# alipbcs/ZetaRay

Measured on AMD Instinct MI355X. Metric: Mrays/s, higher is better.
Workload: dtype f32; 1 GPU; Cornell Box (cornell_emissive: 58 triangles, 2 emissive) 1920x1080, G-buffer + ReSTIR PT (K1 + K11-K16: initial candidates, temporal + spatial reconnection reuse, boiling suppression; 3 non-transmissive / 4 glossy-transmissive bounces, static camera); integrator=restir_pt, parallelism=screen tiles (1, 1), settle_frames=32, ramp_frames=350, arith=contract, library=libzetaray_amd.so, frame_overlap=True, kernel_class=plain

## Files before the change

zetaray_amd/csrc/zr_api.hip:

```cpp
#include <hip/hip_runtime.h>
#include <immintrin.h>
#include <string>
#include <vector>
#include <cstdio>
#include <cstdarg>
#include <cstring>
#include <new>
#include <mutex>
#include "zr_stages.h"
#include "zr_rpt.h"
#include "zr_rdi.h"
#include "zr_sdi.h"
#include "zr_rgi.h"
#include "zr_rgi_spatial.h"
#include "zr_bvh.h"
#include "zr_taa.h"
#include "zr_svgf.h"
#include "zr_post.h"
#include "../../include/zr_srgb_table.h"

static const uint16_t kRptSampleSet[1024] = {
#include "zr_rpt_sample_set.inc"
};


static thread_local std::string g_err;
static int Fail(int code, const char* fmt, ...)
{
    char buf[512];
    va_list ap; va_start(ap, fmt); vsnprintf(buf, sizeof(buf), fmt, ap); va_end(ap);
    g_err = buf;
    return code;
}
#define HIP_TRY(expr) do { hipError_t e_ = (expr); if (e_ != hipSuccess) return Fail(ZR_ERR_HIP, "%s failed: %s (%s:%d)", #expr, hipGetErrorString(e_), __FILE__, __LINE__); } while (0)

static int RequireDevice(int device)
{
    int n = 0;
    hipError_t e = hipGetDeviceCount(&n);
    if (e != hipSuccess || n <= 0) return Fail(ZR_ERR_NO_DEVICE, "no usable HIP device (hipGetDeviceCount: %s); libzetaray_amd has no CPU path", hipGetErrorString(e));
    if (device < 0 || device >= n) return Fail(ZR_ERR_INVALID_ARG, "device %d out of range (0..%d)", device, n - 1);
    HIP_TRY(hipSetDevice(device));
    return ZR_OK;
}

#include "zr_kernels.h"

#ifdef ZR_EXPERIMENTS
#define ZR_EXP_ENV(name) std::getenv(name)
#else
#define ZR_EXP_ENV(name) ((const char*)nullptr)
#endif
#include "zr_bvh_device.h"
namespace zr { int DeviceProbeRun(int device, float min_ms, zr_device_probe* out, std::string& err); }
namespace zr { hipError_t LaunchInscattering(hipStream_t s, const SceneView& sc, const zr_frame_constants& g, const InscatterParams& c, uint32_t* grid); }
namespace zr { hipError_t LaunchDisplayView(hipStream_t s, int option, const GBuf& gb, uint32_t dw, uint32_t dh, float cameraNear, float roughnessTh, F4* out, uint32_t* outSrgb); }
namespace zr { hipError_t LaunchPickOutline(hipStream_t s, const zr_vertex* vertices, const uint32_t* indices, const zr_mesh_instance* instances, uint32_t inst, uint32_t numTris,
    const post::PickWvp& m, uint32_t dw, uint32_t dh, uint32_t rw, uint32_t rh, int4* tris, uint32_t* count, uint8_t* mask, F4* out, uint32_t* outSrgb); }
namespace zr { hipError_t LaunchMoveInstances(hipStream_t st, zr_mesh_instance* cur, const zr_mesh_instance* prev, float* toWorld, uint32_t n, uint32_t* slot,
    const uint32_t* moved, uint32_t nMoved, zr_emissive_triangle* emissives, const zr_emissive_triangle* object, const uint32_t* owner, uint32_t emFirst, uint32_t emEnd); }
ZR_RPT_GROUPS_PRODUCT(extern template)
#ifdef ZR_EXPERIMENTS
ZR_RPT_GROUP_C(extern template)
#endif

__global__ void __launch_bounds__(kBlock) k_gbuffer(SceneView sc, zr_frame_constants g, GBuf gb, uint32_t tilesX, uint32_t pickXY, uint32_t* pick)
{
    uint32_t x, y; PixelOfThread(tilesX, gb.x0, gb.y0, &x, &y);
    if (x >= gb.x0 + gb.w || y >= gb.y0 + gb.h) return;
    ZR_TRAV_STACK(stack);
    GBufferPixel(sc, g, gb, x, y, stack, nullptr, (x | (y << 16)) == pickXY ? pick : nullptr);
}

template<bool TEX, bool PLAIN>
__global__ void __launch_bounds__(kBlock) k_pt_init(SceneView sc, zr_frame_constants g, GBuf gb, PtParams prm, float* finalRGBA,
    F4* firstBOP, PathQueue out, uint32_t* outCount, uint32_t* outRays, uint32_t cap, uint32_t tilesX)
{
    sc.plain = PLAIN; gb.plain = PLAIN;
    uint32_t x, y; PixelOfThread(tilesX, gb.x0, gb.y0, &x, &y);
    PathOut po; po.alive = false;
    if (x < gb.x0 + gb.w && y < gb.y0 + gb.h) PtInitPixel(sc, g, gb, prm, x, y, finalRGBA, firstBOP, po, TEX);
    const uint32_t slot = AllocPathAndRaysBlock(outCount, out.rayList, cap, outRays, po.alive, po.alive && po.rayC_d.w >= 0, po.alive && po.rayM_d.w >= 0, po.alive && po.rayS_d.w >= 0);
    if (po.alive) WritePath(out, slot, po, TEX);
}

__global__ void __launch_bounds__(kBlock) k_trace_simple(SceneView sc, PathQueue q, const uint32_t* rayCount, uint32_t cap, unsigned long long* counters)
{
    const uint32_t nC = rayCount[0], nM = rayCount[kCounterStride], total = nC + nM + rayCount[2 * kCounterStride];
    ZR_TRAV_STACK(stack);
#ifdef ZR_NODE_CACHE_MORE
    ZR_NODE_CACHE_FILL(stack, sc, kBlock);
#endif
    for (uint32_t base = blockIdx.x * kBlock; base < total; base += gridDim.x * kBlock)
    {
        const uint32_t j = base + threadIdx.x;
        bool closest = false, shadow = false;
        if (j < total)
        {
            uint32_t type, i;
            RayOfIndex(q.rayList, cap, nC, nM, j, type, i);
            F4 ro, rd;
            if (type == 0) { rd = q.rayC_d[i]; ro = q.rayC_o[i]; }
            else if (type == 1) { rd = q.rayM_d[i]; ro = q.rayM_o[i]; }
            else { rd = q.rayS_d[i]; ro = q.rayS_o[i]; }
            const uint32_t lightID = type == 2 ? q.sLightID[i] : 0u;
            const bool vis = type == 2 && lightID == kVisibilityRayID;
            const RawHit h = TraverseDyn(sc, xyz(ro), xyz(rd), ro.w, rd.w, (type == 2 && !vis) ? ZR_SUBGROUP_NON_EMISSIVE : ZR_SUBGROUP_ALL, stack, vis);
            if (type == 0) q.hitC[i] = PackRawHit(h);
            else if (type == 1) q.hitM[i] = PackRawHit(h);
            else q.visS[i] = SegmentVisible(sc, h, lightID);
            closest = type != 2; shadow = type == 2;
        }
        CountWave(&counters[0], closest);
        CountWave(&counters[1], shadow);
    }
}

static constexpr uint32_t kTraceChunk = 256;
static constexpr uint32_t kTraceRefillAt = 16;
__global__ void __launch_bounds__(kBlock) k_trace(SceneView sc, PathQueue q, const uint32_t* rayCount, uint32_t cap, uint32_t* cursor, unsigned long long* counters)
{
    const uint32_t nC = rayCount[0], nM = rayCount[kCounterStride], total = nC + nM + rayCount[2 * kCounterStride];
    ZR_TRAV_STACK(stack);
    const uint32_t lane = __lane_id();
    TravState st; TravLane L; L.triCur = 0; L.triEnd = 0; L.done = true;
    uint32_t slot = 0;
    bool laneAnyHit = false;
    uint32_t nClosest = 0, nShadow = 0;
    uint32_t chunkPos = 0, chunkEnd = 0;
    bool exhausted = false;
    for (;;)
    {
        const bool atTri = L.triCur < L.triEnd;
        const bool atNode = !L.done && !atTri;
        const uint64_t mIdle = __ballot(L.done);
        const uint32_t nNode = (uint32_t)__popcll(__ballot(atNode)), nTri = (uint32_t)__popcll(__ballot(atTri)), nIdle = (uint32_t)__popcll(mIdle);
        const bool canRefill = !(exhausted && chunkPos == chunkEnd);
        if (nNode + nTri == 0 && !canRefill) break;
        if (canRefill && (nIdle >= kTraceRefillAt || nNode + nTri == 0))
        {
            if (chunkPos == chunkEnd)
            {
                uint32_t b = 0;
                if (lane == 0) b = atomicAdd(cursor, kTraceChunk);
                b = __builtin_amdgcn_readfirstlane(b);
                exhausted = b >= total;
                chunkPos = b < total ? b : total;
                chunkEnd = b + kTraceChunk < total ? b + kTraceChunk : total;
            }
            const uint32_t rank = (uint32_t)__popcll(mIdle & ((1ull << lane) - 1ull));
            const uint32_t j = chunkPos + rank;
            if (L.done && j < chunkEnd)
            {
                uint32_t type, i;
                RayOfIndex(q.rayList, cap, nC, nM, j, type, i);
                slot = i | (type << 30);
                F4 ro, rd;
                if (type == 0) { rd = q.rayC_d[i]; ro = q.rayC_o[i]; }
                else if (type == 1) { rd = q.rayM_d[i]; ro = q.rayM_o[i]; }
                else { rd = q.rayS_d[i]; ro = q.rayS_o[i]; }
                L.done = false;
                if (type == 2)
                {
                    laneAnyHit = q.sLightID[i] == kVisibilityRayID;
                    TravInit(sc, st, xyz(ro), xyz(rd), ro.w, rd.w, laneAnyHit ? ZR_SUBGROUP_ALL : ZR_SUBGROUP_NON_EMISSIVE, false, 0); nShadow++;
                }
                else { laneAnyHit = false; TravInit(sc, st, xyz(ro), xyz(rd), ro.w, rd.w, ZR_SUBGROUP_ALL, false, 0); nClosest++; }
                TravEnter(sc, st, L, st.cur);
            }
            chunkPos = chunkPos + nIdle < chunkEnd ? chunkPos + nIdle : chunkEnd;
            continue;
        }
        bool stepped = false;
        if (nNode >= nTri) { if (atNode) { TravNodePhase(sc, st, L, stack); stepped = true; } }
        else if (atTri) { TravTriPhase(sc, st, L, stack, laneAnyHit); stepped = true; }
        if (stepped && L.done)
        {
            const uint32_t type = slot >> 30, i = slot & 0x3fffffffu;
            if (type == 0) q.hitC[i] = PackRawHit(st.best);
            else if (type == 1) q.hitM[i] = PackRawHit(st.best);
            else q.visS[i] = SegmentVisible(sc, st.best, q.sLightID[i]);
        }
    }
    uint32_t a = nClosest, b = nShadow;
    for (int s = 1; s < 64; s <<= 1) { a += __shfl_xor(a, s); b += __shfl_xor(b, s); }
    if (lane == 0) { if (a) atomicAdd(&counters[0], (unsigned long long)a); if (b) atomicAdd(&counters[1], (unsigned long long)b); }
}

template<bool TEX>
__device__ __forceinline__ void PtShadeBody(const SceneView& sc, const zr_frame_constants& g, const PtParams& prm, const PathQueue& in, const uint32_t* inCount,
    const PathQueue& out, uint32_t* outCount, uint32_t* outRays, uint32_t cap, float* finalRGBA, const F4* firstBOP, uint32_t* groupMax)
{
    const uint32_t n = *inCount;
    for (uint32_t base = blockIdx.x * kBlock; base < n; base += gridDim.x * kBlock)
    {
        const uint32_t i = base + threadIdx.x;
        PathOut po; po.alive = false;
        if (i < n) PtShadePath(sc, g, prm, in, i, finalRGBA, firstBOP, groupMax, po, TEX);
        const uint32_t slot = AllocPathAndRaysBlock(outCount, out.rayList, cap, outRays, po.alive, po.alive && po.rayC_d.w >= 0, po.alive && po.rayM_d.w >= 0, po.alive && po.rayS_d.w >= 0);
        if (po.alive) WritePath(out, slot, po, TEX);
    }
}
template<bool PLAIN>
__global__ void __launch_bounds__(kBlock) k_pt_shade(SceneView sc, zr_frame_constants g, PtParams prm, PathQueue in, const uint32_t* inCount,
    PathQueue out, uint32_t* outCount, uint32_t* outRays, uint32_t cap, float* finalRGBA, const F4* firstBOP, uint32_t* groupMax)
{ sc.plain = PLAIN; PtShadeBody<false>(sc, g, prm, in, inCount, out, outCount, outRays, cap, finalRGBA, firstBOP, groupMax); }
#ifndef ZR_WAVES_PT_SHADE_TEX
#define ZR_WAVES_PT_SHADE_TEX ZR_WAVES_MIN(2)
#endif
__global__ void __launch_bounds__(kBlock) ZR_WAVES_PT_SHADE_TEX k_pt_shade_tex(SceneView sc, zr_frame_constants g, PtParams prm, PathQueue in, const uint32_t* inCount,
    PathQueue out, uint32_t* outCount, uint32_t* outRays, uint32_t cap, float* finalRGBA, const F4* firstBOP, uint32_t* groupMax)
{ sc.plain = 0; PtShadeBody<true>(sc, g, prm, in, inCount, out, outCount, outRays, cap, finalRGBA, firstBOP, groupMax); }

// ... 112 lines not shown
        if (i < 65536u)
        {
            if (zr_asuint(zr_f16_to_f32((uint16_t)i)) != zr_asuint(zr_f16_to_f32_portable((uint16_t)i))) b1++;
            const float x = (float)(uint32_t)i;
            volatile float d255 = 255.0f, d65535 = 65535.0f;
            if (zr_asuint(zr_div255(x)) != zr_asuint(x / d255)) b1++;
            if (zr_asuint(zr_div65535(x)) != zr_asuint(x / d65535)) b1++;
        }
    }
    if (b0) atomicAdd(bad, b0);
    if (b1) atomicAdd(bad + 1, b1);
}

__global__ void __launch_bounds__(256) k_composite(zr_frame_constants g, const uint16_t* mr, const F4* skyDI, const F4* emissiveDI, const F4* indirect, F4* out, uint32_t n,
    SkyLutView sky, uint32_t w)
{
    const uint32_t i = blockIdx.x * blockDim.x + threadIdx.x;
    if (i < n) out[i] = CompositePixel(g, mr[i], skyDI, emissiveDI, indirect, i, out[i], sky, i % w, i / w);
}
__global__ void __launch_bounds__(256) k_composite_inscattering(zr_frame_constants g, const uint16_t* mr, const float* depth, const F4* skyDI, const F4* emissiveDI,
    const F4* indirect, F4* out, uint32_t n, SkyLutView sky, uint32_t w, InscatterGridView grid)
{
    const uint32_t i = blockIdx.x * blockDim.x + threadIdx.x;
    if (i >= n) return;
    const F4 c = CompositePixel(g, mr[i], skyDI, emissiveDI, indirect, i, out[i], sky, i % w, i / w);
    out[i] = CompositeInscattering(g, mr[i], c, depth[i], grid, i % w, i / w);
}

static constexpr int kFfW = 64, kFfH = 16, kFfLW = kFfW + 2, kFfLH = kFfH + 2;
__global__ void __launch_bounds__(256) k_firefly(const F4* in, const float* depth, F4* out, uint32_t W, uint32_t H)
{
    __shared__ F4 sCol[kFfLW * kFfLH];
    __shared__ float sDep[kFfLW * kFfLH];
    const int bx = (int)blockIdx.x * kFfW, by = (int)blockIdx.y * kFfH;
    for (int t = threadIdx.x; t < kFfLW * kFfLH; t += 256)
    {
        const int lx = t % kFfLW, ly = t / kFfLW;
        const int gx = bx + lx - 1, gy = by + ly - 1;
        const bool inside = gx >= 0 && gy >= 0 && gx < (int)W && gy < (int)H;
        sCol[t] = inside ? in[(size_t)gy * W + gx] : f4(v3(0.0f), 0.0f);
        sDep[t] = inside ? depth[(size_t)gy * W + gx] : ZR_FLT_MAX;
    }
    __syncthreads();
    auto col = [&](int tx, int ty) { return xyz(sCol[ty * kFfLW + tx]); };
    auto dep = [&](int tx, int ty) { return sDep[ty * kFfLW + tx]; };
    for (int k = 0; k < 4; k++)
    {
        const int lx = threadIdx.x & 63, ly = (threadIdx.x >> 6) + 4 * k;
        const int x = bx + lx, y = by + ly;
        if (x >= (int)W || y >= (int)H) continue;
        const F4 c = sCol[(ly + 1) * kFfLW + lx + 1];
        V3 color = xyz(c);
        if (sDep[(ly + 1) * kFfLW + lx + 1] != ZR_FLT_MAX) color = FireflyClamp(col, dep, lx + 1, ly + 1, x, y, (int)W, (int)H, color);
        out[(size_t)y * W + x] = f4(color, c.w);
    }
}

__global__ void k_presample(SceneView sc, uint32_t total, uint32_t frameNum, uint32_t numEmissives, zr_presampled_tri* out)
{
    const uint32_t i = blockIdx.x * blockDim.x + threadIdx.x;
    if (i < total) out[i] = PresampleEmissive(sc, i, frameNum, numEmissives);
}

__global__ void k_estimate_power(SceneView sc, uint32_t n, float* power)
{
    const uint32_t i = blockIdx.x * blockDim.x + threadIdx.x;
    if (i < n) power[i] = EstimateTriPower(sc, sc.emissives[i]);
}

__device__ __forceinline__ float WaveSumButterfly(float v);
__global__ void __launch_bounds__(64) k_build_lvg(SceneView sc, zr_frame_constants g, uint32_t dx, uint32_t dy, uint32_t dz, float ex, float ey, float ez,
    float offset_y, zr_voxel_sample* out)
{
    const uint32_t dim[3] = {dx, dy, dz};
    const int v[3] = {(int)blockIdx.x, (int)blockIdx.y, (int)blockIdx.z};
    zr_voxel_sample r; float w_sum, target_z; uint32_t numLights;
    LvgThread(sc, g, dim, v3(ex, ey, ez), offset_y, v, threadIdx.x, r, w_sum, target_z, numLights);
    const float w_sum_group = WaveSumButterfly(w_sum);
    uint32_t n = numLights;
    for (int s = 1; s < 64; s <<= 1) n += __shfl_xor(n, s);
    LvgFinish(r, target_z, w_sum_group, n);
    out[(size_t)LvgFlatten(v, dim) * ZR_LVG_SAMPLES_PER_VOXEL + threadIdx.x] = r;
}

__global__ void __launch_bounds__(64) k_sky_lut(zr_frame_constants g, uint32_t w, uint32_t h, uint32_t* out)
{
    const uint32_t x = blockIdx.x * 8 + (threadIdx.x & 7), y = blockIdx.y * 8 + (threadIdx.x >> 3);
    if (x < w && y < h) out[(size_t)y * w + x] = SkyViewLutTexel(g, x, y, w, h);
}

__global__ void __launch_bounds__(kBlock) k_trace_rays(SceneView sc, const F4* rays, uint32_t n, uint32_t mask, U4* hits)
{
    ZR_TRAV_STACK(stack);
    for (uint32_t i = blockIdx.x * kBlock + threadIdx.x; i < n; i += gridDim.x * kBlock)
        hits[i] = TraceClosestRay(sc, rays[2 * i], rays[2 * i + 1], mask, stack);
}
__global__ void __launch_bounds__(kBlock) k_trace_rays_any(SceneView sc, const F4* rays, uint32_t n, uint32_t mask, uint32_t* occ)
{
    ZR_TRAV_STACK(stack);
    for (uint32_t i = blockIdx.x * kBlock + threadIdx.x; i < n; i += gridDim.x * kBlock)
    {
        const F4 ro = rays[2 * i], rd = rays[2 * i + 1];
        RawHit h = Traverse<true>(sc, xyz(ro), xyz(rd), ro.w, rd.w, mask, stack);
        occ[i] = h.tri != kInvalidTri ? 1u : 0u;
    }
}

#include "zr_kernels_di.h"
__global__ void k_rgi_spatial(rgi::GiFrame F, zr_frame_constants g, uint32_t tilesX, unsigned long long* counters, rgi::SpatialParams sp);
ZR_DI_GROUP(extern template, false)
ZR_DI_GROUP(extern template, true)
static const uint16_t kRdiSampleSet[64] = {
#include "zr_rdi_sample_set.inc"
};

template<typename T> struct DevBuf
{
    T* p = nullptr; size_t n = 0;
    int Alloc(size_t count) { Free(); n = count; if (!count) return ZR_OK; hipError_t e = hipMalloc((void**)&p, count * sizeof(T)); if (e != hipSuccess) { p = nullptr; return Fail(ZR_ERR_OOM, "hipMalloc(%zu B) failed: %s", count * sizeof(T), hipGetErrorString(e)); } return ZR_OK; }
    int AllocZero(size_t count) { int r = Alloc(count); if (r) return r; HIP_TRY(hipMemset(p, 0, count * sizeof(T))); return ZR_OK; }
    int Upload(const T* src, size_t count) { int r = Alloc(count); if (r) return r; if (count) HIP_TRY(hipMemcpy(p, src, count * sizeof(T), hipMemcpyHostToDevice)); return ZR_OK; }
    void Free() { if (p) { (void)hipFree(p); p = nullptr; } n = 0; }
    ~DevBuf() { Free(); }
};
struct HaloPlane { void* base; size_t bpp; };
template<typename T, size_t PER_PIXEL = 1> struct Plane : DevBuf<T>
{
    static constexpr size_t bpp = sizeof(T) * PER_PIXEL;
    int Alloc(size_t pixels) { return DevBuf<T>::Alloc(pixels * PER_PIXEL); }
    int AllocZero(size_t pixels) { return DevBuf<T>::AllocZero(pixels * PER_PIXEL); }
    size_t Pixels() const { return this->n / PER_PIXEL; }
    HaloPlane Halo() const { return {this->p, bpp}; }
    void Output(void** dev, uint32_t* bytesPerPixel) const { *dev = this->p; if (bytesPerPixel) *bytesPerPixel = (uint32_t)bpp; }
};
template<typename S> static int PlanesAllocZero(S& set, size_t pixels) { return S::Each(set, [&](auto& pl) { return pl.AllocZero(pixels); }); }
template<typename S> static int PlanesHalo(const S& set, HaloPlane* out) { int n = 0; S::Each(set, [&](const auto& pl) { out[n++] = pl.Halo(); return 0; }); return n; }
template<typename S> static void PlanesOutput(const S& set, int i, void** dev, uint32_t* bpp) { S::Each(set, [&](const auto& pl) { if (i-- == 0) pl.Output(dev, bpp); return 0; }); }

struct zr_scene
{
    int device = 0;
    DevBuf<zr_vertex> vertices; DevBuf<uint32_t> indices; DevBuf<zr_mesh_instance> instances; DevBuf<zr_material> materials;
    DevBuf<zr_emissive_triangle> emissives; DevBuf<zr_alias_entry> alias; DevBuf<Bvh4Node> nodes; DevBuf<BvhTri> tris;
    std::vector<zr_material> hMaterials; std::atomic<bool> plainMaterials{false};
    uint64_t uid = [] { static std::atomic<uint64_t> next{1}; return next.fetch_add(1); }();
    DevBuf<TriMeta> meta; DevBuf<uint16_t> rho;
    DevBuf<zr_texture_desc> texDescs; DevBuf<uint8_t> texels; DevBuf<float> srgb;
    DevBuf<zr_presampled_tri> sampleSets; uint32_t numSampleSets = 0;
    DevBuf<zr_voxel_sample> lvg;
    std::vector<zr_alias_entry> aliasHost;
    std::vector<zr_vertex> hVertices; std::vector<uint32_t> hIndices; std::vector<uint8_t> hMask; std::vector<uint32_t> hNumTris;
    DevBuf<zr_mesh_instance> instancesPrev; DevBuf<Bvh4Node> nodesPrev; DevBuf<BvhTri> trisPrev; DevBuf<TriMeta> metaPrev;
    uint32_t numNodesPrev = 0, numTrisPrev = 0; bool hasPrev = false;
    DevBuf<uint32_t> levelNodes; std::vector<uint32_t> levelOffsets, hLevelOrder; DevBuf<float> nodeBounds, toWorld; bool refitReady = false;
    DevBuf<uint8_t> dMask; DeviceBvhScratch bvhScratch; bool deviceBuilt = false;
    bool aliasStale = false;
    SceneView view{};
    mutable std::mutex mtx;
    int64_t maxTex[4] = {-1, -1, -1, -1};
    uint32_t maxDepth = 0;
    struct StageSlot { void* host = nullptr; size_t cap = 0; hipEvent_t ev = nullptr; bool pending = false; };
    StageSlot stage[4]; int stageNext = 0;
    hipEvent_t updated = nullptr; hipStream_t updatedOn = nullptr; bool hasUpdate = false;
    std::vector<std::pair<hipStream_t, hipEvent_t>> users;
    struct Background
    {
        bool enabled = false; std::thread th; std::atomic<int> state{0};
        std::vector<uint32_t> levelOffsets;
        uint32_t numNodes = 0, numTris = 0, stackNeed = 0, maxDepth = 0; bool packed = false;
        uint32_t* pkg = nullptr; size_t pkgCap = 0; hipEvent_t pkgCopied = nullptr; bool pkgInFlight = false;
        std::vector<zr_mesh_instance> inst; std::vector<float> xf; std::vector<uint8_t> own;
        uint32_t refitsSince = 0; std::atomic<uint64_t> started{0}, installed{0};
        bool movedSinceBuild = false;
        double buildMs = 0, packMs = 0;
    } bg;
    DevBuf<uint32_t> bgDev;
    std::vector<float> hToWorld; std::vector<uint8_t> movedEver;
    std::vector<zr_mesh_instance> hInstances; bool toWorldDev = false;
    DevBuf<zr_emissive_triangle> objectEmissives; DevBuf<uint32_t> emissiveOwner, movedDev, movedSlot;
    ~zr_scene()
    {
        if (bg.th.joinable()) bg.th.join();
        if (bg.pkg) (void)hipHostFree(bg.pkg);
        if (bg.pkgCopied) (void)hipEventDestroy(bg.pkgCopied);
        for (StageSlot& t : stage) { if (t.ev) (void)hipEventDestroy(t.ev); if (t.host) (void)hipHostFree(t.host); }
        if (updated) (void)hipEventDestroy(updated);
        for (auto& u : users) (void)hipEventDestroy(u.second);
    }
};

static int StageAcquire(zr_scene* s, size_t bytes, zr_scene::StageSlot** out)
{
    zr_scene::StageSlot& t = s->stage[s->stageNext];
    s->stageNext = (s->stageNext + 1) % 4;
    if (t.pending) { HIP_TRY(hipEventSynchronize(t.ev)); t.pending = false; }
    if (!t.ev) HIP_TRY(hipEventCreateWithFlags(&t.ev, hipEventDisableTiming));
    if (t.cap < bytes)
    {
        if (t.host) { (void)hipHostFree(t.host); t.host = nullptr; t.cap = 0; }
        hipError_t e = hipHostMalloc(&t.host, bytes, hipHostMallocDefault);
        if (e != hipSuccess) { t.host = nullptr; return Fail(ZR_ERR_OOM, "hipHostMalloc(%zu B) failed: %s", bytes, hipGetErrorString(e)); }
        t.cap = bytes;
    }
    *out = &t;
    return ZR_OK;
}
static int StageCommit(zr_scene::StageSlot* t, hipStream_t st) { HIP_TRY(hipEventRecord(t->ev, st)); t->pending = true; return ZR_OK; }
static int SceneWaitUsers(zr_scene* s, hipStream_t st)
{
    std::lock_guard<std::mutex> lock(s->mtx);
    if (!s->hasUpdate) HIP_TRY(hipDeviceSynchronize());
    for (auto& u : s->users) if (u.first != st) HIP_TRY(hipStreamWaitEvent(st, u.second, 0));
    if (s->hasUpdate && s->updated && s->updatedOn != st) HIP_TRY(hipStreamWaitEvent(st, s->updated, 0));
    return ZR_OK;
}
static int SceneMarkUpdated(zr_scene* s, hipStream_t st)
{
    std::lock_guard<std::mutex> lock(s->mtx);
    if (!s->updated) HIP_TRY(hipEventCreateWithFlags(&s->updated, hipEventDisableTiming));
    HIP_TRY(hipEventRecord(s->updated, st));
    s->updatedOn = st; s->hasUpdate = true;
    return ZR_OK;
}
static int SceneAcquireForRender(const zr_scene* sc, hipStream_t st)
{
    std::lock_guard<std::mutex> lock(sc->mtx);
    if (sc->hasUpdate && sc->updatedOn != st) HIP_TRY(hipStreamWaitEvent(st, sc->updated, 0));
    return ZR_OK;
}
static int SceneReleaseAfterRender(const zr_scene* scc, hipStream_t st)
{
    zr_scene* sc = const_cast<zr_scene*>(scc);
    std::lock_guard<std::mutex> lock(sc->mtx);
    if (!sc->hasUpdate) return ZR_OK;
    for (auto& u : sc->users) if (u.first == st) { HIP_TRY(hipEventRecord(u.second, st)); return ZR_OK; }
    hipEvent_t ev; HIP_TRY(hipEventCreateWithFlags(&ev, hipEventDisableTiming));
    sc->users.emplace_back(st, ev);
    HIP_TRY(hipEventRecord(ev, st));
    return ZR_OK;
}

#ifdef ZR_PROF
static unsigned long long* ProfBuffer()
{
    static unsigned long long* p = nullptr;
    if (!p) { (void)hipMalloc(&p, 256 * sizeof(unsigned long long)); (void)hipMemset(p, 0, 256 * sizeof(unsigned long long)); }
    return p;
}
extern "C" int zr_debug_prof_read(unsigned long long* out256)
{
    (void)hipDeviceSynchronize();
    if (hipMemcpy(out256, ProfBuffer(), 256 * sizeof(unsigned long long), hipMemcpyDeviceToHost) != hipSuccess) return -1;
    (void)hipMemset(ProfBuffer(), 0, 256 * sizeof(unsigned long long));
    return 0;
}
#endif
static SceneView FrameView(const zr_scene* sc, const zr_frame_constants* cb)
{
    std::lock_guard<std::mutex> lock(sc->mtx);
    SceneView v = sc->view;
#ifdef ZR_PROF
    v.prof = ProfBuffer();
#endif
    if (cb)
    {
        v.baseColorMapsOffset = cb->base_color_maps_desc_heap_offset; v.normalMapsOffset = cb->normal_maps_desc_heap_offset;
        v.mrMapsOffset = cb->metallic_roughness_maps_desc_heap_offset; v.emissiveMapsOffset = cb->emissive_maps_desc_heap_offset;
    }
    v.texFilter = ZR_TEX_FILTER_ANISOTROPIC_4X;
    return v;
}
static SceneView FrameViewPrev(const zr_scene* sc, const zr_frame_constants* cb)
{
    SceneView v = FrameView(sc, cb);
    std::lock_guard<std::mutex> lock(sc->mtx);
    if (sc->hasPrev)
    {
        v.instances = sc->instancesPrev.p; v.nodes = sc->nodesPrev.p; v.tris = sc->trisPrev.p; v.triMeta = sc->metaPrev.p;
        v.numNodes = sc->numNodesPrev; v.numTris = sc->numTrisPrev;
    }
    return v;
}

struct zr_gbuffer
{
    int device = 0; uint32_t w = 0, h = 0, x0 = 0, y0 = 0;
    DevBuf<uint8_t> planeSets[3][ZR_GB_COUNT];
    int cur = 0, numSets = 2; uint64_t numRendered = 0;
    int Next() const { return (cur + 1) % numSets; }
    int Prev() const { return (cur + numSets - 1) % numSets; }
    bool plainAt[3] = {true, true, true};
    uint64_t sceneAt[3] = {0, 0, 0};
    bool tracked = false;
    hipEvent_t evWritten = nullptr; hipStream_t writer = nullptr; bool hasWrite = false;
    struct Reader { hipStream_t st; hipEvent_t ev; };
    std::vector<Reader> readers[3];
    ~zr_gbuffer() { if (evWritten) (void)hipEventDestroy(evWritten); for (auto& v : readers) for (auto& r : v) (void)hipEventDestroy(r.ev); }
    DevBuf<uint8_t>* Planes() { return planeSets[cur]; }
    const DevBuf<uint8_t>* Planes() const { return planeSets[cur]; }
    GBuf View() const { return ViewOf(cur); }
    GBuf PrevView() const { return ViewOf(Prev()); }
    GBuf ViewOf(int which) const
    {
        const DevBuf<uint8_t>* planes = planeSets[which];
        GBuf g; g.w = w; g.h = h; g.x0 = x0; g.y0 = y0;
        g.baseColor = (uint32_t*)planes[ZR_GB_BASE_COLOR].p; g.normal = (uint32_t*)planes[ZR_GB_NORMAL].p;
        g.mr = (uint16_t*)planes[ZR_GB_METALLIC_ROUGHNESS].p; g.motion = (uint32_t*)planes[ZR_GB_MOTION_VECTOR].p;
        g.emissive = (uint32_t*)planes[ZR_GB_EMISSIVE_COLOR].p; g.ior = (uint8_t*)planes[ZR_GB_IOR].p;
        g.coat = (uint16_t*)planes[ZR_GB_COAT].p; g.depth = (float*)planes[ZR_GB_DEPTH].p;
        g.triA = (uint32_t*)planes[ZR_GB_TRI_DIFF_GEO_A].p; g.triB = (uint32_t*)planes[ZR_GB_TRI_DIFF_GEO_B].p;
        return g;
    }
};

static int GBufferMarkRead(zr_gbuffer* gb, int set, hipStream_t s)
{
    if (!gb || !gb->tracked) return ZR_OK;
    for (auto& r : gb->readers[set]) if (r.st == s) { HIP_TRY(hipEventRecord(r.ev, s)); return ZR_OK; }
    hipEvent_t ev; HIP_TRY(hipEventCreateWithFlags(&ev, hipEventDisableTiming));
    gb->readers[set].push_back({s, ev});
    HIP_TRY(hipEventRecord(ev, s));
    return ZR_OK;
}
static int GBufferAcquireRead(zr_gbuffer* gb, hipStream_t s)
{
    if (!gb || !gb->tracked || !gb->hasWrite || gb->writer == s) return ZR_OK;
    HIP_TRY(hipStreamWaitEvent(s, gb->evWritten, 0));
    return ZR_OK;
}
static int GBufferAcquireWrite(zr_gbuffer* gb, int set, hipStream_t s)
{
    if (!gb->tracked) return ZR_OK;
    for (auto& r : gb->readers[set]) if (r.st != s) HIP_TRY(hipStreamWaitEvent(s, r.ev, 0));
    return ZR_OK;
}
static int GBufferMarkWritten(zr_gbuffer* gb, hipStream_t s)
{
    if (!gb->tracked) return ZR_OK;
    if (!gb->evWritten) HIP_TRY(hipEventCreateWithFlags(&gb->evWritten, hipEventDisableTiming));
    HIP_TRY(hipEventRecord(gb->evWritten, s));
    gb->writer = s; gb->hasWrite = true;
    return ZR_OK;
}

struct QueueStorage
{
    DevBuf<U4> s0; DevBuf<F4> f[8]; DevBuf<F4> rays[6]; DevBuf<uint32_t> lightID; DevBuf<U4> hitC, hitM; DevBuf<uint32_t> visS, rayList;
    DevBuf<F4> t[8];
    int AllocTex(size_t cap)
    {
        int r;
        for (auto& b : t) if (b.n != cap && (r = b.Alloc(cap))) return r;
        return ZR_OK;
    }
    int Alloc(size_t cap)
    {
        int r;
        if ((r = s0.Alloc(cap))) return r;
        for (auto& b : f) if ((r = b.Alloc(cap))) return r;
        for (auto& b : rays) if ((r = b.Alloc(cap))) return r;
        if ((r = lightID.Alloc(cap))) return r;
        if ((r = hitC.Alloc(cap))) return r;
        if ((r = hitM.Alloc(cap))) return r;
        if ((r = visS.Alloc(cap))) return r;
        if ((r = rayList.Alloc(3 * cap))) return r;
        return ZR_OK;
    }
    PathQueue View() const
    {
        PathQueue q;
        q.s0 = s0.p; q.s1 = f[0].p; q.s2 = f[1].p; q.s3 = f[2].p; q.s4 = f[3].p; q.s5 = f[4].p; q.s6 = f[5].p; q.s7 = f[6].p; q.s8 = f[7].p;
        q.rayC_o = rays[0].p; q.rayC_d = rays[1].p; q.rayM_o = rays[2].p; q.rayM_d = rays[3].p; q.rayS_o = rays[4].p; q.rayS_d = rays[5].p;
        q.sLightID = lightID.p; q.hitC = hitC.p; q.hitM = hitM.p; q.visS = visS.p; q.rayList = rayList.p;
        for (int k = 0; k < 8; k++) q.t[k] = t[k].p;
        return q;
    }
};

static constexpr uint32_t kRptListWords = 12;
static constexpr uint32_t kLargeSceneNodes = 1;
static std::atomic<uint32_t> g_largeSceneNodes{kLargeSceneNodes};
static std::atomic<bool> g_materialClassKernels{true};
static bool PlainClass(const zr_scene* sc, const zr_gbuffer* gb)
{
    if (!sc->plainMaterials.load(std::memory_order_relaxed) || !g_materialClassKernels.load(std::memory_order_relaxed)) return false;
    const int c = gb->cur;
    if (!(gb->plainAt[c] && gb->sceneAt[c] == sc->uid)) return false;
    if (gb->numRendered >= 2 && !(gb->plainAt[gb->Prev()] && gb->sceneAt[gb->Prev()] == sc->uid)) return false;
    return true;
}
static constexpr int kMaxRounds = 16;
static constexpr int kMaxTimers = 64;
static constexpr int kCounterSlots = 16;
static const char* const kCounterNames[kCounterSlots] = {"trace", "rpt_pathtrace", "rpt_replay_ctt", "rpt_replay_ttc", "rpt_reconnect_temporal",
    "rpt_replay_cts", "rpt_replay_stc", "rpt_reconnect_spatial", "rdi_temporal", "rdi_spatial", "rgi", "sdi_temporal", "sdi_spatial", "rgi_spatial", "", ""};

struct zr_pass
{
    int kind = 0, device = 0, integrator = 0;
    bool initialized = false;
    uint32_t w = 0, h = 0;
    zr_params params{};
    QueueStorage q[2];
    DevBuf<uint32_t> skyLut;
    bool inscatterOn = false; InscatterParams inscatter{}; DevBuf<uint32_t> inscatterGrid;
    const zr_pass* inscatterSky = nullptr;
    Plane<float, 4> finalRGBA; Plane<F4> firstBOP; DevBuf<uint32_t> counts; DevBuf<unsigned long long> counters;
    DevBuf<uint32_t> groupMax;
    zr_counters hostCounters{0, 0};
    uint32_t pickXY = 0xffffffffu; DevBuf<uint32_t> pickBuf; bool pickWritten = false;
    struct ResStorage
    {
        Plane<uint32_t> A; Plane<float, 2> B; Plane<U4> C, D; Plane<uint16_t> E; Plane<float, 2> F; Plane<uint32_t, 2> G;
        template<typename S, typename Fn> static int Each(S& s, Fn f)
        { int r; if ((r = f(s.A)) || (r = f(s.B)) || (r = f(s.C)) || (r = f(s.D)) || (r = f(s.E)) || (r = f(s.F)) || (r = f(s.G))) return r; return ZR_OK; }
        rpt::ResPlanes View() const { rpt::ResPlanes v; v.A = A.p; v.B = B.p; v.C = C.p; v.D = D.p; v.E = E.p; v.F = F.p; v.G = G.p; return v; }
    } res[3];
    struct RBufStorage
    {
        Plane<uint16_t, 4> A; Plane<U4> B, C; Plane<uint16_t> D;
        template<typename S, typename Fn> static int Each(S& s, Fn f) { int r; if ((r = f(s.A)) || (r = f(s.B)) || (r = f(s.C)) || (r = f(s.D))) return r; return ZR_OK; }
        rpt::RBuf View() const { rpt::RBuf v; v.A = A.p; v.B = B.p; v.C = C.p; v.D = D.p; return v; }
    } rb[2];
    Plane<F4> rptTarget, rptTargetAlt; Plane<uint8_t, 2> rptNeighbor; DevBuf<uint16_t> rptSampleSet;
    bool overlap = false, overlapCarry = false; int rptSet[3] = {0, 1, 2}; int tgtIdx = 0, finIdx = 0, finOut = 0;
    Plane<float, 4> finalAlt, finalAlt2;
    hipEvent_t evDone[2] = {nullptr, nullptr}; bool haveDone[2] = {false, false}; hipStream_t doneStream[2] = {nullptr, nullptr}; uint64_t ovFrame = 0;
    hipStream_t overlapStream = nullptr;
    hipEvent_t evCand = nullptr, evTemporal = nullptr;
    hipStream_t candStream = nullptr, reuseStream = nullptr; bool haveCand = false, haveTemporal = false;
    zr_pass::ResStorage& RptCur() { return res[rptSet[currIdx]]; }
// ... 217 lines not shown
    for (int r = 0; r < 3; r++) { nodeBounds[6 * (size_t)ni + r] = lo[r]; nodeBounds[6 * (size_t)ni + 3 + r] = hi[r]; }
}

struct HaloJob
{
    struct Plane { char* base; uint32_t bpp; } planes[8];
    struct Rect { uint32_t first, w, h; uint32_t pad; uint64_t offset; } rects[ZR_HALO_MAX_RECTS];
    uint32_t numPlanes, numRects, pitch;
    char* buf;
};
template<bool PACK> __global__ void __launch_bounds__(256) k_halo(HaloJob J)
{
    const HaloJob::Rect r = J.rects[blockIdx.y];
    const uint32_t n = r.w * r.h;
    for (uint32_t i = blockIdx.x * blockDim.x + threadIdx.x; i < n; i += gridDim.x * blockDim.x)
    {
        const size_t px = (size_t)r.first + (size_t)(i / r.w) * J.pitch + (i % r.w);
        char* cursor = J.buf + r.offset;
        for (uint32_t k = 0; k < J.numPlanes; k++)
        {
            const uint32_t bpp = J.planes[k].bpp;
            char* a = J.planes[k].base + px * bpp;
            char* b = cursor + (size_t)i * bpp;
            char* dst = PACK ? b : a; const char* src = PACK ? a : b;
            switch (bpp)
            {
            case 16: *(uint4*)dst = *(const uint4*)src; break;
            case 8: *(uint2*)dst = *(const uint2*)src; break;
            case 4: *(uint32_t*)dst = *(const uint32_t*)src; break;
            case 2: *(uint16_t*)dst = *(const uint16_t*)src; break;
            default: *dst = *src; break;
            }
            cursor += (size_t)n * bpp;
        }
    }
}

extern "C" {

int zr_abi_version(void) { return ZR_ABI_VERSION; }
const char* zr_last_error(void) { return g_err.c_str(); }

int zr_device_count(int* count)
{
    if (!count) return Fail(ZR_ERR_INVALID_ARG, "count is null");
    int n = 0;
    hipError_t e = hipGetDeviceCount(&n);
    *count = (e == hipSuccess) ? n : 0;
    return ZR_OK;
}

int zr_device_probe_run(int device, float min_ms, zr_device_probe* out)
{
    if (!out) return Fail(ZR_ERR_INVALID_ARG, "out is null");
    if (int r = RequireDevice(device)) return r;
    std::string err;
    if (zr::DeviceProbeRun(device, min_ms, out, err)) return Fail(ZR_ERR_HIP, "zr_device_probe_run: %s", err.c_str());
    return ZR_OK;
}

int zr_selftest_half_conversions(int device, uint64_t* m0, uint64_t* m1)
{
    if (!m0 || !m1) return Fail(ZR_ERR_INVALID_ARG, "null argument");
    int r = RequireDevice(device);
    if (r) return r;
    DevBuf<unsigned long long> bad;
    if ((r = bad.Alloc(2))) return r;
    HIP_TRY(hipMemset(bad.p, 0, 2 * sizeof(unsigned long long)));
    hipLaunchKernelGGL(k_selftest_half, dim3(256 * 64), dim3(256), 0, 0, bad.p);
    HIP_TRY(hipGetLastError());
    unsigned long long h[2];
    HIP_TRY(hipMemcpy(h, bad.p, sizeof(h), hipMemcpyDeviceToHost));
    *m0 = h[0]; *m1 = h[1];
    return ZR_OK;
}

int zr_params_default(zr_params* p)
{
    if (!p) return Fail(ZR_ERR_INVALID_ARG, "params is null");
    memset(p, 0, sizeof(*p));
    p->flags = ZR_IND_TEMPORAL_RESAMPLE | ZR_IND_SPATIAL_RESAMPLE | ZR_IND_RUSSIAN_ROULETTE | ZR_IND_BOILING_SUPPRESSION |
               ZR_IND_SORT_TEMPORAL | ZR_IND_SORT_SPATIAL;
    p->max_non_tr_bounces = 3; p->max_glossy_tr_bounces = 4; p->m_max_temporal = 10; p->m_max_spatial = 8;
    p->alpha_min = 0.175f * 0.175f; p->presampling = 0; p->num_sample_sets = 128; p->sample_set_size = 512;
    p->taa_blend_weight = 0.1f;
    p->ae_min_lum = 5e-3f; p->ae_max_lum = 4.0f; p->ae_lum_map_exp = 0.5f; p->ae_adaptation_rate = 1.0f;
    p->tex_filter = ZR_TEX_FILTER_ANISOTROPIC_4X;
    p->svgf_alpha = 0.2f; p->svgf_alpha_moments = 0.2f; p->svgf_sigma_l = 4.0f; p->svgf_sigma_z = 1.0f; p->svgf_normal_power_log2 = 7; p->svgf_iterations = 5;
    p->num_spatial_passes = 1;
    p->display_tonemapper = ZR_TONEMAP_NEUTRAL; p->display_auto_exposure = 1; p->display_saturation = 1.0f; p->display_agx_exp = 1.0f;
    p->use_lvg = 0; p->lvg_grid_dim = 32u | (8u << 10) | (40u << 20);
    p->lvg_extents[0] = 0.6f; p->lvg_extents[1] = 0.45f; p->lvg_extents[2] = 0.6f; p->lvg_offset_y = 0.1f;
    return ZR_OK;
}

int zr_alias_table_build(const float* power, uint32_t n, uint32_t align_phase, zr_alias_entry* out)
{
    if (!power || !out || n == 0) return Fail(ZR_ERR_INVALID_ARG, "zr_alias_table_build: null/empty input");
    std::vector<float> probs(power, power + n);
    BuildAliasTableHost(probs, out, align_phase);
    return ZR_OK;
}

static void BvhLevels(const std::vector<Bvh4Node>& nodes, std::vector<uint32_t>& order, std::vector<uint32_t>& offsets)
{
    order.clear(); offsets.clear();
    if (nodes.empty()) return;
    std::vector<std::vector<uint32_t>> levels(1, std::vector<uint32_t>(1, 0u));
    for (size_t l = 0; l < levels.size(); l++)
    {
        std::vector<uint32_t> next;
        for (uint32_t ni : levels[l]) for (int c = 0; c < 4; c++) { const uint32_t r = nodes[ni].child[c]; if (r != kEmptyChild && !(r & kLeafBit)) next.push_back(r); }
        if (!next.empty()) levels.push_back(std::move(next));
    }
    for (size_t l = levels.size(); l-- > 0;) { offsets.push_back((uint32_t)order.size()); order.insert(order.end(), levels[l].begin(), levels[l].end()); }
    offsets.push_back((uint32_t)order.size());
}

static int DeviceRebuild(zr_scene* s, hipStream_t st)
{
    const uint32_t nt = (uint32_t)s->meta.n;
    int r;
    if (s->nodes.n < nt || s->tris.n < nt || s->nodeBounds.n < 6 * (size_t)nt)
    {
        HIP_TRY(hipDeviceSynchronize());
        if (s->nodes.n < nt && (r = s->nodes.Alloc(nt))) return r;
        if (s->tris.n < nt && (r = s->tris.Alloc(nt))) return r;
        if (s->nodeBounds.n < 6 * (size_t)nt && (r = s->nodeBounds.Alloc(6 * (size_t)nt))) return r;
    }
    if (!s->dMask.p && (r = s->dMask.Upload(s->hMask.data(), s->hMask.size()))) return r;
    DeviceBvhInputs in; in.numTris = nt; in.meta = s->meta.p; in.instances = s->instances.p; in.toWorld = s->toWorld.p; in.vertices = s->vertices.p;
    in.indices = s->indices.p; in.instanceMask = s->dMask.p;
    DeviceBvhOutputs out; out.tris = s->tris.p; out.nodes = s->nodes.p; out.nodeCap = (uint32_t)s->nodes.n;
    std::string err;
    if (DeviceBuildBvh4(st, s->bvhScratch, in, out, err)) return Fail(ZR_ERR_HIP, "device BVH build: %s", err.c_str());
    if (out.stackNeed + 1 > (uint32_t)kTravStack) return Fail(ZR_ERR_UNSUPPORTED, "device-built BVH has %u levels: needs %u traversal stack entries (limit %d); use the host builder", out.numLevels, out.stackNeed, kTravStack - 1);
    s->hLevelOrder = out.levelOrder; s->levelOffsets = out.levelOffsets;
    if (s->levelNodes.n < s->hLevelOrder.size()) { HIP_TRY(hipStreamSynchronize(st)); if ((r = s->levelNodes.Alloc(nt))) return r; }
    HIP_TRY(hipMemcpyAsync(s->levelNodes.p, s->hLevelOrder.data(), s->hLevelOrder.size() * sizeof(uint32_t), hipMemcpyHostToDevice, st));
    for (size_t l = 0; l + 1 < s->levelOffsets.size(); l++)
    {
        const uint32_t first = s->levelOffsets[l], cnt = s->levelOffsets[l + 1] - first;
        hipLaunchKernelGGL(k_refit_level, dim3((cnt + 63) / 64), dim3(64), 0, st, s->nodes.p, s->levelNodes.p + first, cnt, s->tris.p, s->nodeBounds.p);
    }
    HIP_TRY(hipGetLastError());
    HIP_TRY(hipStreamSynchronize(st));
    SceneView& v = s->view;
    v.nodes = s->nodes.p; v.tris = s->tris.p; v.numNodes = out.numNodes; v.numTris = nt;
    if (out.numLevels > s->maxDepth) s->maxDepth = out.numLevels;
    s->deviceBuilt = true;
    return ZR_OK;
}

static bool MaterialsArePlain(const std::vector<zr_material>& m)
{
    const uint32_t lobes = (1u << ZR_MAT_METALLIC_BIT) | (1u << ZR_MAT_TRANSMISSIVE_BIT) | (1u << ZR_MAT_THIN_WALLED_BIT);
    for (const zr_material& x : m) if ((x.coat_color_flags & lobes) || ((x.base_color_tex_subsurf_coat_weight >> 24) & 0xffu)) return false;
    return !m.empty();
}
int zr_scene_create(int device, const zr_scene_desc* d, zr_scene** out)
{
    if (!d || !out) return Fail(ZR_ERR_INVALID_ARG, "zr_scene_create: null argument");
    if (!d->vertices || !d->indices || !d->instances || !d->materials || !d->rho_lut || !d->instance_to_world || !d->instance_mask || !d->instance_num_tris)
        return Fail(ZR_ERR_INVALID_ARG, "zr_scene_create: incomplete scene description");
    int r = RequireDevice(device);
    if (r) return r;
    zr_scene* s = new (std::nothrow) zr_scene();
    if (!s) return Fail(ZR_ERR_OOM, "out of host memory");
    s->device = device;
    uint64_t totalTris = 0;
    for (uint32_t i = 0; i < d->num_instances; i++) totalTris += d->instance_num_tris[i];
    const char* buildEnv = std::getenv("ZR_BVH_BUILD");
    const bool deviceBuild = buildEnv && !std::strcmp(buildEnv, "device") && totalTris > BvhBuilder::kTinyScene;
    BuiltBvh bvh;
    if (deviceBuild)
    {
        bvh.meta.reserve((size_t)totalTris);
        for (uint32_t i = 0; i < d->num_instances; i++) for (uint32_t p = 0; p < d->instance_num_tris[i]; p++) { TriMeta m; m.mesh = i; m.prim = p; bvh.meta.push_back(m); }
    }
    else
    {
        BvhBuilder builder;
        bvh = builder.Build(*d);
    }
    if (bvh.stackNeed + 1 > (uint32_t)kTravStack) { delete s; return Fail(ZR_ERR_UNSUPPORTED, "BVH needs %u traversal stack entries (limit %d)", bvh.stackNeed, kTravStack - 1); }
    s->maxDepth = bvh.maxDepth;
#define UP(buf, ptr, cnt) if ((r = s->buf.Upload(ptr, cnt))) { delete s; return r; }
    UP(vertices, d->vertices, d->num_vertices);
    UP(indices, d->indices, d->num_indices);
    UP(instances, d->instances, d->num_instances);
    UP(materials, d->materials, d->num_materials);
    UP(emissives, d->emissives, d->num_emissives);
    UP(nodes, bvh.nodes4.data(), bvh.nodes4.size());
    UP(tris, bvh.tris.data(), bvh.tris.size());
    UP(meta, bvh.meta.data(), bvh.meta.size());
    UP(rho, d->rho_lut, (size_t)d->rho_dim[0] * d->rho_dim[1] * d->rho_dim[2]);
    if (d->num_textures)
    {
        if (!d->textures || !d->texels) { delete s; return Fail(ZR_ERR_INVALID_ARG, "zr_scene_create: num_textures > 0 without textures / texels"); }
        for (uint32_t i = 0; i < d->num_textures; i++)
        {
            const zr_texture_desc& t = d->textures[i];
            const zr_tex_mip last = zr_tex_mip_of(&t, t.num_mips ? t.num_mips - 1u : 0u);
            const uint64_t end = last.offset + (uint64_t)last.w * last.h * (t.format == ZR_TEX_RG8 ? 2u : 4u);
            if (!t.num_mips || !t.width || !t.height || t.format > ZR_TEX_RG8 || (t.offset & 3u) || end > d->texel_bytes)
            { delete s; return Fail(ZR_ERR_INVALID_ARG, "zr_scene_create: texture %u is malformed or lies outside the texel blob", i); }
        }
        UP(texDescs, d->textures, d->num_textures);
        UP(texels, d->texels, d->texel_bytes);
    }
    UP(srgb, zr_srgb_to_linear_table, 256);
#undef UP
    SceneView& v = s->view;
    v.vertices = s->vertices.p; v.indices = s->indices.p; v.instances = s->instances.p; v.materials = s->materials.p;
    v.emissives = s->emissives.p; v.alias = nullptr; v.sampleSets = nullptr; v.sampleSetSize = 0; v.nodes = s->nodes.p; v.tris = s->tris.p; v.triMeta = s->meta.p;
    v.rho.data = s->rho.p; v.rho.dx = d->rho_dim[0]; v.rho.dy = d->rho_dim[1]; v.rho.dz = d->rho_dim[2];
    v.numEmissives = d->num_emissives; v.numNodes = (uint32_t)bvh.nodes4.size(); v.numTris = (uint32_t)bvh.tris.size();
    s->hMaterials.assign(d->materials, d->materials + d->num_materials);
    s->plainMaterials = MaterialsArePlain(s->hMaterials) && d->num_textures == 0;
    v.tex.descs = s->texDescs.p; v.tex.texels = s->texels.p; v.tex.srgb = s->srgb.p; v.tex.count = d->num_textures;
    for (uint32_t i = 0; i < d->num_materials; i++)
    {
        const zr_material& m = d->materials[i];
        const uint32_t t[4] = { m.base_color_tex_subsurf_coat_weight & 0xffffu, m.normal_tex_tr_depth & 0xffffu,
                                m.mr_tex_spec_roughness_coat_roughness & 0xffffu, m.emissive_tex_alpha_cutoff_coat_ior & 0xffffu };
        for (int k = 0; k < 4; k++) if (t[k] != ZR_INVALID_TEX && (int64_t)t[k] > s->maxTex[k]) s->maxTex[k] = t[k];
    }
    for (uint32_t i = 0; i < d->num_instances; i++)
        if (d->instances[i].base_color_tex != ZR_INVALID_TEX && (int64_t)d->instances[i].base_color_tex > s->maxTex[0]) s->maxTex[0] = d->instances[i].base_color_tex;
    for (uint32_t i = 0; i < d->num_emissives; i++)
    { const uint32_t t = d->emissives[i].packed_b & 0xffffu; if (t != ZR_INVALID_TEX && (int64_t)t > s->maxTex[3]) s->maxTex[3] = t; }
    { const char* e = getenv("ZR_SCENE_UPDATE"); s->bg.enabled = e && !strcmp(e, "refit_sah"); }
    s->hVertices.assign(d->vertices, d->vertices + d->num_vertices); s->hIndices.assign(d->indices, d->indices + d->num_indices);
    s->hMask.assign(d->instance_mask, d->instance_mask + d->num_instances); s->hNumTris.assign(d->instance_num_tris, d->instance_num_tris + d->num_instances);
    s->hToWorld.assign(d->instance_to_world, d->instance_to_world + 12 * (size_t)d->num_instances); s->movedEver.assign(d->num_instances, 0);
    s->hInstances.assign(d->instances, d->instances + d->num_instances);
    BvhLevels(bvh.nodes4, s->hLevelOrder, s->levelOffsets);
    if (!s->hLevelOrder.empty() && (r = s->levelNodes.Upload(s->hLevelOrder.data(), s->hLevelOrder.size()))) { delete s; return r; }
    if (deviceBuild)
    {
        if ((r = s->toWorld.Upload(d->instance_to_world, 12 * (size_t)d->num_instances)) || (r = DeviceRebuild(s, nullptr))) { delete s; return r; }
        s->toWorldDev = true;
    }
    { hipError_t e = hipDeviceSynchronize(); if (e != hipSuccess) { delete s; return Fail(ZR_ERR_HIP, "hipDeviceSynchronize failed: %s", hipGetErrorString(e)); } }
    *out = s;
    return ZR_OK;
}

static void RaiseMaxTex(zr_scene* s, int table, uint32_t tex) { if (tex != ZR_INVALID_TEX && (int64_t)tex > s->maxTex[table]) s->maxTex[table] = tex; }

int zr_scene_update_emissives_async(zr_scene* s, void* stream, const zr_emissive_triangle* triangles, uint32_t first, uint32_t count)
{
    if (!s || (!triangles && count)) return Fail(ZR_ERR_INVALID_ARG, "zr_scene_update_emissives: null argument");
    if ((uint64_t)first + count > s->emissives.n) return Fail(ZR_ERR_INVALID_ARG, "zr_scene_update_emissives: [%u, %u) exceeds the scene's %zu emissive triangles", first, first + count, s->emissives.n);
    if (!count) return ZR_OK;
    HIP_TRY(hipSetDevice(s->device));
    hipStream_t st = (hipStream_t)stream;
    int r; zr_scene::StageSlot* t;
    if ((r = StageAcquire(s, (size_t)count * sizeof(zr_emissive_triangle), &t))) return r;
    memcpy(t->host, triangles, (size_t)count * sizeof(zr_emissive_triangle));
    for (uint32_t i = 0; i < count; i++) RaiseMaxTex(s, 3, triangles[i].packed_b & 0xffffu);
    if ((r = SceneWaitUsers(s, st))) return r;
    HIP_TRY(hipMemcpyAsync(s->emissives.p + first, t->host, (size_t)count * sizeof(zr_emissive_triangle), hipMemcpyHostToDevice, st));
    if ((r = StageCommit(t, st))) return r;
    return SceneMarkUpdated(s, st);
}
int zr_scene_update_materials_async(zr_scene* s, void* stream, const zr_material* materials, uint32_t first, uint32_t count)
{
    if (!s || (!materials && count)) return Fail(ZR_ERR_INVALID_ARG, "zr_scene_update_materials: null argument");
    if ((uint64_t)first + count > s->materials.n) return Fail(ZR_ERR_INVALID_ARG, "zr_scene_update_materials: [%u, %u) exceeds the scene's %zu materials", first, first + count, s->materials.n);
    if (!count) return ZR_OK;
    HIP_TRY(hipSetDevice(s->device));
    hipStream_t st = (hipStream_t)stream;
    int r; zr_scene::StageSlot* t;
    if ((r = StageAcquire(s, (size_t)count * sizeof(zr_material), &t))) return r;
    memcpy(t->host, materials, (size_t)count * sizeof(zr_material));
    for (uint32_t i = 0; i < count; i++)
    {
        RaiseMaxTex(s, 0, materials[i].base_color_tex_subsurf_coat_weight & 0xffffu); RaiseMaxTex(s, 1, materials[i].normal_tex_tr_depth & 0xffffu);
        RaiseMaxTex(s, 2, materials[i].mr_tex_spec_roughness_coat_roughness & 0xffffu); RaiseMaxTex(s, 3, materials[i].emissive_tex_alpha_cutoff_coat_ior & 0xffffu);
    }
    if ((r = SceneWaitUsers(s, st))) return r;
    std::copy(materials, materials + count, s->hMaterials.begin() + first);
    s->plainMaterials = MaterialsArePlain(s->hMaterials) && s->view.tex.count == 0;
    HIP_TRY(hipMemcpyAsync(s->materials.p + first, t->host, (size_t)count * sizeof(zr_material), hipMemcpyHostToDevice, st));
    if ((r = StageCommit(t, st))) return r;
    return SceneMarkUpdated(s, st);
}
int zr_scene_update_emissives(zr_scene* s, const zr_emissive_triangle* triangles, uint32_t first, uint32_t count)
{
    int r = zr_scene_update_emissives_async(s, nullptr, triangles, first, count);
    if (r || !count) return r;
    HIP_TRY(hipDeviceSynchronize());
    return ZR_OK;
}
int zr_scene_update_materials(zr_scene* s, const zr_material* materials, uint32_t first, uint32_t count)
{
    int r = zr_scene_update_materials_async(s, nullptr, materials, first, count);
    if (r || !count) return r;
    HIP_TRY(hipDeviceSynchronize());
    return ZR_OK;
}
int zr_scene_invalidate_alias_table(zr_scene* s)
{
    if (!s) return Fail(ZR_ERR_INVALID_ARG, "zr_scene_invalidate_alias_table: null argument");
    std::lock_guard<std::mutex> lock(s->mtx);
    s->view.alias = nullptr; s->aliasHost.clear();
    return ZR_OK;
}
int zr_scene_invalidate_alias_table_deferred(zr_scene* s)
{
    if (!s) return Fail(ZR_ERR_INVALID_ARG, "zr_scene_invalidate_alias_table_deferred: null argument");
    std::lock_guard<std::mutex> lock(s->mtx);
    if (s->view.alias) s->aliasStale = true;
    return ZR_OK;
}
struct MovedList { const uint32_t* idx; const float* xf; uint32_t n, emFirst, emEnd; };
static int SceneRefitUpdate(zr_scene* s, hipStream_t st, const zr_mesh_instance* instances, const float* instance_to_world, uint32_t n, const MovedList* moved);

int zr_scene_update_instances_async(zr_scene* s, void* stream, const zr_mesh_instance* instances, const float* instance_to_world, uint32_t n)
{
    if (!s || !instances || !instance_to_world) return Fail(ZR_ERR_INVALID_ARG, "zr_scene_update_instances: null argument");
    if (n != s->instances.n) return Fail(ZR_ERR_INVALID_ARG, "zr_scene_update_instances: %u instances, the scene has %zu", n, s->instances.n);
    HIP_TRY(hipSetDevice(s->device));
    hipStream_t st = (hipStream_t)stream;
    const char* modeEnv = std::getenv("ZR_SCENE_UPDATE");
    bool rebuild = modeEnv && !std::strcmp(modeEnv, "rebuild");
    int r;
    for (uint32_t i = 0; i < n; i++) RaiseMaxTex(s, 0, instances[i].base_color_tex);
    for (uint32_t i = 0; i < n; i++)
        if (std::memcmp(s->hToWorld.data() + 12 * (size_t)i, instance_to_world + 12 * (size_t)i, 12 * sizeof(float))) { s->movedEver[i] = 1; s->bg.movedSinceBuild = true; }
    std::memcpy(s->hToWorld.data(), instance_to_world, 12 * (size_t)n * sizeof(float));
    s->hInstances.assign(instances, instances + n);
    const bool rebuildHost = modeEnv && !std::strcmp(modeEnv, "rebuild_host");
    if (rebuild && s->meta.n > BvhBuilder::kTinyScene)
    {
        const size_t nt = s->meta.n;
        HIP_TRY(hipDeviceSynchronize());
        std::lock_guard<std::mutex> lock(s->mtx);
        const SceneView viewBefore = s->view;
        const uint32_t numNodesPrevBefore = s->numNodesPrev, numTrisPrevBefore = s->numTrisPrev;
        if ((r = (s->instancesPrev.n == n ? ZR_OK : s->instancesPrev.Alloc(n))) || (s->nodesPrev.n < nt && (r = s->nodesPrev.Alloc(nt))) ||
            (s->trisPrev.n < nt && (r = s->trisPrev.Alloc(nt))) || (s->metaPrev.n != s->meta.n && (r = s->metaPrev.Alloc(s->meta.n))) ||
            (s->toWorld.n != 12 * (size_t)n && (r = s->toWorld.Alloc(12 * (size_t)n)))) return r;
        if (!s->hasPrev && !s->refitReady) HIP_TRY(hipMemcpy(s->metaPrev.p, s->meta.p, s->meta.n * sizeof(TriMeta), hipMemcpyDeviceToDevice));
        std::swap(s->instances.p, s->instancesPrev.p); std::swap(s->instances.n, s->instancesPrev.n);
        std::swap(s->nodes.p, s->nodesPrev.p); std::swap(s->nodes.n, s->nodesPrev.n);
        std::swap(s->tris.p, s->trisPrev.p); std::swap(s->tris.n, s->trisPrev.n);
        std::swap(s->meta.p, s->metaPrev.p); std::swap(s->meta.n, s->metaPrev.n);
        s->numNodesPrev = s->view.numNodes; s->numTrisPrev = s->view.numTris; s->hasPrev = true;
        HIP_TRY(hipMemcpy(s->instances.p, instances, (size_t)n * sizeof(zr_mesh_instance), hipMemcpyHostToDevice));
        HIP_TRY(hipMemcpy(s->toWorld.p, instance_to_world, 12 * (size_t)n * sizeof(float), hipMemcpyHostToDevice));
        s->toWorldDev = true;
        s->view.instances = s->instances.p; s->view.triMeta = s->meta.p;
        if ((r = DeviceRebuild(s, st)))
        {
            (void)hipDeviceSynchronize();
            std::swap(s->instances.p, s->instancesPrev.p); std::swap(s->instances.n, s->instancesPrev.n);
            std::swap(s->nodes.p, s->nodesPrev.p); std::swap(s->nodes.n, s->nodesPrev.n);
            std::swap(s->tris.p, s->trisPrev.p); std::swap(s->tris.n, s->trisPrev.n);
            std::swap(s->meta.p, s->metaPrev.p); std::swap(s->meta.n, s->metaPrev.n);
            s->view = viewBefore; s->numNodesPrev = numNodesPrevBefore; s->numTrisPrev = numTrisPrevBefore; s->hasPrev = false;
            return r;
        }
        s->refitReady = false;
        return ZR_OK;
    }
    if (rebuild || rebuildHost)
    {
        zr_scene_desc d; memset(&d, 0, sizeof(d));
        d.vertices = s->hVertices.data(); d.num_vertices = (uint32_t)s->hVertices.size(); d.indices = s->hIndices.data(); d.num_indices = (uint32_t)s->hIndices.size();
        d.instances = instances; d.num_instances = n; d.instance_to_world = instance_to_world; d.instance_mask = s->hMask.data(); d.instance_num_tris = s->hNumTris.data();
        BvhBuilder builder;
        BuiltBvh bvh = builder.Build(d);
        if (bvh.stackNeed + 1 > (uint32_t)kTravStack) return Fail(ZR_ERR_UNSUPPORTED, "BVH needs %u traversal stack entries (limit %d)", bvh.stackNeed, kTravStack - 1);
        HIP_TRY(hipDeviceSynchronize());
        std::lock_guard<std::mutex> lock(s->mtx);
        std::swap(s->instances.p, s->instancesPrev.p); std::swap(s->instances.n, s->instancesPrev.n);
        std::swap(s->nodes.p, s->nodesPrev.p); std::swap(s->nodes.n, s->nodesPrev.n);
        std::swap(s->tris.p, s->trisPrev.p); std::swap(s->tris.n, s->trisPrev.n);
        std::swap(s->meta.p, s->metaPrev.p); std::swap(s->meta.n, s->metaPrev.n);
        s->numNodesPrev = s->view.numNodes; s->numTrisPrev = s->view.numTris; s->hasPrev = true;
        if ((r = s->instances.Upload(instances, n)) || (r = s->nodes.Upload(bvh.nodes4.data(), bvh.nodes4.size())) ||
            (r = s->tris.Upload(bvh.tris.data(), bvh.tris.size())) || (r = s->meta.Upload(bvh.meta.data(), bvh.meta.size()))) return r;
        SceneView& v = s->view;
        v.instances = s->instances.p; v.nodes = s->nodes.p; v.tris = s->tris.p; v.triMeta = s->meta.p;
        v.numNodes = (uint32_t)bvh.nodes4.size(); v.numTris = (uint32_t)bvh.tris.size();
        if (bvh.maxDepth > s->maxDepth) s->maxDepth = bvh.maxDepth;
        BvhLevels(bvh.nodes4, s->hLevelOrder, s->levelOffsets);
        if ((r = s->levelNodes.Upload(s->hLevelOrder.data(), s->hLevelOrder.size()))) return r;
        s->refitReady = false;
        s->toWorldDev = false;
        return ZR_OK;
    }
    return SceneRefitUpdate(s, st, instances, instance_to_world, n, nullptr);
}
static int SceneRefitUpdate(zr_scene* s, hipStream_t st, const zr_mesh_instance* instances, const float* instance_to_world, uint32_t n, const MovedList* moved)
{
    int r;
    const bool install = s->bg.enabled && s->bg.state.load(std::memory_order_acquire) == 2 && s->bg.packed && s->bg.inst.size() == n &&
                         s->bg.numTris == s->view.numTris && s->bg.stackNeed + 1 <= (uint32_t)kTravStack;
    if (s->bg.enabled && s->bg.state.load(std::memory_order_acquire) == 2 && !install)
    {
        if (s->bg.th.joinable()) s->bg.th.join();
        s->bg.state.store(0);
    }
    if (install && s->bg.th.joinable()) s->bg.th.join();
    if (s->bg.enabled)
    {
        const size_t cap = s->view.numTris;
        if (s->nodes.n < cap || (s->refitReady && s->nodesPrev.n < cap) || s->levelNodes.n < cap || s->nodeBounds.n < 6 * cap || s->bgDev.n < 5 * cap || !s->dMask.p)
        {
            HIP_TRY(hipDeviceSynchronize());
            if (!s->dMask.p && (r = s->dMask.Upload(s->hMask.data(), s->hMask.size()))) return r;
            if (s->bgDev.n < 5 * cap && (r = s->bgDev.Alloc(5 * cap))) return r;
            auto grow = [&](auto& buf, size_t count, size_t keep) -> int {
                if (buf.n >= count) return ZR_OK;
                std::remove_reference_t<decltype(buf)> nb; int rr = nb.Alloc(count); if (rr) return rr;
                if (keep && buf.p) HIP_TRY(hipMemcpy(nb.p, buf.p, keep * sizeof(*buf.p), hipMemcpyDeviceToDevice));
                std::swap(buf.p, nb.p); std::swap(buf.n, nb.n);
                return ZR_OK; };
            std::lock_guard<std::mutex> lockGrow(s->mtx);
            if ((r = grow(s->nodes, cap, s->view.numNodes)) || (s->nodesPrev.p && (r = grow(s->nodesPrev, cap, s->refitReady || s->hasPrev ? s->numNodesPrev : 0))) ||
                (r = grow(s->levelNodes, cap, s->hLevelOrder.size())) || (r = grow(s->nodeBounds, 6 * cap, 0))) return r;
            s->view.nodes = s->nodes.p;
        }
    }
    const size_t nn = s->view.numNodes, nt = s->view.numTris;
    const size_t instBytes = (size_t)n * sizeof(zr_mesh_instance), xfBytes = 12 * (size_t)n * sizeof(float);
    zr_scene::StageSlot* t;
    const bool seedXf = moved && (!s->toWorldDev || s->toWorld.n != 12 * (size_t)n);
    const size_t movedBytes = moved ? 13 * (size_t)moved->n * sizeof(uint32_t) : 0, seedBytes = seedXf ? xfBytes : 0;
    if ((r = StageAcquire(s, moved ? seedBytes + movedBytes : instBytes + xfBytes, &t))) return r;
    if (!moved) { memcpy(t->host, instances, instBytes); memcpy((char*)t->host + instBytes, instance_to_world, xfBytes); }
    else
    {
        if (seedXf) memcpy(t->host, s->hToWorld.data(), xfBytes);
        memcpy((char*)t->host + seedBytes, moved->xf, 12 * (size_t)moved->n * sizeof(float));
        memcpy((char*)t->host + seedBytes + 12 * (size_t)moved->n * sizeof(float), moved->idx, (size_t)moved->n * sizeof(uint32_t));
    }
    if ((r = SceneWaitUsers(s, st))) return r;
    std::lock_guard<std::mutex> lock(s->mtx);
    if (moved && (s->movedSlot.n != n || s->movedDev.n != 13 * (size_t)n))
    {
        if ((r = s->movedSlot.Alloc(n)) || (r = s->movedDev.Alloc(13 * (size_t)n))) return r;
        HIP_TRY(hipMemsetAsync(s->movedSlot.p, 0xff, (size_t)n * sizeof(uint32_t), st));
    }
    if (!s->refitReady)
    {
        const size_t nodeCap = s->bg.enabled ? std::max(nn, nt) : nn;
        if ((s->instancesPrev.n != n && (r = s->instancesPrev.Alloc(n))) || (nodeCap && s->nodesPrev.n < nodeCap && (r = s->nodesPrev.Alloc(nodeCap))) ||
            (s->trisPrev.n != nt && (r = s->trisPrev.Alloc(nt))) || (s->metaPrev.n != s->meta.n && (r = s->metaPrev.Alloc(s->meta.n))) ||
            (nodeCap && s->nodeBounds.n < 6 * nodeCap && (r = s->nodeBounds.Alloc(6 * nodeCap))) || (s->toWorld.n != 12 * (size_t)n && (r = s->toWorld.Alloc(12 * (size_t)n)))) return r;
        HIP_TRY(hipMemcpyAsync(s->instancesPrev.p, s->instances.p, instBytes, hipMemcpyDeviceToDevice, st));
        if (nn) HIP_TRY(hipMemcpyAsync(s->nodesPrev.p, s->nodes.p, nn * sizeof(Bvh4Node), hipMemcpyDeviceToDevice, st));
        HIP_TRY(hipMemcpyAsync(s->trisPrev.p, s->tris.p, nt * sizeof(BvhTri), hipMemcpyDeviceToDevice, st));
        HIP_TRY(hipMemcpyAsync(s->metaPrev.p, s->meta.p, s->meta.n * sizeof(TriMeta), hipMemcpyDeviceToDevice, st));
        s->refitReady = true;
    }
    std::swap(s->instances.p, s->instancesPrev.p); std::swap(s->nodes.p, s->nodesPrev.p); std::swap(s->tris.p, s->trisPrev.p); std::swap(s->meta.p, s->metaPrev.p);
    s->numNodesPrev = (uint32_t)nn; s->numTrisPrev = (uint32_t)nt; s->hasPrev = true;
    if (!moved)
    {
        HIP_TRY(hipMemcpyAsync(s->instances.p, t->host, instBytes, hipMemcpyHostToDevice, st));
        HIP_TRY(hipMemcpyAsync(s->toWorld.p, (char*)t->host + instBytes, xfBytes, hipMemcpyHostToDevice, st));
    }
    else
    {
        if (seedXf) HIP_TRY(hipMemcpyAsync(s->toWorld.p, t->host, xfBytes, hipMemcpyHostToDevice, st));
        if (moved->n) HIP_TRY(hipMemcpyAsync(s->movedDev.p, (char*)t->host + seedBytes, movedBytes, hipMemcpyHostToDevice, st));
        HIP_TRY(zr::LaunchMoveInstances(st, s->instances.p, s->instancesPrev.p, s->toWorld.p, n, s->movedSlot.p, s->movedDev.p, moved->n,
            s->emissives.p, s->objectEmissives.p, s->emissiveOwner.p, moved->emFirst, moved->emEnd));
    }
    s->toWorldDev = true;
    if ((r = StageCommit(t, st))) return r;
    uint32_t numNodesNow = (uint32_t)nn;
    if (install)
    {
        zr_scene::Background& B = s->bg;
        const size_t devWords = 4 * (size_t)B.numNodes + B.numTris;
        if (!B.pkgCopied) HIP_TRY(hipEventCreateWithFlags(&B.pkgCopied, hipEventDisableTiming));
        HIP_TRY(hipMemcpyAsync(s->bgDev.p, B.pkg, devWords * sizeof(uint32_t), hipMemcpyHostToDevice, st));
        HIP_TRY(hipMemcpyAsync(s->levelNodes.p, B.pkg + devWords, (size_t)B.numNodes * sizeof(uint32_t), hipMemcpyHostToDevice, st));
        HIP_TRY(hipEventRecord(B.pkgCopied, st)); B.pkgInFlight = true;
        hipLaunchKernelGGL(k_install_topology, dim3((uint32_t)((std::max<size_t>(B.numNodes, B.numTris) + 255) / 256)), dim3(256), 0, st,
            s->nodes.p, s->bgDev.p, B.numNodes, s->tris.p, s->bgDev.p + 4 * (size_t)B.numNodes, B.numTris, s->meta.p, s->dMask.p);
        s->hLevelOrder.assign(B.pkg + devWords, B.pkg + devWords + B.numNodes); s->levelOffsets = B.levelOffsets;
        numNodesNow = B.numNodes;
        if (B.maxDepth > s->maxDepth) s->maxDepth = B.maxDepth;
        s->refitReady = false;
        s->deviceBuilt = false;
        B.installed++; B.refitsSince = 0;
        B.state.store(0, std::memory_order_release);
    }
    else if (s->bg.enabled) s->bg.refitsSince++;
    hipLaunchKernelGGL(k_refit_tris, dim3((uint32_t)((nt + 255) / 256)), dim3(256), 0, st, s->tris.p, (uint32_t)nt, s->meta.p, s->instances.p, s->toWorld.p, s->vertices.p, s->indices.p);
    for (size_t l = 0; l + 1 < s->levelOffsets.size(); l++)
    {
        const uint32_t first = s->levelOffsets[l], cnt = s->levelOffsets[l + 1] - first;
        hipLaunchKernelGGL(k_refit_level, dim3((cnt + 63) / 64), dim3(64), 0, st, s->nodes.p, s->levelNodes.p + first, cnt, s->tris.p, s->nodeBounds.p);
    }
    HIP_TRY(hipGetLastError());
    if (moved)
    {
        for (uint32_t j = 0; j < moved->n; j++)
        {
            float* M = s->hToWorld.data() + 12 * (size_t)moved->idx[j];
            if (std::memcmp(M, moved->xf + 12 * (size_t)j, 12 * sizeof(float))) { s->movedEver[moved->idx[j]] = 1; s->bg.movedSinceBuild = true; }
            std::memcpy(M, moved->xf + 12 * (size_t)j, 12 * sizeof(float));
        }
    }
    SceneView& v = s->view;
    v.instances = s->instances.p; v.nodes = s->nodes.p; v.tris = s->tris.p; v.triMeta = s->meta.p; v.numNodes = numNodesNow;
    if (!s->updated) HIP_TRY(hipEventCreateWithFlags(&s->updated, hipEventDisableTiming));
    HIP_TRY(hipEventRecord(s->updated, st));
    s->updatedOn = st; s->hasUpdate = true;
    if (s->bg.enabled && s->bg.state.load(std::memory_order_acquire) == 0 && s->bg.refitsSince >= 1 && s->bg.movedSinceBuild && s->meta.n > BvhBuilder::kTinyScene)
    {
        zr_scene::Background& B = s->bg;
        B.movedSinceBuild = false;
        if (B.th.joinable()) B.th.join();
        B.inst.assign(instances, instances + n); B.xf.assign(s->hToWorld.begin(), s->hToWorld.end());
        { const char* e = ZR_EXP_ENV("ZR_BVH_GROUP"); if (e && !std::strcmp(e, "0")) B.own.clear(); else B.own = s->movedEver; }
        B.state.store(1, std::memory_order_release); B.started++;
        zr_scene* sp = s;
        B.th = std::thread([sp] {
            zr_scene::Background& Q = sp->bg;
            const auto t0 = std::chrono::steady_clock::now();
            zr_scene_desc d; memset(&d, 0, sizeof(d));
            d.vertices = sp->hVertices.data(); d.num_vertices = (uint32_t)sp->hVertices.size(); d.indices = sp->hIndices.data(); d.num_indices = (uint32_t)sp->hIndices.size();
            d.instances = Q.inst.data(); d.num_instances = (uint32_t)Q.inst.size(); d.instance_to_world = Q.xf.data(); d.instance_mask = sp->hMask.data(); d.instance_num_tris = sp->hNumTris.data();
            BvhBuilder builder;
            BuiltBvh bvh = builder.Build(d, Q.own.empty() ? nullptr : Q.own.data());
            std::vector<uint32_t> levelOrder;
            BvhLevels(bvh.nodes4, levelOrder, Q.levelOffsets);
            const auto t1 = std::chrono::steady_clock::now();
            const size_t nn = bvh.nodes4.size(), nt = bvh.tris.size(), words = 5 * nn + nt;
            Q.packed = false;
            if (hipSetDevice(sp->device) == hipSuccess)
            {
                if (Q.pkgInFlight) { (void)hipEventSynchronize(Q.pkgCopied); Q.pkgInFlight = false; }
                if (Q.pkgCap < words)
                {
                    if (Q.pkg) { (void)hipHostFree(Q.pkg); Q.pkg = nullptr; Q.pkgCap = 0; }
                    void* h = nullptr;
                    if (hipHostMalloc(&h, (words + words / 8) * sizeof(uint32_t), hipHostMallocDefault) == hipSuccess) { Q.pkg = (uint32_t*)h; Q.pkgCap = words + words / 8; }
                    else (void)hipGetLastError();
                }
                if (Q.pkg)
                {
                    uint32_t* w = Q.pkg;
                    for (size_t i = 0; i < nn; i++) for (int c = 0; c < 4; c++) *w++ = bvh.nodes4[i].child[c];
                    for (size_t i = 0; i < nt; i++) *w++ = bvh.tris[i].gidx;
                    std::memcpy(w, levelOrder.data(), nn * sizeof(uint32_t));
                    Q.packed = true;
                }
            }
            Q.numNodes = (uint32_t)nn; Q.numTris = (uint32_t)nt; Q.stackNeed = bvh.stackNeed; Q.maxDepth = bvh.maxDepth;
            Q.buildMs = std::chrono::duration<double, std::milli>(t1 - t0).count();
            Q.packMs = std::chrono::duration<double, std::milli>(std::chrono::steady_clock::now() - t1).count();
            if (ZR_EXP_ENV("ZR_BVH_TIMING"))
                std::fprintf(stderr, "[zr_scene] background tree: %zu nodes over %zu triangles, build %.1f ms, package (%.1f MB pinned) %.1f ms\n", nn, nt, Q.buildMs, words * 4e-6, Q.packMs);
            Q.state.store(2, std::memory_order_release);
        });
    }
    return ZR_OK;
}
int zr_scene_set_background_rebuild(zr_scene* s, int enable)
{
    if (!s) return Fail(ZR_ERR_INVALID_ARG, "zr_scene_set_background_rebuild: null scene");
    std::lock_guard<std::mutex> lock(s->mtx);
    s->bg.enabled = enable != 0;
    return ZR_OK;
}
int zr_scene_background_rebuild_stats(zr_scene* s, uint64_t* started, uint64_t* installed, int* building)
{
    if (!s) return Fail(ZR_ERR_INVALID_ARG, "zr_scene_background_rebuild_stats: null scene");
    if (started) *started = s->bg.started.load(std::memory_order_relaxed);
    if (installed) *installed = s->bg.installed.load(std::memory_order_relaxed);
    if (building) *building = s->bg.state.load(std::memory_order_acquire);
    return ZR_OK;
}
int zr_scene_update_instances(zr_scene* s, const zr_mesh_instance* instances, const float* instance_to_world, uint32_t n)
{
    int r = zr_scene_update_instances_async(s, nullptr, instances, instance_to_world, n);
    if (r) return r;
    HIP_TRY(hipDeviceSynchronize());
    return ZR_OK;
}

int zr_scene_set_object_emissives(zr_scene* s, const zr_emissive_triangle* object_space, uint32_t n)
{
    if (!s || (!object_space && n)) return Fail(ZR_ERR_INVALID_ARG, "zr_scene_set_object_emissives: null argument");
    if (n != s->emissives.n) return Fail(ZR_ERR_INVALID_ARG, "zr_scene_set_object_emissives: %u records, the scene has %zu emissive triangles", n, s->emissives.n);
    std::vector<uint32_t> owner(n, 0xffffffffu);
    for (size_t i = 0; i < s->hInstances.size(); i++)
    {
        const uint32_t b = s->hInstances[i].base_emissive_tri_offset;
        if (b == 0xffffffffu) continue;
        if ((uint64_t)b + s->hNumTris[i] > n) return Fail(ZR_ERR_INVALID_ARG, "zr_scene_set_object_emissives: instance %zu carries light triangles [%u, %llu), the scene has %u", i, b, (unsigned long long)b + s->hNumTris[i], n);
        std::fill(owner.begin() + b, owner.begin() + b + s->hNumTris[i], (uint32_t)i);
    }
    HIP_TRY(hipSetDevice(s->device));
    HIP_TRY(hipDeviceSynchronize());
    int r;
    if ((r = s->objectEmissives.Upload(object_space, n)) || (r = s->emissiveOwner.Upload(owner.data(), n))) { s->objectEmissives.Free(); s->emissiveOwner.Free(); return r; }
    HIP_TRY(hipDeviceSynchronize());
    for (uint32_t i = 0; i < n; i++) RaiseMaxTex(s, 3, object_space[i].packed_b & 0xffffu);
    return ZR_OK;
}
int zr_scene_has_object_emissives(const zr_scene* s) { return s && s->objectEmissives.p ? 1 : 0; }
int zr_scene_move_instances_async(zr_scene* s, void* stream, const uint32_t* instance_idx, const float* world_3x4, uint32_t n_moved)
{
    if (!s) return Fail(ZR_ERR_INVALID_ARG, "zr_scene_move_instances: null scene");
    if (n_moved && (!instance_idx || !world_3x4)) return Fail(ZR_ERR_INVALID_ARG, "zr_scene_move_instances: null argument with %u moved instances", n_moved);
    const char* modeEnv = std::getenv("ZR_SCENE_UPDATE");
    if (modeEnv && (!std::strcmp(modeEnv, "rebuild") || !std::strcmp(modeEnv, "rebuild_host")))
        return Fail(ZR_ERR_UNSUPPORTED, "zr_scene_move_instances: ZR_SCENE_UPDATE=%s is a host-synchronous path; the device form of the update needs the refit (default or refit_sah)", modeEnv);
    const uint32_t n = (uint32_t)s->instances.n;
    MovedList moved{instance_idx, world_3x4, n_moved, 0xffffffffu, 0u};
    {
        std::vector<uint8_t> listed(n, 0);
        for (uint32_t j = 0; j < n_moved; j++)
        {
            const uint32_t i = instance_idx[j];
            if (i >= n) return Fail(ZR_ERR_INVALID_ARG, "zr_scene_move_instances: instance %u (entry %u of the list), the scene has %u", i, j, n);
            if (listed[i]) return Fail(ZR_ERR_INVALID_ARG, "zr_scene_move_instances: instance %u is listed twice", i);
// ... 1782 lines not shown
```

zetaray_amd/csrc/zr_dev_scene.h:

```cpp
#pragma once
#include "zr_dev_bsdf.h"
#include "zr_sky.h"
#include "../../include/zr_texture.h"
#include "../../include/zr_intersect.h"

namespace zr {

struct BvhNode { float lmin[3], lmax[3], rmin[3], rmax[3]; uint32_t left, right, pad0, pad1; };
struct Bvh4Node
{
    float ox, oy, oz; uint32_t exps;
    uint32_t child[4];
    uint32_t qlox, qloy, qloz, qhix;
    uint32_t qhiy, qhiz, pad0, pad1;
};
struct BvhTri { float v0[3]; uint32_t gidx; float e1[3]; uint32_t mask; float e2[3]; uint32_t id; };
struct TriMeta { uint32_t mesh, prim; };

static constexpr uint32_t kLeafBit = 0x80000000u;
static constexpr uint32_t kInvalidTri = 0xffffffffu;
static constexpr uint32_t kEmptyChild = 0xffffffffu;
static constexpr uint32_t kWholeSceneLeaf = 0xfffffffeu;

struct SceneView
{
    const zr_vertex* vertices;
    const uint32_t* indices;
    const zr_mesh_instance* instances;
    const zr_material* materials;
    const zr_emissive_triangle* emissives;
    const zr_alias_entry* alias;
    const zr_presampled_tri* sampleSets;
    uint32_t sampleSetSize;
    SkyLutView sky;
    const zr_voxel_sample* lvg;
    uint32_t lvgDim[3]; float lvgExtents[3]; float lvgOffsetY;
    const Bvh4Node* nodes;
    const BvhTri* tris;
    const TriMeta* triMeta;
    RhoView rho;
    zr_tex_heap tex;
    uint32_t baseColorMapsOffset, normalMapsOffset, mrMapsOffset, emissiveMapsOffset;
    uint32_t texFilter;
    uint32_t numEmissives;
    uint32_t plain;
    uint32_t numNodes;
    uint32_t numTris;
#ifdef ZR_PROF
    unsigned long long* prof;
#endif
};

#if defined(ZR_PROF) && defined(__HIP_DEVICE_COMPILE__)
__shared__ unsigned long long zrProfAcc[4 * 32];
__device__ __forceinline__ void ProfAdd(int i, unsigned long long v)
{
    const unsigned long long m = __ballot(1);
    if (__lane_id() == (uint32_t)(__ffsll((long long)m) - 1)) zrProfAcc[(threadIdx.x >> 6) * 32 + i] += v;
}
struct ProfScope
{
    int i; unsigned long long t0;
    __device__ __forceinline__ ProfScope(int i_) : i(i_), t0(__builtin_readcyclecounter()) {}
    __device__ __forceinline__ ~ProfScope() { ProfAdd(i, __builtin_readcyclecounter() - t0); }
};
struct ProfKernel
{
    unsigned long long* dst; unsigned long long t0;
    __device__ __forceinline__ ProfKernel(unsigned long long* d) : dst(d), t0(__builtin_readcyclecounter())
    { if ((threadIdx.x & 63u) < 32u) zrProfAcc[(threadIdx.x >> 6) * 32 + (threadIdx.x & 63u)] = 0; }
    __device__ __forceinline__ ~ProfKernel()
    {
        ProfAdd(0, __builtin_readcyclecounter() - t0);
        if ((threadIdx.x & 63u) < 32u) atomicAdd(dst + (threadIdx.x & 63u), zrProfAcc[(threadIdx.x >> 6) * 32 + (threadIdx.x & 63u)]);
    }
};
#define ZR_PROF_SCOPE(i) ProfScope zrProfScope##i(i)
#define ZR_PROF_KERNEL(sc, k) ProfKernel zrProfKernel((sc).prof + 32 * (k))
#else
#define ZR_PROF_SCOPE(i)
#define ZR_PROF_KERNEL(sc, k)
#endif
enum { ZRP_KERNEL = 0, ZRP_TRAV, ZRP_TRAV_CALLS, ZRP_RAYS, ZRP_NODE_ITERS, ZRP_NODE_LANES, ZRP_TRI_ITERS, ZRP_TRI_LANES, ZRP_MATERIAL, ZRP_NEE, ZRP_BSDF, ZRP_MISC0, ZRP_MISC1, ZRP_MISC2, ZRP_MISC3, ZRP_MISC4, ZRP_STEALS, ZRP_STEAL_PAIRS };

struct RawHit { float t, u, v; uint32_t tri; };

ZR_HD uint32_t TriID(uint32_t meshIdx, uint32_t primIdx)
{ uint32_t kx = meshIdx, ky = 0, kz = primIdx; zr_pcg3d(&kx, &ky, &kz); return kx; }

ZR_HD bool TestOpacity(const SceneView& sc, uint32_t meshIdx, uint32_t primIdx, float bu, float bv)
{
    const zr_mesh_instance& md = sc.instances[meshIdx];
    const float alphaFactor = zr_div255((float)(md.alpha_factor_cutoff & 0xffu));
    const float cutoff = zr_div255((float)(md.alpha_factor_cutoff >> 8));
    if (cutoff == 1.0f) return false;
    float alpha = alphaFactor;
    if (md.base_color_tex != 0xffffu)
    {
        const uint32_t tri = primIdx * 3 + md.base_idx_offset;
        const zr_vertex& V0 = sc.vertices[sc.indices[tri] + md.base_vtx_offset];
        const zr_vertex& V1 = sc.vertices[sc.indices[tri + 1] + md.base_vtx_offset];
        const zr_vertex& V2_ = sc.vertices[sc.indices[tri + 2] + md.base_vtx_offset];
        const float u = V0.uv[0] + bu * (V1.uv[0] - V0.uv[0]) + bv * (V2_.uv[0] - V0.uv[0]);
        const float v = V0.uv[1] + bu * (V1.uv[1] - V0.uv[1]) + bv * (V2_.uv[1] - V0.uv[1]);
        float c[4];
        zr_tex_sample_level(&sc.tex, sc.baseColorMapsOffset + md.base_color_tex, u, v, 0.0f, c);
        alpha *= c[3];
    }
    if (alpha < cutoff) return false;
    return true;
}

struct TravStack;
ZR_HD BvhTri FetchTri(const SceneView& sc, uint32_t i, const TravStack* st);
template<bool CullNonOpaque = false>
ZR_HD void IntersectTri(const SceneView& sc, uint32_t i, V3 o, V3 d, float tmin, float tmax,
    uint32_t mask, RawHit& best, bool filterID = false, uint32_t ignoreID = 0, bool alphaTest = false, const TravStack* st = nullptr)
{
    const BvhTri T = FetchTri(sc, i, st);
    if (!(T.mask & mask)) return;
    if (CullNonOpaque && (T.mask & ZR_INSTANCE_NON_OPAQUE)) return;
    if (filterID && T.id == ignoreID) return;
    float t, u, v;
    if (zr_ray_tri(o.x, o.y, o.z, d.x, d.y, d.z, T.v0[0], T.v0[1], T.v0[2], T.e1[0], T.e1[1], T.e1[2],
            T.e2[0], T.e2[1], T.e2[2], tmin, tmax, &t, &u, &v))
    {
        if (alphaTest && (T.mask & ZR_INSTANCE_NON_OPAQUE))
        { const TriMeta tm = sc.triMeta[T.gidx]; if (!TestOpacity(sc, tm.mesh, tm.prim, u, v)) return; }
        if (best.tri == kInvalidTri || t < best.t || (t == best.t && T.gidx < best.tri))
        { best.t = t; best.u = u; best.v = v; best.tri = T.gidx; }
    }
}
template<bool CullNonOpaque = false>
ZR_HD void IntersectLeaf(const SceneView& sc, uint32_t first, uint32_t count, V3 o, V3 d, float tmin, float tmax,
    uint32_t mask, RawHit& best, bool filterID = false, uint32_t ignoreID = 0, bool alphaTest = false)
{
    for (uint32_t i = first; i < first + count; i++) IntersectTri<CullNonOpaque>(sc, i, o, d, tmin, tmax, mask, best, filterID, ignoreID, alphaTest);
}

static constexpr int kTravStack = 64;
static constexpr int kTravStackWords = 2 * kTravStack;
#ifndef ZR_TRI_PHASE_WHOLE_LEAF
#define ZR_TRI_PHASE_WHOLE_LEAF 1
#endif
#ifndef ZR_VOTE_WN
#define ZR_VOTE_WN 1
#define ZR_VOTE_WT 1
#endif
#ifndef ZR_TRAV_LDS_ENTRIES
#define ZR_TRAV_LDS_ENTRIES 8
#endif
#ifndef ZR_STEAL
#define ZR_STEAL 0
#endif
#ifndef ZR_STEAL_MIN_IDLE
#define ZR_STEAL_MIN_IDLE 16
#endif
#ifndef ZR_STEAL_MIN_PAIRS
#define ZR_STEAL_MIN_PAIRS 2
#endif
#ifndef ZR_STEAL_COOLDOWN
#define ZR_STEAL_COOLDOWN 1
#endif
static constexpr int kTravLdsEntries = ZR_TRAV_LDS_ENTRIES;

struct StackEntry { uint32_t child; float t; };
#ifdef __HIP_DEVICE_COMPILE__
#define ZR_LDS_AS __attribute__((address_space(3)))
#define ZR_PRIVATE_AS __attribute__((address_space(5)))
#else
#define ZR_LDS_AS
#define ZR_PRIVATE_AS
#endif
#ifndef ZR_NODE_CACHE
#define ZR_NODE_CACHE 32
#endif
struct alignas(16) NodeQuad { uint32_t x, y, z, w; };
struct TravStack { ZR_LDS_AS StackEntry* lds; uint32_t stride; ZR_PRIVATE_AS StackEntry* mem; uint32_t* aux = nullptr; const ZR_LDS_AS NodeQuad* cache = nullptr;
    uint32_t cacheNodes = 0;
    const ZR_LDS_AS NodeQuad* triCache = nullptr; uint32_t cacheTris = 0;
    uint32_t voteTri = ZR_VOTE_WT; };
static constexpr uint32_t kStealAuxWords = 64 * 2 + 64 * 3 + 64;

ZR_HD BvhTri FetchTri(const SceneView& sc, uint32_t i, const TravStack* st)
{
#if defined(__HIP_DEVICE_COMPILE__)
    if (st != nullptr && st->triCache != nullptr && i < st->cacheTris)
    {
        const ZR_LDS_AS NodeQuad* c = st->triCache + 3u * i;
        BvhTri T;
        T.v0[0] = zr_asfloat(c[0].x); T.v0[1] = zr_asfloat(c[0].y); T.v0[2] = zr_asfloat(c[0].z); T.gidx = c[0].w;
        T.e1[0] = zr_asfloat(c[1].x); T.e1[1] = zr_asfloat(c[1].y); T.e1[2] = zr_asfloat(c[1].z); T.mask = c[1].w;
        T.e2[0] = zr_asfloat(c[2].x); T.e2[1] = zr_asfloat(c[2].y); T.e2[2] = zr_asfloat(c[2].z); T.id = c[2].w;
        return T;
    }
#endif
    return sc.tris[i];
}
ZR_HD void StackWrite(const TravStack& st, int e, uint32_t c, float t)
{
// ... 158 lines not shown
    L.triCur++;
    if (anyHit && s.best.tri != kInvalidTri) { L.done = true; L.triCur = L.triEnd; }
    else if (L.triCur == L.triEnd) TravPopEnter(sc, s, L, stack);
}

#if ZR_STEAL
#define ZR_STEAL_ANYHIT anyH
#else
#define ZR_STEAL_ANYHIT anyHit
#endif
#if defined(__HIP_DEVICE_COMPILE__) && ZR_STEAL
__device__ __forceinline__ unsigned long long StealKey(const RawHit& b)
{ return ((unsigned long long)zr_asuint(b.t + 0.0f) << 32) | b.tri; }
__device__ __forceinline__ void StealPublish(const TravStack& st, uint32_t owner, const RawHit& b)
{
    if (b.tri == kInvalidTri) return;
    unsigned long long* keys = (unsigned long long*)st.aux;
    const unsigned long long key = StealKey(b);
    atomicMin(&keys[owner], key);
    if (((volatile unsigned long long*)keys)[owner] == key)
    { float* pl = (float*)(st.aux + 128) + 3 * owner; pl[0] = b.t; pl[1] = b.u; pl[2] = b.v; }
}
#endif

template<bool CullNonOpaque = false>
ZR_HD RawHit TraverseDyn(const SceneView& sc, V3 o, V3 d, float tmin, float tmax, uint32_t mask, const TravStack& stack, bool anyHit,
    bool filterID = false, uint32_t ignoreID = 0, bool alphaTest = false)
{
    TravState s;
    TravInit(sc, s, o, d, tmin, tmax, mask, filterID, ignoreID);
#ifdef __HIP_DEVICE_COMPILE__
#ifdef ZR_PROF
    ZR_PROF_SCOPE(ZRP_TRAV);
    unsigned long long pNI = 0, pNL = 0, pTI = 0, pTL = 0, pST = 0, pSP = 0;
    ProfAdd(ZRP_TRAV_CALLS, 1); ProfAdd(ZRP_RAYS, __popcll(__ballot(1)));
#endif
    TravLane L; L.triCur = 0; L.triEnd = 0; L.done = false;
    TravEnter(sc, s, L, s.cur);
#if ZR_STEAL
    const uint32_t lane = __lane_id();
    uint32_t owner = lane;
    bool pub = true;
    bool stolen = false;
    int cool = 0;
    bool anyH = anyHit;
#endif
    for (;;)
    {
        const bool atTri = L.triCur < L.triEnd;
        const bool atNode = !L.done && !atTri;
        const uint64_t mNode = __ballot(atNode), mTri = __ballot(atTri);
        if ((mNode | mTri) == 0) break;
#if ZR_STEAL
        if (cool > 0) cool--;
        else
        {
            const uint64_t mIdle = __ballot(L.done);
            if (__popcll(mIdle) >= ZR_STEAL_MIN_IDLE)
            {
                const bool canGive = !L.done && s.sp >= 1 && s.sp <= kTravLdsEntries;
                const uint64_t mDon = __ballot(canGive);
                const uint32_t nPairs = (uint32_t)min(__popcll(mIdle), __popcll(mDon));
                if (nPairs >= ZR_STEAL_MIN_PAIRS)
                {
                    unsigned long long* keys = (unsigned long long*)stack.aux;
                    uint32_t* pairLane = stack.aux + 128 + 192;
                    if (!stolen) { keys[lane] = ~0ull; stolen = true; pub = false; }
                    const uint64_t lt = (1ull << lane) - 1ull;
                    const uint32_t rI = (uint32_t)__popcll(mIdle & lt), rD = (uint32_t)__popcll(mDon & lt);
                    const bool give = canGive && rD < nPairs, take = L.done && rI < nPairs;
                    if (give) pairLane[rD] = lane;
                    if (take && !pub) StealPublish(stack, owner, s.best);
                    const int src = take ? (int)((volatile uint32_t*)pairLane)[rI] : (int)lane;
                    const float ox = __shfl(s.o.x, src), oy = __shfl(s.o.y, src), oz = __shfl(s.o.z, src);
                    const float dx = __shfl(s.d.x, src), dy = __shfl(s.d.y, src), dz = __shfl(s.d.z, src);
                    const float tmn = __shfl(s.tmin, src), bt = __shfl(s.best.t, src);
                    const uint32_t msk = __shfl(s.mask, src), ign = __shfl(s.ignoreID, src), own = __shfl(owner, src);
                    const int dsp = __shfl(s.sp, src);
                    const int flg = __shfl((int)s.filterID | ((int)anyH << 1) | ((int)(s.best.tri != kInvalidTri) << 2), src);
                    if (take)
                    {
                        TravInit(sc, s, v3(ox, oy, oz), v3(dx, dy, dz), tmn, (flg & 4) ? NextFloat32(bt) : bt, msk, (flg & 1) != 0, ign);
                        anyH = (flg & 2) != 0; owner = own; pub = false;
                        const ZR_LDS_AS StackEntry* e = stack.lds + (uint32_t)(dsp - 1) * stack.stride + (src - (int)lane);
                        const uint32_t c = e->child; const float et = e->t;
                        L.triCur = 0; L.triEnd = 0;
                        if (et <= zr_widen_far(bt)) { L.done = false; TravEnter(sc, s, L, c); }
                    }
                    if (give) s.sp--;
                    if (anyH && !L.done && !take && ((volatile unsigned long long*)keys)[owner] != ~0ull) { L.done = true; L.triCur = L.triEnd; }
                    cool = ZR_STEAL_COOLDOWN;
#ifdef ZR_PROF
                    pST++; pSP += nPairs;
#endif
                    continue;
                }
            }
        }
#endif
#ifdef ZR_PROF
        if (ZR_VOTE_WN * __popcll(mNode) >= (int)stack.voteTri * __popcll(mTri)) { pNI++; pNL += __popcll(mNode); } else { pTI++; pTL += __popcll(mTri); }
#endif
        if (ZR_VOTE_WN * __popcll(mNode) >= (int)stack.voteTri * __popcll(mTri)) { if (atNode) TravNodePhase(sc, s, L, stack, ZR_STEAL_ANYHIT); }
        else { if (atTri) TravTriPhase<CullNonOpaque>(sc, s, L, stack, ZR_STEAL_ANYHIT, alphaTest); }
    }
#if ZR_STEAL
    if (stolen)
    {
        if (!pub) StealPublish(stack, owner, s.best);
        const unsigned long long key = ((volatile unsigned long long*)stack.aux)[lane];
        if (key == ~0ull) { s.best.t = tmax; s.best.u = 0; s.best.v = 0; s.best.tri = kInvalidTri; }
        else
        {
            const volatile float* pl = (volatile float*)(stack.aux + 128) + 3 * lane;
            s.best.t = pl[0]; s.best.u = pl[1]; s.best.v = pl[2]; s.best.tri = (uint32_t)(key & 0xffffffffull);
        }
    }
#endif
#ifdef ZR_PROF
    ProfAdd(ZRP_NODE_ITERS, pNI); ProfAdd(ZRP_NODE_LANES, pNL); ProfAdd(ZRP_TRI_ITERS, pTI); ProfAdd(ZRP_TRI_LANES, pTL);
    ProfAdd(ZRP_STEALS, pST); ProfAdd(ZRP_STEAL_PAIRS, pSP);
#endif
#else
    while (!TravStep<CullNonOpaque>(sc, s, stack, anyHit, alphaTest)) {}
#endif
    return s.best;
}
template<bool AnyHit>
ZR_HD RawHit Traverse(const SceneView& sc, V3 o, V3 d, float tmin, float tmax, uint32_t mask, const TravStack& stack, bool filterID = false, uint32_t ignoreID = 0)
{ return TraverseDyn(sc, o, d, tmin, tmax, mask, stack, AnyHit, filterID, ignoreID); }

ZR_HD bool MatDoubleSided(const zr_material& m) { return m.coat_color_flags & (1u << ZR_MAT_DOUBLE_SIDED_BIT); }
ZR_HD bool MatMetallic(const zr_material& m) { return m.coat_color_flags & (1u << ZR_MAT_METALLIC_BIT); }
ZR_HD bool MatTransmissive(const zr_material& m) { return m.coat_color_flags & (1u << ZR_MAT_TRANSMISSIVE_BIT); }
ZR_HD bool MatThinWalled(const zr_material& m) { return m.coat_color_flags & (1u << ZR_MAT_THIN_WALLED_BIT); }
ZR_HD float MatRoughness(const zr_material& m) { return zr_div255((float)((m.mr_tex_spec_roughness_coat_roughness >> 16) & 0xff)); }
ZR_HD float MatCoatRoughness(const zr_material& m) { return zr_div255((float)((m.mr_tex_spec_roughness_coat_roughness >> 24) & 0xff)); }
ZR_HD float MatIOR(const zr_material& m) { return zr_fma(1.5f / 65535.0f, (float)(m.emissive_strength_ior >> 16), kMinIOR); }
ZR_HD float MatCoatIOR(const zr_material& m) { return zr_fma(1.5f / 255.0f, (float)((m.emissive_tex_alpha_cutoff_coat_ior >> 24) & 0xff), kMinIOR); }
ZR_HD float MatTrDepth(const zr_material& m) { return zr_f16_to_f32((uint16_t)(m.normal_tex_tr_depth >> 16)); }
ZR_HD float MatSubsurface(const zr_material& m) { return zr_div255((float)((m.base_color_tex_subsurf_coat_weight >> 16) & 0xff)); }
ZR_HD float MatCoatWeight(const zr_material& m) { return zr_div255((float)((m.base_color_tex_subsurf_coat_weight >> 24) & 0xff)); }
ZR_HD float MatEmissiveStrength(const zr_material& m) { return zr_f16_to_f32((uint16_t)(m.emissive_strength_ior & 0xffff)); }

struct HitInfo { float t; V3 normal; uint32_t ID; uint32_t meshIdx; uint32_t matIdx; V3 dndu, dndv, dpdu, dpdv; V2 uv; };

template<bool WantDiffs>
ZR_HD void FillHit(const SceneView& sc, uint32_t meshIdx, uint32_t primIdx, float bu, float bv, bool wantID, HitInfo& ret, bool currFrame = true)
{
    const zr_mesh_instance& md = sc.instances[meshIdx];
    ret.matIdx = md.mat_idx;
    ret.meshIdx = meshIdx;
    uint32_t tri = primIdx * 3 + md.base_idx_offset;
    const zr_vertex& V0 = sc.vertices[sc.indices[tri] + md.base_vtx_offset];
    const zr_vertex& V1 = sc.vertices[sc.indices[tri + 1] + md.base_vtx_offset];
    const zr_vertex& V2_ = sc.vertices[sc.indices[tri + 2] + md.base_vtx_offset];

    V4 q = normalize(DecodeNormalized4(currFrame ? md.rotation : md.prev_rotation));
    const uint16_t* sh = currFrame ? md.scale : md.prev_scale;
    V3 s = v3(zr_f16_to_f32(sh[0]), zr_f16_to_f32(sh[1]), zr_f16_to_f32(sh[2]));

    float tmp = 1 - bu - bv;
    V2 uv = v2(zr_fma(bv, V2_.uv[0], tmp * V0.uv[0]), zr_fma(bv, V2_.uv[1], tmp * V0.uv[1]));
    ret.uv = v2(zr_fma(bu, V1.uv[0], uv.x), zr_fma(bu, V1.uv[1], uv.y));

    V3 v0_n = DecodeOct32(V0.normal), v1_n = DecodeOct32(V1.normal), v2_n = DecodeOct32(V2_.normal);
    V3 hn = mad(bv, v2_n, tmp * v0_n);
    hn = mad(bu, v1_n, hn);
    const V3 scaleInv = v3(1.0f / s.x, 1.0f / s.y, 1.0f / s.z);
    hn = hn * scaleInv;
    hn = RotateVector(hn, q);
    ret.normal = normalize(hn);

    if (WantDiffs)
    {
        V3 trn = v3p(md.translation);
        if (!currFrame) trn = trn - v3(zr_f16_to_f32(md.d_translation[0]), zr_f16_to_f32(md.d_translation[1]), zr_f16_to_f32(md.d_translation[2]));
        V3 v0W = TransformTRS(v3p(V0.pos), trn, q, s);
        V3 v1W = TransformTRS(v3p(V1.pos), trn, q, s);
        V3 v2W = TransformTRS(v3p(V2_.pos), trn, q, s);
        V3 n0W = normalize(RotateVector(v0_n * scaleInv, q));
        V3 n1W = normalize(RotateVector(v1_n * scaleInv, q));
        V3 n2W = normalize(RotateVector(v2_n * scaleInv, q));
        TriDiffs td = ComputeTriDiffs(v0W, v1W, v2W, n0W, n1W, n2W, v2(V0.uv[0], V0.uv[1]), v2(V1.uv[0], V1.uv[1]), v2(V2_.uv[0], V2_.uv[1]));
        ret.dpdu = td.dpdu; ret.dpdv = td.dpdv; ret.dndu = td.dndu; ret.dndv = td.dndv;
    }
    ret.ID = 0xffffffffu;
    if (wantID)
    {
        uint32_t kx = meshIdx, ky = 0, kz = primIdx;
        zr_pcg3d(&kx, &ky, &kz);
        ret.ID = kx;
    }
}

ZR_HD void SampleMaterialTex(const SceneView& sc, uint32_t tex, bool isotropic, V2 uv, V4 g, float out[4])
{
    if (!isotropic) { zr_tex_sample_grad_filter(&sc.tex, tex, sc.texFilter, uv.x, uv.y, g.x, g.y, g.z, g.w, out); return; }
    const zr_texture_desc& d = sc.tex.descs[tex];
    const float mip = zr_log2(zr_max(g.x * (float)d.width, g.y * (float)d.height));
    zr_tex_sample_level(&sc.tex, tex, uv.x, uv.y, mip, out);
}

ZR_HD bool GetMaterialData(const SceneView& sc, V3 wo, float eta_curr, HitInfo& hit, Surface& surface, float& eta,
    V4 uv_grads = v4(0, 0, 0, 0), bool tex = false, bool isotropic = false)
{
    const zr_material mat = sc.materials[hit.matIdx];
    const bool hitBackface = dot(wo, hit.normal) < 0;
    eta = kDefaultEtaMat;
    const bool ds = MatDoubleSided(mat);
    if (!ds && hitBackface) return false;
    if (ds && hitBackface)
    {
        hit.normal = hit.normal * -1.0f;
        if (tex) { hit.dndu = hit.dndu * -1.0f; hit.dndv = hit.dndv * -1.0f; }
    }
    V3 baseColor = UnpackRGB8(mat.base_color_factor);
    float metallic = MatMetallic(mat) ? 1.0f : 0.0f;
    float roughness = MatRoughness(mat);
    bool tr = MatTransmissive(mat);
    eta = MatIOR(mat);
    float trDepth = tr ? MatTrDepth(mat) : 0;
    if (tex)
    {
        const uint32_t baseColorTex = mat.base_color_tex_subsurf_coat_weight & 0xffffu;
        const uint32_t mrTex = mat.mr_tex_spec_roughness_coat_roughness & 0xffffu;
        if ((trDepth == 0) && (baseColorTex != ZR_INVALID_TEX))
        {
            float c[4];
            SampleMaterialTex(sc, sc.baseColorMapsOffset + baseColorTex, isotropic, hit.uv, uv_grads, c);
            baseColor = baseColor * v3(c[0], c[1], c[2]);
        }
        if (mrTex != ZR_INVALID_TEX)
        {
            float c[4];
            SampleMaterialTex(sc, sc.mrMapsOffset + mrTex, isotropic, hit.uv, uv_grads, c);
            metallic *= c[0];
            roughness *= c[1];
        }
    }
    float eta_next = eta_curr == kEtaAir ? eta : kEtaAir;
    float subsurface = MatThinWalled(mat) ? zr_round_f16(MatSubsurface(mat)) : 0;
    surface = InitSurface(hit.normal, wo, metallic >= kMinMetalnessMetal, roughness, baseColor, eta_curr, eta_next, tr, trDepth,
        subsurface, MatCoatWeight(mat), UnpackRGB8(mat.coat_color_flags), MatCoatRoughness(mat), MatCoatIOR(mat), sc.plain != 0);
    return true;
}

ZR_HD bool EmDoubleSided(const zr_emissive_triangle& t) { return t.packed_a & (1u << 25); }
ZR_HD V3 EmV1(const zr_emissive_triangle& t)
{
    V3 d = DecodeUnitVector(v2(zr_div65535((float)t.v0v1[0]), zr_div65535((float)t.v0v1[1])));
    return mad(zr_f16_to_f32(t.edge_lengths[0]), d, v3p(t.vtx0));
}
ZR_HD V3 EmV2(const zr_emissive_triangle& t)
{
    V3 d = DecodeUnitVector(v2(zr_div65535((float)t.v0v2[0]), zr_div65535((float)t.v0v2[1])));
    return mad(zr_f16_to_f32(t.edge_lengths[1]), d, v3p(t.vtx0));
}
struct PresampledLight { V3 pos, normal, le; float pdf; uint32_t idx, ID; bool twoSided; };
ZR_HD PresampledLight SamplePresampledSet(const SceneView& sc, uint32_t sampleSetIdx, V3 shadingPos, Rng& rng)
{
    uint32_t u = rng.UniformUintBounded_Faster(sc.sampleSetSize);
    const zr_presampled_tri t = sc.sampleSets[(size_t)sampleSetIdx * sc.sampleSetSize + u];
    PresampledLight r;
    r.pos = v3p(t.pos); r.normal = DecodeOct32(t.normal);
    r.le = v3(zr_f16_to_f32(t.le[0]), zr_f16_to_f32(t.le[1]), zr_f16_to_f32(t.le[2]));
    r.pdf = t.pdf; r.idx = t.idx; r.ID = t.id; r.twoSided = t.two_sided != 0;
    if (r.twoSided && dot(shadingPos - r.pos, r.normal) < 0) r.normal = r.normal * -1.0f;
    return r;
}

ZR_HD V2 EmUV(const uint16_t* h) { return v2(zr_f16_to_f32(h[0]), zr_f16_to_f32(h[1])); }
ZR_HD V3 EmLe(const SceneView& sc, const zr_emissive_triangle& t, V2 bary)
{
    V3 le = UnpackRGB8(t.packed_a) * zr_f16_to_f32((uint16_t)(t.packed_b >> 16));
    if (Luminance(le) == 0) return v3(0.0f);
    const uint32_t emissiveTex = t.packed_b & 0xffffu;
    if (emissiveTex != ZR_INVALID_TEX)
    {
        const V2 texUV = (1.0f - bary.x - bary.y) * EmUV(t.uv0) + bary.x * EmUV(t.uv1) + bary.y * EmUV(t.uv2);
        float c[4];
        zr_tex_point(&sc.tex, sc.emissiveMapsOffset + emissiveTex, texUV.x, texUV.y, c);
        le = le * v3(c[0], c[1], c[2]);
    }
    return le;
}

}
```

zetaray_amd/csrc/zr_kernels.h:

```cpp
#pragma once
#include <hip/hip_runtime.h>
#include "zr_stages.h"
#include "zr_rpt.h"

using namespace zr;

static constexpr int kBlock = 256;
#ifndef ZR_RPT_BLOCK
#define ZR_RPT_BLOCK 64
#endif
static constexpr int kRptBlock = ZR_RPT_BLOCK;
#define ZR_WAVES(n) __attribute__((amdgpu_waves_per_eu(n, n)))
#define ZR_WAVES_MIN(n) __attribute__((amdgpu_waves_per_eu(n)))
#ifndef ZR_WAVES_PATHTRACE_N
#define ZR_WAVES_PATHTRACE_N 3
#endif
#ifndef ZR_WAVES_PATHTRACE_LARGE_N
#define ZR_WAVES_PATHTRACE_LARGE_N 4
#endif
#ifndef ZR_WAVES_TEMPORAL_N
#define ZR_WAVES_TEMPORAL_N 4
#endif
#ifndef ZR_WAVES_STC_N
#define ZR_WAVES_STC_N 4
// ... 437 lines not shown
}

#ifndef ZR_RECON_BLOCK
#define ZR_RECON_BLOCK 256
#endif
static constexpr int kReconBlock = ZR_RECON_BLOCK;
#ifndef ZR_STC_BLOCK
#define ZR_STC_BLOCK ZR_RECON_BLOCK
#endif
#ifndef ZR_STC_LDS
#define ZR_STC_LDS 0
#endif
static constexpr int kStcBlock = ZR_STC_BLOCK;
#ifndef ZR_VOTE_WT_STC
#define ZR_VOTE_WT_STC 2
#endif

template<bool EMISSIVE, bool TEX, bool PLAIN = false>
__global__ void __launch_bounds__(kReconBlock) ZR_WAVES_TEMPORAL k_rpt_temporal(rpt::RptFrame F, zr_frame_constants g, uint32_t tilesX, unsigned long long* counters)
{
    const unsigned long long t0 = __builtin_readcyclecounter();
    F.prm.emissive = EMISSIVE ? 1u : 0u; F.prm.textured = TEX ? 1u : 0u;
    rpt::SetMaterialClass(F, PLAIN);
    uint32_t x, y; PixelOfThreadB<kReconBlock>(tilesX, F.ox0, F.oy0, &x, &y);
    if (F.prm.temporalMap && F.Owns(x, y)) { const uint16_t e = (F.prm.temporalMap == 1u ? F.mapCtN : F.mapNtC)[rpt::Pix(F.gb, x, y)]; rpt::DecodeSorted(e & 0x7fffu, x, y); }
    ZR_TRAV_STACK_B(stack, kReconBlock);
#if ZR_SCENE_LDS
    ZR_SCENE_CACHE_FILL(stack, F.sc, kReconBlock);
#endif
    ZR_PROF_KERNEL(F.sc, 2);
    uint32_t cnt[2] = {0u, 0u};
    if (F.Owns(x, y)) rpt::ReconnectTemporalPixel(F, g, x, y, stack, cnt);
    FlushRayCountersCost(F, counters, cnt, x, y, F.Owns(x, y), t0);
}

__device__ __forceinline__ float WaveSumButterfly(float v)
{
    for (int s = 1; s < 64; s <<= 1) v = v + __shfl_xor(v, s);
    return v;
}

template<bool EMISSIVE, bool TEX, bool PLAIN = false>
__global__ void __launch_bounds__(kStcBlock) ZR_WAVES_STC k_rpt_stc(rpt::RptFrame F, zr_frame_constants g, uint32_t tilesX, unsigned long long* counters)
{
    const unsigned long long t0 = __builtin_readcyclecounter();
    F.prm.emissive = EMISSIVE ? 1u : 0u; F.prm.textured = TEX ? 1u : 0u;
    rpt::SetMaterialClass(F, PLAIN);
    uint32_t x, y; PixelOfThreadB<kStcBlock>(tilesX, F.ox0, F.oy0, &x, &y);
    if (F.prm.sortSpatial && F.Owns(x, y) && !rpt::DecodeSorted(F.mapNtC[rpt::Pix(F.gb, x, y)], x, y)) x = 0xffffffffu;
    ZR_TRAV_STACK_B(stack, kStcBlock);
    stack.voteTri = ZR_VOTE_WT_STC;
#if ZR_SCENE_LDS
    ZR_SCENE_CACHE_FILL(stack, F.sc, kStcBlock);
#endif
    uint32_t cnt[2] = {0u, 0u};
    ZR_PROF_KERNEL(F.sc, 3);
#if ZR_STC_LDS
    __shared__ __attribute__((aligned(16))) uint32_t stcLaneLds[kStcBlock * ((sizeof(rpt::StcLane) + 15) / 16 * 4)];
    rpt::StcLane& a = *reinterpret_cast<rpt::StcLane*>(stcLaneLds + threadIdx.x * ((sizeof(rpt::StcLane) + 15) / 16 * 4));
    a.r_curr.park.p = nullptr; a.r_curr.park.stride = 0; a.r_curr.parked = false; a.r_spatial.park.p = nullptr; a.r_spatial.park.stride = 0; a.r_spatial.parked = false;
#else
    rpt::StcLane a;
    if (!PLAIN) ZR_KEEP_IN_MEMORY(a);
#endif
    float v1, v2, v3, v4;
    { ZR_PROF_SCOPE(ZRP_MISC0); rpt::StcPhase0(F, g, x, y, a, v1, v2); }
    { ZR_PROF_SCOPE(ZRP_MISC1);
    if (a.valid && a.hasN) rpt::ReconnectCtSPixel(F, g, x, y, stack, cnt); }
    const float sum1 = WaveSumButterfly(v1), sum2 = WaveSumButterfly(v2);
    rpt::StcPhase1(F, g, a, sum1, v3);
    const float sum3 = WaveSumButterfly(v3);
    ZR_PROF_SCOPE(ZRP_MISC2);
    rpt::StcPhase2(F, g, a, sum1, stack, cnt, v4);
    const float sum4 = WaveSumButterfly(v4);
    rpt::StcPhase3(F, g, a, sum2 + sum3 + sum4);
    FlushRayCountersCost(F, counters, cnt, x, y, x != 0xffffffffu && F.Owns(x, y), t0);
}

template<bool EMISSIVE, bool TEX>
__global__ void __launch_bounds__(kRptBlock) __attribute__((amdgpu_waves_per_eu(TEX ? 6 : ZR_WAVES_PATHTRACE_LARGE_N, TEX ? 6 : ZR_WAVES_PATHTRACE_LARGE_N)))
k_rpt_pathtrace_view(rpt::RptFrame F, zr_frame_constants g, uint32_t tilesX, unsigned long long* counters, uint32_t view)
{ RptPathtraceBody<EMISSIVE, TEX, !TEX, false, false, true>(F, g, tilesX, counters, view); }
template<bool EMISSIVE, bool TEX>
__global__ void __launch_bounds__(kReconBlock) ZR_WAVES(ZR_WAVES_TEMPORAL_N) k_rpt_temporal_view(rpt::RptFrame F, zr_frame_constants g, uint32_t tilesX, unsigned long long* counters, uint32_t view)
{
    const unsigned long long t0 = __builtin_readcyclecounter();
    F.prm.emissive = EMISSIVE ? 1u : 0u; F.prm.textured = TEX ? 1u : 0u;
    rpt::SetMaterialClass(F, false);
    uint32_t x, y; PixelOfThreadB<kReconBlock>(tilesX, F.ox0, F.oy0, &x, &y);
    if (F.prm.temporalMap && F.Owns(x, y)) { const uint16_t e = (F.prm.temporalMap == 1u ? F.mapCtN : F.mapNtC)[rpt::Pix(F.gb, x, y)]; rpt::DecodeSorted(e & 0x7fffu, x, y); }
    ZR_TRAV_STACK_B(stack, kReconBlock);
#if ZR_SCENE_LDS
    ZR_SCENE_CACHE_FILL(stack, F.sc, kReconBlock);
#endif
    ZR_PROF_KERNEL(F.sc, 2);
    uint32_t cnt[2] = {0u, 0u};
    if (F.Owns(x, y)) rpt::ReconnectTemporalPixel<true>(F, g, x, y, stack, cnt, view);
    FlushRayCountersCost(F, counters, cnt, x, y, F.Owns(x, y), t0);
}
template<bool EMISSIVE, bool TEX>
__global__ void __launch_bounds__(kStcBlock) ZR_WAVES(ZR_WAVES_STC_N) k_rpt_stc_view(rpt::RptFrame F, zr_frame_constants g, uint32_t tilesX, unsigned long long* counters, uint32_t view)
{
    const unsigned long long t0 = __builtin_readcyclecounter();
    F.prm.emissive = EMISSIVE ? 1u : 0u; F.prm.textured = TEX ? 1u : 0u;
    rpt::SetMaterialClass(F, false);
    uint32_t x, y; PixelOfThreadB<kStcBlock>(tilesX, F.ox0, F.oy0, &x, &y);
    if (F.prm.sortSpatial && F.Owns(x, y) && !rpt::DecodeSorted(F.mapNtC[rpt::Pix(F.gb, x, y)], x, y)) x = 0xffffffffu;
    ZR_TRAV_STACK_B(stack, kStcBlock);
    stack.voteTri = ZR_VOTE_WT_STC;
#if ZR_SCENE_LDS
    ZR_SCENE_CACHE_FILL(stack, F.sc, kStcBlock);
#endif
    uint32_t cnt[2] = {0u, 0u};
    ZR_PROF_KERNEL(F.sc, 3);
#if ZR_STC_LDS
    __shared__ __attribute__((aligned(16))) uint32_t stcLaneLds[kStcBlock * ((sizeof(rpt::StcLane) + 15) / 16 * 4)];
    rpt::StcLane& a = *reinterpret_cast<rpt::StcLane*>(stcLaneLds + threadIdx.x * ((sizeof(rpt::StcLane) + 15) / 16 * 4));
    a.r_curr.park.p = nullptr; a.r_curr.park.stride = 0; a.r_curr.parked = false; a.r_spatial.park.p = nullptr; a.r_spatial.park.stride = 0; a.r_spatial.parked = false;
#else
    rpt::StcLane a;
    ZR_KEEP_IN_MEMORY(a);
#endif
    float v1, v2, v3, v4;
    { ZR_PROF_SCOPE(ZRP_MISC0); rpt::StcPhase0(F, g, x, y, a, v1, v2); }
    { ZR_PROF_SCOPE(ZRP_MISC1);
    if (a.valid && a.hasN) rpt::ReconnectCtSPixel(F, g, x, y, stack, cnt); }
    const float sum1 = WaveSumButterfly(v1), sum2 = WaveSumButterfly(v2);
    rpt::StcPhase1<true>(F, g, a, sum1, v3, view);
    const float sum3 = WaveSumButterfly(v3);
    ZR_PROF_SCOPE(ZRP_MISC2);
    rpt::StcPhase2<true>(F, g, a, sum1, stack, cnt, v4, view);
    const float sum4 = WaveSumButterfly(v4);
    rpt::StcPhase3<true>(F, g, a, sum2 + sum3 + sum4, view);
    FlushRayCountersCost(F, counters, cnt, x, y, x != 0xffffffffu && F.Owns(x, y), t0);
}


#define ZR_RPT_ARGS_TILE (rpt::RptFrame, zr_frame_constants, uint32_t, unsigned long long*)
#define ZR_RPT_ARGS_LIST (rpt::RptFrame, zr_frame_constants, const uint32_t*, const uint32_t*, uint32_t*, unsigned long long*)
#define ZR_RPT_GROUP_A(X) \
    X __global__ void k_rpt_pathtrace<true, false> ZR_RPT_ARGS_TILE; X __global__ void k_rpt_pathtrace<false, false> ZR_RPT_ARGS_TILE; \
    X __global__ void k_rpt_pathtrace_w4<true, false> ZR_RPT_ARGS_TILE; X __global__ void k_rpt_pathtrace_w4<false, false> ZR_RPT_ARGS_TILE;
#define ZR_RPT_GROUP_G(X) \
    X __global__ void k_rpt_pathtrace_tex<true> ZR_RPT_ARGS_TILE; X __global__ void k_rpt_pathtrace_tex<false> ZR_RPT_ARGS_TILE; \
    X __global__ void k_rpt_temporal<true, true, false> ZR_RPT_ARGS_TILE; X __global__ void k_rpt_temporal<false, true, false> ZR_RPT_ARGS_TILE;
#define ZR_RPT_GROUP_H(X) \
    X __global__ void k_rpt_temporal<true, false, false> ZR_RPT_ARGS_TILE; X __global__ void k_rpt_temporal<false, false, false> ZR_RPT_ARGS_TILE; \
    X __global__ void k_rpt_stc<true, false, false> ZR_RPT_ARGS_TILE; X __global__ void k_rpt_stc<false, false, false> ZR_RPT_ARGS_TILE;
#define ZR_RPT_GROUP_D(X) \
    X __global__ void k_rpt_stc<true, true, false> ZR_RPT_ARGS_TILE; X __global__ void k_rpt_stc<false, true, false> ZR_RPT_ARGS_TILE;
#define ZR_RPT_GROUP_E(X) \
    X __global__ void k_rpt_pathtrace<true, true> ZR_RPT_ARGS_TILE; X __global__ void k_rpt_pathtrace<false, true> ZR_RPT_ARGS_TILE; \
    X __global__ void k_rpt_pathtrace_w4<true, true> ZR_RPT_ARGS_TILE; X __global__ void k_rpt_pathtrace_w4<false, true> ZR_RPT_ARGS_TILE; \
    X __global__ void k_rpt_temporal<true, false, true> ZR_RPT_ARGS_TILE; X __global__ void k_rpt_temporal<false, false, true> ZR_RPT_ARGS_TILE; \
    X __global__ void k_rpt_stc<true, false, true> ZR_RPT_ARGS_TILE; X __global__ void k_rpt_stc<false, false, true> ZR_RPT_ARGS_TILE;
#define ZR_RPT_GROUP_C(X) \
    X __global__ void k_rpt_pathtrace_park<true> ZR_RPT_ARGS_TILE; X __global__ void k_rpt_pathtrace_park<false> ZR_RPT_ARGS_TILE; \
    X __global__ void k_rpt_pathtrace_coop<false> ZR_RPT_ARGS_TILE; X __global__ void k_rpt_pathtrace_coop_w4<false> ZR_RPT_ARGS_TILE; \
    X __global__ void k_rpt_pathtrace_trip<false> ZR_RPT_ARGS_TILE; X __global__ void k_rpt_pathtrace_trip_w4<false> ZR_RPT_ARGS_TILE; \
    X __global__ void k_rpt_pt_first<true> ZR_RPT_ARGS_TILE; X __global__ void k_rpt_pt_first<false> ZR_RPT_ARGS_TILE; \
    X __global__ void k_rpt_pt_next<true> ZR_RPT_ARGS_TILE; X __global__ void k_rpt_pt_next<false> ZR_RPT_ARGS_TILE;
#define ZR_RPT_GROUP_B(X) \
    X __global__ void k_rpt_replay<RPT_REPLAY_CTT, true, true> ZR_RPT_ARGS_LIST; X __global__ void k_rpt_replay<RPT_REPLAY_CTT, true, false> ZR_RPT_ARGS_LIST;
#define ZR_RPT_GROUP_I(X) \
    X __global__ void k_rpt_replay<RPT_REPLAY_CTT, false, true> ZR_RPT_ARGS_LIST; X __global__ void k_rpt_replay<RPT_REPLAY_CTT, false, false> ZR_RPT_ARGS_LIST;
#define ZR_RPT_GROUP_F(X) \
    X __global__ void k_rpt_replay<RPT_REPLAY_CTS, true, true> ZR_RPT_ARGS_LIST; X __global__ void k_rpt_replay<RPT_REPLAY_CTS, true, false> ZR_RPT_ARGS_LIST; \
    X __global__ void k_rpt_replay<RPT_REPLAY_CTS, false, true> ZR_RPT_ARGS_LIST; X __global__ void k_rpt_replay<RPT_REPLAY_CTS, false, false> ZR_RPT_ARGS_LIST;
#define ZR_RPT_ARGS_VIEW (rpt::RptFrame, zr_frame_constants, uint32_t, unsigned long long*, uint32_t)
#define ZR_RPT_VIEW_PERMS(X, kern) \
    X __global__ void kern<true, true> ZR_RPT_ARGS_VIEW; X __global__ void kern<true, false> ZR_RPT_ARGS_VIEW; \
    X __global__ void kern<false, true> ZR_RPT_ARGS_VIEW; X __global__ void kern<false, false> ZR_RPT_ARGS_VIEW;
#define ZR_RPT_GROUP_VP(X) ZR_RPT_VIEW_PERMS(X, k_rpt_pathtrace_view)
#define ZR_RPT_GROUP_VT(X) ZR_RPT_VIEW_PERMS(X, k_rpt_temporal_view)
#define ZR_RPT_GROUP_VS(X) ZR_RPT_VIEW_PERMS(X, k_rpt_stc_view)
#define ZR_RPT_GROUPS_PRODUCT(X) ZR_RPT_GROUP_A(X) ZR_RPT_GROUP_B(X) ZR_RPT_GROUP_D(X) ZR_RPT_GROUP_E(X) ZR_RPT_GROUP_F(X) ZR_RPT_GROUP_G(X) ZR_RPT_GROUP_H(X) ZR_RPT_GROUP_I(X) ZR_RPT_GROUP_VP(X) ZR_RPT_GROUP_VT(X) ZR_RPT_GROUP_VS(X)
```

zetaray_amd/csrc/zr_rpt.h:

```cpp
#pragma once
#include "zr_stages.h"

namespace zr {
namespace rpt {

static constexpr float kMaxPlaneDistReuse = 1.0f;
static constexpr float kMaxRoughDiffTemporal = 0.3f;
static constexpr float kMaxRoughDiffSpatial = 0.05f;
static constexpr float kMinNormalSimSpatial = 0.9f;
static constexpr uint32_t kMmaxXkTransmissive = 4, kMmaxXkInMotion = 4;
static constexpr int kNeighborOffset = 32;
#if defined(__HIP_DEVICE_COMPILE__)
#define ZR_KEEP_IN_MEMORY(obj) asm volatile("" :: "v"(&(obj)) : "memory")
#else
#define ZR_KEEP_IN_MEMORY(obj) ((void)0)
#endif
#ifndef ZR_PIN_TEMPORAL
#define ZR_PIN_TEMPORAL 0
#endif
#ifndef ZR_PREP_SHIFT
#define ZR_PREP_SHIFT 1
#endif
static constexpr uint32_t kPrepShift = ZR_PREP_SHIFT;
#ifndef ZR_PREP_SHIFT_PLAIN
// ... 1854 lines not shown
    {
        ctx = LoadOffsetCtx(rbuffer, DTidIdx, rc.IsCase3(), g.textured);
        if (dot(ctx.throughput, ctx.throughput) == 0) return ret;
        for (int b = 0; b < numBounces; b++) for (int k = 0; k < 9; k++) ctx.rngReplay.Uniform();
    }
    ret.surfKMin1Transmissive = ctx.surface.specTr;
    if (!rc.IsCase3())
    {
        ret.partialJacobian = StepPath(g, currFrame, ctx, rc);
        if (ret.partialJacobian == 0) return ret;
        if (rc.IsCase1())
        {
            ZR_PROF_SCOPE(ZRP_NEE);
            SamplerEval e = EvalBSDFSampler(g.sc->rho, ctx.normal, ctx.surface, rc.w, rc.lobe_k, ctx.rngReplay);
            ctx.throughput = ctx.throughput * e.bsdfOverPdf;
            ret.target = ctx.throughput * rc.L;
            ret.partialJacobian *= e.pdf;
            return ret;
        }
    }
    else
    {
        if (!IsLobeValid(ctx.surface, rc.lobe_k_min_1)) return ret;
        if (LobeAlpha(ctx.surface, rc.lobe_k_min_1) < g.alpha_min) return ret;
        if (PrepShiftGroups(g.sc->plain)) PrepareWo(g.sc->rho, ctx.surface, PrepShiftGroups(g.sc->plain));
    }
    Rng rngNEE = Rng::Seed(rc.seed_nee);
    if (!g.emissive)
    {
        const uint32_t lt = rc.IsCase2() ? rc.lt_k_plus_1 : rc.lt_k;
        const uint32_t lobe_a = rc.lobe_k, lobe_b = rc.lobe_k_min_1;
        const uint32_t lobe = rc.IsCase2() ? lobe_a : lobe_b;
        float pdf;
        const V3 target = EstimateDirect_y_k_min_1(g, ctx, lt, rc.w, lobe, rngNEE, pdf);
        ret.target = ctx.throughput * target;
        if (rc.IsCase2()) ret.partialJacobian *= pdf;
        else
        {
            ret.partialJacobian = pdf;
            if (dot(ret.target, ret.target) > 0)
            {
                const V3 wi = rc.lt_k == LT_SUN ? -v3p(g.frame->sun_dir) : rc.w;
                ret.target = ret.target * (VisibilityRay(g, ctx.pos, wi, ctx.normal, ctx.surface.Transmissive()) ? 1.0f : 0.0f);
            }
        }
        return ret;
    }
    ZR_PROF_SCOPE(ZRP_NEE);
    if (rc.IsCase2())
    {
        Direct ls = EvalDirect_Case2(g, ctx.normal, ctx.surface, rc.w, rc.L, rc.dwdA, rc.lightPdf, rc.lobe_k, ctx.rngReplay, rngNEE);
        ret.target = ctx.throughput * ls.ld;
        ret.partialJacobian *= ls.pdf_solidAngle;
    }
    else
    {
        V3 wi = rc.x_k - ctx.pos;
        float t = length(wi);
        wi = wi / t;
        bool twoSided = rc.lightPdf > 0;
        Direct ls = EvalDirect_Case3(g, ctx.pos, ctx.pos, ctx.surface, wi, t, rc.L, rc.w, zr_abs(rc.lightPdf), rc.ID, twoSided, rc.lobe_k_min_1,
            ctx.rngReplay, rngNEE);
        ret.target = ctx.throughput * ls.ld;
        ret.partialJacobian = ls.pdf_solidAngle;
    }
    return ret;
}

struct RptFrame
{
    SceneView sc; GBuf gb, gbPrev; ResPlanes cur, prev;
    SceneView scPrev;
    RBuf rbCtN, rbNtC; RptTex tex; float* finalRGBA; const uint16_t* sampleSet; RptParams prm;
    uint16_t* mapCtN; uint16_t* mapNtC;
    uint32_t ox0, oy0, ow, oh;
    ZR_HDM bool Owns(uint32_t x, uint32_t y) const { return x >= ox0 && y >= oy0 && x < ox0 + ow && y < oy0 + oh; }
    uint32_t* costMap; uint32_t costW; uint32_t costMode;
    uint32_t* trip; unsigned long long* tripStats; size_t tripStride;
    uint32_t* carryOut; const uint32_t* carryIn; uint32_t* carryCount; size_t carryCap; uint32_t carryBounce;
};

ZR_HD void SetMaterialClass(RptFrame& F, bool plain)
{ const uint32_t p = plain ? 1u : 0u; F.sc.plain = p; F.scPrev.plain = p; F.gb.plain = p; F.gbPrev.plain = p; F.rbCtN.plain = p; F.rbNtC.plain = p; }
ZR_HD Globals MakeGlobals(const RptFrame& F, const zr_frame_constants& g, bool transmissive, TravStack stack, uint32_t* cnt)
{
    Globals gl; gl.textured = F.prm.textured != 0; gl.sc = &F.sc; gl.scPrev = &F.scPrev; gl.frame = &g; gl.emissive = F.prm.emissive != 0; gl.numEmissives = g.num_emissive_triangles; gl.alpha_min = F.prm.alpha_min; gl.stack = stack; gl.cnt = cnt; gl.presampled = false; gl.sampleSetIdx = 0;
    gl.maxNumBounces = transmissive ? (int)F.prm.maxGlossyTrBounces : (int)F.prm.maxNonTrBounces;
    return gl;
}

struct TemporalPixel { bool ok; int px, py; PixelSurface prev; };
ZR_HD TemporalPixel FindTemporal(const RptFrame& F, const zr_frame_constants& g, uint32_t x, uint32_t y, const PixelSurface& cur, float planeTh,
    bool coatAtDTid)
{
    TemporalPixel t; t.ok = false; t.px = 0; t.py = 0;
    const V2 renderDim = v2((float)g.render_width, (float)g.render_height);
    const size_t px = Pix(F.gb, x, y);
    const V2 motionVec = DecodeMotion(F.gb.motion[px]);
    const V2 currUV = v2(((float)x + 0.5f) / renderDim.x, ((float)y + 0.5f) / renderDim.y);
    const V2 prevUV = currUV - motionVec;
    int ppx = (int)(prevUV.x * renderDim.x), ppy = (int)(prevUV.y * renderDim.y);
    if (prevUV.x < 0 || prevUV.y < 0 || prevUV.x > 1 || prevUV.y > 1) return t;
    if (ppx >= (int)g.render_width || ppy >= (int)g.render_height) return t;
    if (!InPlanes(F.gb, ppx, ppy)) return t;
    const size_t pp = Pix(F.gb, (uint32_t)ppx, (uint32_t)ppy);
    if (F.gbPrev.depth[pp] == ZR_FLT_MAX) return t;
    const Camera pcam = PrevCamera(g);
    t.prev = LoadPixelSurface(F.gbPrev, pcam, (uint32_t)ppx, (uint32_t)ppy, g.frame_num - 1, coatAtDTid ? px : pp);
    float planeDist = zr_abs(dot(cur.normal, t.prev.pos - cur.pos));
    if (!(planeDist <= planeTh * cur.z)) return t;
    if (t.prev.flags.emissive || (zr_abs(t.prev.roughness - cur.roughness) > kMaxRoughDiffTemporal) || (t.prev.flags.transmissive != cur.flags.transmissive)) return t;
    t.ok = true; t.px = ppx; t.py = ppy;
    return t;
}

ZR_HD_FLAT void ReplayTemporalPixel(const RptFrame& F, const zr_frame_constants& g, int variant, uint32_t x, uint32_t y, TravStack stack, uint32_t* cnt)
{
    const size_t px = Pix(F.gb, x, y);
    GFlags flags = DecodeFlags(F.gb.mr[px]);
    if (flags.invalid || flags.emissive) return;
    const Camera cam = CurrCamera(g);
    PixelSurface ps = LoadPixelSurface(F.gb, cam, x, y, g.frame_num, px);
    TemporalPixel tp = FindTemporal(F, g, x, y, ps, 0.01f, false);
    if (!tp.ok) return;
    Globals gl = MakeGlobals(F, g, flags.transmissive, stack, cnt);
    const size_t pp = Pix(F.gb, (uint32_t)tp.px, (uint32_t)tp.py);
    if (variant == 0)
    {
        Reservoir r = Load_Metadata(F.cur, px);
        if (!r.rc.Empty() && (r.rc.k > 2))
        {
            r.Load_Reconnection(F.cur, px, F.prm.emissive != 0);
            Globals glP = gl; glP.sc = &F.scPrev;
            OffsetCtx ctx = Replay_kGt2(glP, false, tp.prev.pos, tp.prev.normal, tp.prev.eta_next, tp.prev.surface, r.rc,
                MakePrimaryDiffs(PrevCamera(g), tp.px, tp.py, tp.prev, F.gbPrev, pp), true);
            WriteOffsetCtx(ctx, F.rbCtN, px, r.rc.IsCase3(), gl.textured);
        }
    }
    else
    {
        Reservoir r = Load_Metadata(F.prev, pp);
        if (!r.rc.Empty() && (r.rc.k > 2))
        {
            r.Load_Reconnection(F.prev, pp, F.prm.emissive != 0);
            OffsetCtx ctx = Replay_kGt2(gl, true, ps.pos, ps.normal, ps.eta_next, ps.surface, r.rc, MakePrimaryDiffs(cam, (int)x, (int)y, ps, F.gb, px));
            WriteOffsetCtx(ctx, F.rbNtC, px, r.rc.IsCase3(), gl.textured);
        }
    }
}

ZR_HD void MoveXk(const SceneView& sc, Reconnection& rc, bool currToPrev, bool setMotionFlag)
{
    const zr_mesh_instance& md = sc.instances[rc.meshIdx];
    V4 q_curr = normalize(DecodeNormalized4(md.rotation));
    V4 q_prev = normalize(DecodeNormalized4(md.prev_rotation));
    V3 s_curr = v3(zr_f16_to_f32(md.scale[0]), zr_f16_to_f32(md.scale[1]), zr_f16_to_f32(md.scale[2]));
    V3 s_prev = v3(zr_f16_to_f32(md.prev_scale[0]), zr_f16_to_f32(md.prev_scale[1]), zr_f16_to_f32(md.prev_scale[2]));
    V3 dT = v3(zr_f16_to_f32(md.d_translation[0]), zr_f16_to_f32(md.d_translation[1]), zr_f16_to_f32(md.d_translation[2]));
    V3 t_curr = v3p(md.translation), t_prev = t_curr - dT;
    if (currToPrev) rc.x_k = TransformTRS(InverseTransformTRS(rc.x_k, t_curr, q_curr, s_curr), t_prev, q_prev, s_prev);
    else rc.x_k = TransformTRS(InverseTransformTRS(rc.x_k, t_prev, q_prev, s_prev), t_curr, q_curr, s_curr);
    if (setMotionFlag)
    {
        V4 dRot = v4(q_prev.x - q_curr.x, q_prev.y - q_curr.y, q_prev.z - q_curr.z, q_prev.w - q_curr.w);
        V3 dScale = s_prev - s_curr;
        rc.x_k_in_motion = dot(dT, dT) > 0;
        rc.x_k_in_motion = rc.x_k_in_motion || dot(dRot, dRot) > 0;
        rc.x_k_in_motion = rc.x_k_in_motion || dot(dScale, dScale) > 0;
    }
}

template<bool VIEW = false>
ZR_HD void ReconnectTemporalPixel(const RptFrame& F, const zr_frame_constants& g, uint32_t x, uint32_t y, TravStack stack, uint32_t* cnt, uint32_t view = RPT_VIEW_NONE)
{
    const size_t px = Pix(F.gb, x, y);
    GFlags flags = DecodeFlags(F.gb.mr[px]);
    if (flags.invalid || flags.emissive) return;
    const bool doSpatial = F.prm.doSpatial;
    const Camera cam = CurrCamera(g);
    PixelSurface ps; TemporalPixel tp;
    if ((ZR_PIN_TEMPORAL & 1) && !F.sc.plain) ZR_KEEP_IN_MEMORY(ps);
    if ((ZR_PIN_TEMPORAL & 2) && !F.sc.plain) ZR_KEEP_IN_MEMORY(tp);
    {
    ZR_PROF_SCOPE(ZRP_MISC4);
    ps = LoadPixelSurface(F.gb, cam, x, y, g.frame_num, px);
    tp = FindTemporal(F, g, x, y, ps, kMaxPlaneDistReuse, true);
    }
    Globals gl = MakeGlobals(F, g, flags.transmissive, stack, cnt);
    const size_t pp = Pix(F.gb, (uint32_t)tp.px, (uint32_t)tp.py);

    if (tp.ok)
    {
        Reservoir r_curr = Load_NonReconnection(F.cur, px);
        Reservoir r_prev = Load_Metadata(F.prev, pp);
        if (r_curr.w_sum != 0 && r_prev.M > 0 && !r_curr.rc.Empty())
        {
            r_curr.Load_Reconnection(F.cur, px, F.prm.emissive != 0);
            Globals glP = gl; glP.sc = &F.scPrev;
            if (r_curr.rc.IsCase1() || r_curr.rc.IsCase2()) MoveXk(F.scPrev, r_curr.rc, true, false);
            OffsetPath shift = Shift2(glP, false, px, tp.prev.pos, tp.prev.normal, tp.prev.eta_next, tp.prev.surface, r_curr.rc, F.rbCtN,
                MakePrimaryDiffs(PrevCamera(g), tp.px, tp.py, tp.prev, F.gbPrev, pp));
            float target_prev = Luminance(shift.target);
            if (target_prev > 0)
            {
                float targetLum_curr = r_curr.W > 0 ? r_curr.w_sum / r_curr.W : 0;
                float jacobian = r_curr.rc.partialJacobian > 0 ? shift.partialJacobian / r_curr.rc.partialJacobian : 0;
                float m_curr = targetLum_curr / (targetLum_curr + (float)r_prev.M * target_prev * jacobian);
                r_curr.w_sum *= m_curr;
                F.cur.B[2 * px] = r_curr.w_sum;
            }
        }
    }

    Reservoir r_curr = Load_NonReconnection(F.cur, px);
    r_curr.target = xyz(F.tex.target[px]);
    if (!tp.ok)
    {
        if (!doSpatial) WriteOutputColor<VIEW>(g, F.finalRGBA, px, r_curr.target * r_curr.W, view);
        return;
    }
    Reservoir r_prev = Load_NonReconnection(F.prev, pp);
    const uint32_t M_max = F.prm.M_max_temporal;
    const uint32_t M_new = (r_curr.M + r_prev.M) & 0xffffu;
    if (r_prev.rc.Empty())
    {
        float targetLum = Luminance(r_curr.target);
        r_curr.W = targetLum > 0 ? r_curr.w_sum / targetLum : 0;
        r_curr.M = M_new;
        r_curr.WriteReservoirData2(F.cur, px, M_max);
        if (!doSpatial) WriteOutputColor<VIEW>(g, F.finalRGBA, px, r_curr.target * r_curr.W, view);
        return;
    }
    r_prev.Load_Reconnection(F.prev, pp, F.prm.emissive != 0);
    if (r_prev.rc.IsCase1() || r_prev.rc.IsCase2()) MoveXk(F.sc, r_prev.rc, false, true);
    OffsetPath shift = Shift2(gl, true, px, ps.pos, ps.normal, ps.eta_next, ps.surface, r_prev.rc, F.rbNtC, MakePrimaryDiffs(cam, (int)x, (int)y, ps, F.gb, px));
    float targetLum_curr = Luminance(shift.target);
    float jacobian = r_prev.rc.partialJacobian > 0 ? shift.partialJacobian / r_prev.rc.partialJacobian : 0;
    bool changed = false;
    if (targetLum_curr > 1e-6f && jacobian > 1e-5f)
    {
        Rng rng = Rng::Init(y, x, g.frame_num + 31);
        float targetLum_prev = r_prev.W > 0 ? r_prev.w_sum / r_prev.W : 0;
        float numerator = (float)r_prev.M * targetLum_prev;
        float denom = numerator / jacobian + targetLum_curr;
        float m_prev = denom > 0 ? numerator / denom : 0;
        float w_prev = m_prev * r_prev.W * targetLum_curr;
        if (r_curr.Update(w_prev, shift.target, r_prev.rc, rng)) { r_curr.rc.partialJacobian = shift.partialJacobian; changed = true; }
    }
    float targetLum = Luminance(r_curr.target);
    r_curr.W = targetLum > 0 ? r_curr.w_sum / targetLum : 0;
    r_curr.M = M_new;
    if (changed)
    {
        r_curr.Write(F.cur, px, M_max, F.prm.emissive != 0);
        if (doSpatial) F.tex.target[px] = f4(Sanitize3(r_curr.target), 0.0f);
    }
    else r_curr.WriteReservoirData(F.cur, px, M_max);
    if (!doSpatial)
    {
        V3 li = r_curr.target * r_curr.W;
        if (VIEW) DebugColor(r_curr.rc, view, li);
        WriteOutputColor<VIEW>(g, F.finalRGBA, px, li, view, false);
    }
}

ZR_HD uint32_t ReplayClass(uint32_t a) { const uint32_t k = a & 0xfu; return (k == Reconnection::EMPTY || k == 0u) ? 0u : (k < 3u ? k : 3u); }
ZR_HD uint32_t NeedsReplayCtT(const RptFrame& F, uint32_t x, uint32_t y)
{
    const size_t px = Pix(F.gb, x, y);
    GFlags flags = DecodeFlags(F.gb.mr[px]);
    if (flags.invalid || flags.emissive) return 0u;
    return ReplayClass(F.cur.A[px]);
}
ZR_HD uint32_t NeedsReplayTtC(const RptFrame& F, const zr_frame_constants& g, uint32_t x, uint32_t y)
{
    const size_t px = Pix(F.gb, x, y);
    GFlags flags = DecodeFlags(F.gb.mr[px]);
    if (flags.invalid || flags.emissive) return false;
    const V2 renderDim = v2((float)g.render_width, (float)g.render_height);
    const V2 motionVec = DecodeMotion(F.gb.motion[px]);
    const V2 prevUV = v2(((float)x + 0.5f) / renderDim.x, ((float)y + 0.5f) / renderDim.y) - motionVec;
    if (prevUV.x < 0 || prevUV.y < 0 || prevUV.x > 1 || prevUV.y > 1) return false;
    const int ppx = (int)(prevUV.x * renderDim.x), ppy = (int)(prevUV.y * renderDim.y);
    if (ppx >= (int)g.render_width || ppy >= (int)g.render_height || !InPlanes(F.gb, ppx, ppy)) return false;
    return ReplayClass(F.prev.A[Pix(F.gb, (uint32_t)ppx, (uint32_t)ppy)]);
}

ZR_HD V3 WorldPosSS(float px, float py, V2 renderDim, float z_view, float tanHalfFOV, float aspect, const float* viewInv, V2 jitter)
{
    V2 uv = v2((px + 0.5f + jitter.x) / renderDim.x, (py + 0.5f + jitter.y) / renderDim.y);
    V2 ndc = NDCFromUV(uv);
    V3 d = v3(ndc.x * aspect * tanHalfFOV * z_view, ndc.y * tanHalfFOV * z_view, z_view);
    return v3(viewInv[0] * d.x + viewInv[1] * d.y + viewInv[2] * d.z + viewInv[3],
              viewInv[4] * d.x + viewInv[5] * d.y + viewInv[6] * d.z + viewInv[7],
              viewInv[8] * d.x + viewInv[9] * d.y + viewInv[10] * d.z + viewInv[11]);
}

struct PlaneFetch
{
    const GBuf* gb;
    ZR_HDM void operator()(int sx, int sy, uint16_t& mr, float& depth, uint32_t& normal) const
    { const size_t sp = Pix(*gb, (uint32_t)sx, (uint32_t)sy); mr = gb->mr[sp]; depth = gb->depth[sp]; normal = gb->normal[sp]; }
};
template<typename Fetch>
ZR_HD void SpatialSearchPixelT(const RptFrame& F, const zr_frame_constants& g, uint32_t x, uint32_t y, const Fetch& fetch)
{
    const GBuf& gb = F.gb;
    const uint32_t W = g.render_width, H = g.render_height;
    const size_t px = Pix(gb, x, y);
    const uint16_t mrp = gb.mr[px];
    GFlags flags = DecodeFlags(mrp);
    if (flags.invalid || flags.emissive) return;
    const V2 renderDim = v2((float)g.render_width, (float)g.render_height);
    const V2 jitter = v2(g.curr_camera_jitter[0], g.curr_camera_jitter[1]);
// ... 324 lines not shown
```

zetaray_amd/csrc/zr_stages.h:

```cpp
#pragma once
#include "zr_dev_scene.h"
#include "../../include/zetaray_amd.h"

namespace zr {

struct alignas(16) F4 { float x, y, z, w; };
struct alignas(16) U4 { uint32_t x, y, z, w; };
ZR_HD F4 f4(V3 a, float w) { F4 r; r.x = a.x; r.y = a.y; r.z = a.z; r.w = w; return r; }
ZR_HD F4 f4(float x, float y, float z, float w) { F4 r; r.x = x; r.y = y; r.z = z; r.w = w; return r; }
ZR_HD V3 xyz(F4 a) { return v3(a.x, a.y, a.z); }

struct GBuf
{
    uint32_t w, h, x0, y0;
    uint32_t* baseColor; uint32_t* normal; uint16_t* mr; uint32_t* motion; uint32_t* emissive; uint8_t* ior;
    uint16_t* coat; float* depth; uint32_t* triA; uint32_t* triB;
    uint32_t plain = 0;
};

ZR_HD float EncodeMetallic(float metalness, bool tr, V3 emissive, float trDepth, float subsurface, float coat_weight)
{
    uint32_t r = tr ? 1u : 0u;
    r |= ((uint32_t)(dot(emissive, emissive) > 0) << 1);
    r |= ((uint32_t)(trDepth > 0) << 3);
    r |= ((uint32_t)(subsurface > 0) << 4);
    r |= ((uint32_t)(coat_weight > 0) << 5);
    r |= ((uint32_t)(metalness >= kMinMetalnessMetal) << 7);
    return zr_div255((float)r);
}
ZR_HD float EncodeIOR(float ior) { return (ior - kMinIOR) / (kMaxIOR - kMinIOR); }
ZR_HD float DecodeIOR(float e) { return zr_fma(e, kMaxIOR - kMinIOR, kMinIOR); }

ZR_HD F4 UVDifferentials(int px, int py, V3 origin, V3 dir, bool thinLens, V2 lensSample, float focusDepth, float t,
    V3 dpdu, V3 dpdv, const zr_frame_constants& g)
{
    const float dpduDotdpdu = dot(dpdu, dpdu);
    const float dpdvDotdpdv = dot(dpdv, dpdv);
    const float dpduDotdpdv = dot(dpdu, dpdv);
    const float det = dpduDotdpdu * dpdvDotdpdv - dpduDotdpdv * dpduDotdpdv;
    if (zr_abs(det) < 1e-7f) return f4(0, 0, 0, 0);

    const V2 renderDim = v2((float)g.render_width, (float)g.render_height);
    const V2 jitter = v2(g.curr_camera_jitter[0], g.curr_camera_jitter[1]);
    V3 dir_cs_x = GeneratePinholeCameraRay_CS(px + 1, py, renderDim, g.aspect_ratio, g.tan_half_fov, jitter);
    V3 dir_cs_y = GeneratePinholeCameraRay_CS(px, py - 1, renderDim, g.aspect_ratio, g.tan_half_fov, jitter);
    if (thinLens)
    {
        dir_cs_x = focusDepth * dir_cs_x - v3(lensSample.x, lensSample.y, 0);
        dir_cs_y = focusDepth * dir_cs_y - v3(lensSample.x, lensSample.y, 0);
    }
    const V3 vbx = Row3(g.curr_view, 0), vby = Row3(g.curr_view, 1), vbz = Row3(g.curr_view, 2);
    const V3 dir_x = normalize(mad(dir_cs_x.x, vbx, mad(dir_cs_x.y, vby, dir_cs_x.z * vbz)));
    const V3 dir_y = normalize(mad(dir_cs_y.x, vbx, mad(dir_cs_y.y, vby, dir_cs_y.z * vbz)));

    const V3 faceNormal = normalize(cross(dpdu, dpdv));
    const V3 p = origin + t * dir;
    const float d = -dot(faceNormal, p);
    const float numerator = -dot(faceNormal, origin) - d;

    float denom_x = dot(faceNormal, dir_x);
    denom_x = (denom_x < 0 ? -1.0f : 1.0f) * zr_max(zr_abs(denom_x), 1e-8f);
    const float t_x = numerator / denom_x;
    const V3 p_x = origin + t_x * dir_x;

    float denom_y = dot(faceNormal, dir_y);
    denom_y = (denom_y < 0 ? -1.0f : 1.0f) * zr_max(zr_abs(denom_y), 1e-8f);
    const float t_y = numerator / denom_y;
    const V3 p_y = origin + t_y * dir_y;

    const V3 dpdx = p_x - p;
    const V2 bx = v2(dot(dpdu, dpdx), dot(dpdv, dpdx));
    const V3 dpdy = p_y - p;
    const V2 by = v2(dot(dpdu, dpdy), dot(dpdv, dpdy));
    return f4((dpdvDotdpdv * bx.x + -dpduDotdpdv * bx.y) / det, (-dpduDotdpdv * bx.x + dpduDotdpdu * bx.y) / det,
              (dpdvDotdpdv * by.x + -dpduDotdpdv * by.y) / det, (-dpduDotdpdv * by.x + dpduDotdpdu * by.y) / det);
}

ZR_HD V3 TangentSpaceToWorldSpace(V2 bumpNormal2, V3 tangent, V3 normal, float scale)
{
    V3 bumpNormal = v3(zr_fma(2.0f, bumpNormal2.x, -1.0f), zr_fma(2.0f, bumpNormal2.y, -1.0f), 0.0f);
    bumpNormal.z = zr_sqrt(zr_saturate(1.0f - dot(bumpNormal, bumpNormal)));
    V3 scaledBumpNormal = bumpNormal * v3(scale, scale, 1.0f);
    if (dot(scaledBumpNormal, scaledBumpNormal) < 1e-6f) return normal;
    scaledBumpNormal = normalize(scaledBumpNormal);
    normal = normalize(normal);
    tangent = normalize(tangent - dot(tangent, normal) * normal);
    const V3 bitangent = cross(normal, tangent);
    return scaledBumpNormal.x * tangent + scaledBumpNormal.y * bitangent + scaledBumpNormal.z * normal;
}

ZR_HD void GBufferPixel(const SceneView& sc, const zr_frame_constants& g, const GBuf& gb, uint32_t x, uint32_t y,
    TravStack stack, uint64_t* nClosest, uint32_t* picked = nullptr)
{
    const uint32_t px = (y - gb.y0) * gb.w + (x - gb.x0);
    const V2 renderDim = v2((float)g.render_width, (float)g.render_height);
    const V2 jitter = v2(g.curr_camera_jitter[0], g.curr_camera_jitter[1]);
    const V3 vbx = Row3(g.curr_view, 0), vby = Row3(g.curr_view, 1), vbz = Row3(g.curr_view, 2);

    V2 lens = v2(0, 0);
    V3 dirCS = GeneratePinholeCameraRay_CS((int)x, (int)y, renderDim, g.aspect_ratio, g.tan_half_fov, jitter);
    V3 origin = v3p(g.camera_pos);
    if (g.dof)
    {
        uint32_t hx = x, hy = y, hz = x; zr_pcg3d(&hx, &hy, &hz);
        Rng rng = Rng::Init(hz, hy, g.frame_num);
        lens = UniformSampleDiskConcentric(rng.Uniform2D());
        lens = lens * g.lens_radius;
        origin = origin + mad(lens.x, vbx, lens.y * vby);
        dirCS = g.focus_depth * dirCS - v3(lens.x, lens.y, 0);
    }
    V3 dir = normalize(mad(dirCS.x, vbx, mad(dirCS.y, vby, dirCS.z * vbz)));

    (void)nClosest;
    RawHit h = TraverseDyn(sc, origin, dir, 0.0f, ZR_FLT_MAX, ZR_SUBGROUP_ALL, stack, false, false, 0,  true);

    if (h.tri == kInvalidTri)
    {
        if (picked) *picked = 0xffffffffu;
        gb.depth[px] = ZR_FLT_MAX;
        gb.mr[px] = (uint16_t)FloatToUNorm8(4.0f / 255.0f);
        V3 prevCam = v3(g.prev_view_inv[3], g.prev_view_inv[7], g.prev_view_inv[11]);
        V3 motion = v3p(g.camera_pos) - prevCam;
        V2 mndc = motion.z > 0 ? v2(motion.x / (motion.z * g.tan_half_fov), motion.y / (motion.z * g.tan_half_fov)) : v2(0, 0);
        mndc.x /= g.aspect_ratio;
        V2 muv = UVFromNDC(mndc);
        gb.motion[px] = PackSnorm16(muv.x) | (PackSnorm16(muv.y) << 16);
        gb.baseColor[px] = 0; gb.normal[px] = 0; gb.emissive[px] = 0; gb.ior[px] = 0;
        for (int k = 0; k < 4; k++) { gb.coat[4 * px + k] = 0; gb.triA[4 * px + k] = 0; }
        gb.triB[2 * px] = 0; gb.triB[2 * px + 1] = 0;
        return;
    }

    const TriMeta tm = sc.triMeta[h.tri];
    if (picked) *picked = tm.mesh;
    const zr_mesh_instance& md = sc.instances[tm.mesh];
    uint32_t tri = tm.prim * 3 + md.base_idx_offset;
    const zr_vertex& V0 = sc.vertices[sc.indices[tri] + md.base_vtx_offset];
    const zr_vertex& V1 = sc.vertices[sc.indices[tri + 1] + md.base_vtx_offset];
    const zr_vertex& V2_ = sc.vertices[sc.indices[tri + 2] + md.base_vtx_offset];
    V4 q = normalize(DecodeNormalized4(md.rotation));
    const V3 scale = v3(zr_f16_to_f32(md.scale[0]), zr_f16_to_f32(md.scale[1]), zr_f16_to_f32(md.scale[2]));
    const V3 trn = v3p(md.translation);
    const V2 uv0 = v2(V0.uv[0], V0.uv[1]), uv1 = v2(V1.uv[0], V1.uv[1]), uv2 = v2(V2_.uv[0], V2_.uv[1]);

    V3 v0_n = DecodeOct32(V0.normal), v1_n = DecodeOct32(V1.normal), v2_n = DecodeOct32(V2_.normal);
    V3 normal = v0_n + h.u * (v1_n - v0_n) + h.v * (v2_n - v0_n);
    const V3 scaleInv = v3(1.0f / scale.x, 1.0f / scale.y, 1.0f / scale.z);
    normal = normalize(RotateVector(normal * scaleInv, q));

    const V2 uv = uv0 + h.u * (uv1 - uv0) + h.v * (uv2 - uv0);

    const V3 v0_t = DecodeOct32(V0.tangent), v1_t = DecodeOct32(V1.tangent), v2_t = DecodeOct32(V2_.tangent);
    V3 tangent = v0_t + h.u * (v1_t - v0_t) + h.v * (v2_t - v0_t);
    tangent = normalize(RotateVector(tangent * scale, q));

    V3 v0W = TransformTRS(v3p(V0.pos), trn, q, scale);
    V3 v1W = TransformTRS(v3p(V1.pos), trn, q, scale);
    V3 v2W = TransformTRS(v3p(V2_.pos), trn, q, scale);
    V3 n0W = normalize(RotateVector(v0_n * scaleInv, q));
    V3 n1W = normalize(RotateVector(v1_n * scaleInv, q));
    V3 n2W = normalize(RotateVector(v2_n * scaleInv, q));
    TriDiffs td = ComputeTriDiffs(v0W, v1W, v2W, n0W, n1W, n2W, uv0, uv1, uv2);

    V3 hitPos = mad(h.t, dir, origin);
    V3 posL = InverseTransformTRS(hitPos, trn, q, scale);
    V3 prevT = trn - v3(zr_f16_to_f32(md.d_translation[0]), zr_f16_to_f32(md.d_translation[1]), zr_f16_to_f32(md.d_translation[2]));
    V4 qp = normalize(DecodeNormalized4(md.prev_rotation));
    V3 ps = v3(zr_f16_to_f32(md.prev_scale[0]), zr_f16_to_f32(md.prev_scale[1]), zr_f16_to_f32(md.prev_scale[2]));
    V3 posPrev = TransformTRS(posL, prevT, qp, ps);
    V3 pvPrev = Mul3x4(g.prev_view, posPrev);
    V2 ndcPrev = v2(pvPrev.x / (pvPrev.z * g.tan_half_fov), pvPrev.y / (pvPrev.z * g.tan_half_fov));
    ndcPrev.x /= g.aspect_ratio;
    V2 currUV = v2(((float)x + 0.5f) / renderDim.x, ((float)y + 0.5f) / renderDim.y);
    V2 prevUV = UVFromNDC(ndcPrev) - v2(jitter.x / renderDim.x, jitter.y / renderDim.y);
    V2 motionVec = currUV - prevUV;

    V3 pos = mad(h.t, dir, origin);
    V3 posV = Mul3x4(g.curr_view, pos);
    float z = g.dof ? h.t : posV.z;
    V3 wo = origin - pos;

    const zr_material mat = sc.materials[md.mat_idx];
    const uint32_t baseColorTex = mat.base_color_tex_subsurf_coat_weight & 0xffffu, normalTex = mat.normal_tex_tr_depth & 0xffffu;
    const uint32_t mrTex = mat.mr_tex_spec_roughness_coat_roughness & 0xffffu, emissiveTex = mat.emissive_tex_alpha_cutoff_coat_ior & 0xffffu;
    F4 grads = f4(0, 0, 0, 0);
    if (baseColorTex != ZR_INVALID_TEX || normalTex != ZR_INVALID_TEX || mrTex != ZR_INVALID_TEX)
        grads = UVDifferentials((int)x, (int)y, origin, dir, g.dof != 0, lens, g.focus_depth, h.t, td.dpdu, td.dpdv, g);
    grads = f4(grads.x * g.camera_ray_uv_grads_scale, grads.y * g.camera_ray_uv_grads_scale,
               grads.z * g.camera_ray_uv_grads_scale, grads.w * g.camera_ray_uv_grads_scale);
    V3 baseColor = UnpackRGB8(mat.base_color_factor);
    V3 emissive = UnpackRGB8(mat.emissive_factor_normal_scale);
    float metallic = MatMetallic(mat) ? 1.0f : 0.0f;
    float roughness = MatRoughness(mat);
    V3 sn = normal;
    V3 dndu = td.dndu, dndv = td.dndv;
    if (baseColorTex != ZR_INVALID_TEX)
    {
        float c[4];
        zr_tex_sample_grad_aniso(&sc.tex, g.base_color_maps_desc_heap_offset + baseColorTex, uv.x, uv.y, grads.x, grads.y, grads.z, grads.w, 16, c);
        baseColor = baseColor * v3(c[0], c[1], c[2]);
    }
    if (normalTex != ZR_INVALID_TEX && zr_abs(dot(tangent, tangent)) > 1e-6f)
    {
        float c[4];
        zr_tex_sample_grad_aniso(&sc.tex, g.normal_maps_desc_heap_offset + normalTex, uv.x, uv.y, grads.x, grads.y, grads.z, grads.w, 16, c);
        sn = TangentSpaceToWorldSpace(v2(c[0], c[1]), tangent, normal, zr_div255((float)(mat.emissive_factor_normal_scale >> 24)));
    }
    if (MatDoubleSided(mat) && dot(wo, normal) < 0) { sn = sn * -1.0f; dndu = dndu * -1.0f; dndv = dndv * -1.0f; }
    if (dot(wo, normal) > 0 && dot(wo, sn) < 0)
    {
        wo = normalize(wo);
        sn = sn - dot(sn, wo) * wo;
        sn = 1e-4f * wo + sn;
        sn = normalize(sn);
    }
    if (mrTex != ZR_INVALID_TEX)
    {
        float c[4];
        zr_tex_sample_grad_aniso(&sc.tex, g.metallic_roughness_maps_desc_heap_offset + mrTex, uv.x, uv.y, grads.x, grads.y, grads.z, grads.w, 16, c);
        metallic *= c[0];
        roughness *= c[1];
    }
    if (emissiveTex != ZR_INVALID_TEX)
    {
        float c[4];
        zr_tex_sample_level(&sc.tex, g.emissive_maps_desc_heap_offset + emissiveTex, uv.x, uv.y, 0.0f, c);
        emissive = emissive * v3(c[0], c[1], c[2]);
    }
    emissive = emissive * MatEmissiveStrength(mat);
    bool tr = MatTransmissive(mat);
    float ior = MatIOR(mat);
    float trDepth = tr ? MatTrDepth(mat) : 0;
    float subsurface = MatThinWalled(mat) ? MatSubsurface(mat) : 0;
    float coat_w = MatCoatWeight(mat);
    float encoded = EncodeMetallic(metallic, tr, emissive, trDepth, subsurface, coat_w);

    gb.depth[px] = z;
    V2 en = EncodeUnitVector(sn);
    gb.normal[px] = FloatToUNorm16(en.x) | (FloatToUNorm16(en.y) << 16);
    gb.baseColor[px] = FloatToUNorm8(baseColor.x) | (FloatToUNorm8(baseColor.y) << 8) | (FloatToUNorm8(baseColor.z) << 16) |
        ((subsurface > 0 ? FloatToUNorm8(subsurface) : 0u) << 24);
    gb.mr[px] = (uint16_t)(FloatToUNorm8(encoded) | (FloatToUNorm8(roughness) << 8));
    gb.emissive[px] = dot(emissive, emissive) > 0 ? PackR11G11B10F(vmax(emissive, 0.0f)) : 0u;
    gb.ior[px] = tr ? (uint8_t)FloatToUNorm8(EncodeIOR(ior)) : (uint8_t)0;
    if (coat_w > 0)
    {
        uint32_t c = Float3ToRGB8(UnpackRGB8(mat.coat_color_flags));
        gb.coat[4 * px + 0] = (uint16_t)(c & 0xffff);
        gb.coat[4 * px + 1] = (uint16_t)((c >> 16) | (FloatToUNorm8(coat_w) << 8));
        gb.coat[4 * px + 2] = (uint16_t)(FloatToUNorm8(MatCoatRoughness(mat)) | (FloatToUNorm8(EncodeIOR(MatCoatIOR(mat))) << 8));
        gb.coat[4 * px + 3] = 0;
    }
    else { for (int k = 0; k < 4; k++) gb.coat[4 * px + k] = 0; }
    gb.motion[px] = PackSnorm16(motionVec.x) | (PackSnorm16(motionVec.y) << 16);
    uint32_t a0 = zr_f32_to_f16(td.dpdu.x), a1 = zr_f32_to_f16(td.dpdu.y), a2 = zr_f32_to_f16(td.dpdu.z);
    uint32_t b0 = zr_f32_to_f16(td.dpdv.x), b1 = zr_f32_to_f16(td.dpdv.y), b2 = zr_f32_to_f16(td.dpdv.z);
    uint32_t c0 = zr_f32_to_f16(dndu.x), c1 = zr_f32_to_f16(dndu.y), c2 = zr_f32_to_f16(dndu.z);
    uint32_t d0 = zr_f32_to_f16(dndv.x), d1 = zr_f32_to_f16(dndv.y), d2 = zr_f32_to_f16(dndv.z);
    gb.triA[4 * px + 0] = a0 | (a1 << 16);
    gb.triA[4 * px + 1] = a2 | (b0 << 16);
    gb.triA[4 * px + 2] = b1 | (b2 << 16);
    gb.triA[4 * px + 3] = c0 | (c1 << 16);
    gb.triB[2 * px + 0] = c2 | (d0 << 16);
    gb.triB[2 * px + 1] = d1 | (d2 << 16);
}

static constexpr uint32_t PF_BOUNCE_MASK = 0xfu;
static constexpr uint32_t PF_IN_MEDIUM = 1u << 4;
static constexpr uint32_t PF_DRAIN = 1u << 5;
static constexpr uint32_t PF_PENDING = 1u << 6;
static constexpr uint32_t PF_NLS = 1u << 7;
static constexpr uint32_t PF_MAXB_SHIFT = 8;
static constexpr uint32_t PF_S_RAY = 1u << 12;
static constexpr uint32_t PF_PARKED = 1u << 13;
static constexpr uint32_t PF_RD_PENDING = 1u << 14;

struct PathQueue
{
    U4* s0;
    F4* s1;
    F4* s2;
    F4* s3;
    F4* s4;
    F4* s5;
    F4* s6;
    F4* s7;
    F4* s8;
    F4* t[8];
    F4* rayC_o; F4* rayC_d; F4* rayM_o; F4* rayM_d; F4* rayS_o; F4* rayS_d;
    uint32_t* sLightID;
    U4* hitC; U4* hitM;
    uint32_t* visS;
    uint32_t* rayList;
};

struct PathOut
{
    bool alive;
    U4 s0; F4 s1, s2, s3, s4, s5, s6, s7, s8;
    F4 rayC_o, rayC_d, rayM_o, rayM_d, rayS_o, rayS_d;
    uint32_t sLightID;
    F4 t[8];
};

ZR_HD void PackRayDiffs(const RayDiffs& rd, F4* t)
{
    t[0] = f4(rd.origin_x, rd.uv_grads.x); t[1] = f4(rd.dir_x, rd.uv_grads.y);
    t[2] = f4(rd.origin_y, rd.uv_grads.z); t[3] = f4(rd.dir_y, rd.uv_grads.w);
}
ZR_HD RayDiffs UnpackRayDiffs(F4 t0, F4 t1, F4 t2, F4 t3)
{
    RayDiffs rd; rd.origin_x = xyz(t0); rd.dir_x = xyz(t1); rd.origin_y = xyz(t2); rd.dir_y = xyz(t3);
    rd.uv_grads = v4(t0.w, t1.w, t2.w, t3.w);
    return rd;
}

ZR_HD void WritePath(const PathQueue& q, uint32_t slot, const PathOut& p, bool tex = false)
{
    if (tex) { for (int k = 0; k < 8; k++) q.t[k][slot] = p.t[k]; }
    q.s0[slot] = p.s0; q.s1[slot] = p.s1; q.s2[slot] = p.s2; q.s3[slot] = p.s3; q.s4[slot] = p.s4;
    q.s5[slot] = p.s5; q.s6[slot] = p.s6; q.s7[slot] = p.s7; q.s8[slot] = p.s8;
// ... 621 lines not shown
```

zetaray_amd/csrc/zr_tu_rpt_a.hip:

```cpp
#include "zr_kernels.h"
ZR_RPT_GROUP_A(template)
```

zetaray_amd/csrc/zr_tu_scene_update.hip:

```cpp
#include <hip/hip_runtime.h>
#include <cstddef>
#include "../../include/zr_scene_math.h"

namespace zr {

static constexpr uint32_t kNone = 0xffffffffu;
static constexpr uint32_t kBlock = 256;

template<typename T> __device__ inline T LoadRecord(const T* p)
{
    static_assert(sizeof(T) % 16 == 0, "record size");
    uint4 w[sizeof(T) / 16];
    ZR_UNROLL
    for (uint32_t k = 0; k < sizeof(T) / 16; k++) w[k] = reinterpret_cast<const uint4*>(p)[k];
    T t; __builtin_memcpy(&t, w, sizeof(T));
    return t;
}
template<typename T> __device__ inline void StoreRecord(T* p, const T& v)
{
    uint4 w[sizeof(T) / 16]; __builtin_memcpy(w, &v, sizeof(T));
    ZR_UNROLL
    for (uint32_t k = 0; k < sizeof(T) / 16; k++) reinterpret_cast<uint4*>(p)[k] = w[k];
}
static_assert(sizeof(zr_mesh_instance) == 64 && offsetof(zr_mesh_instance, rotation) == 8 && offsetof(zr_mesh_instance, scale) == 16 &&
    offsetof(zr_mesh_instance, mat_idx) == 22 && offsetof(zr_mesh_instance, base_emissive_tri_offset) == 24 && offsetof(zr_mesh_instance, translation) == 28 &&
    offsetof(zr_mesh_instance, prev_rotation) == 40 && offsetof(zr_mesh_instance, prev_scale) == 48 && offsetof(zr_mesh_instance, d_translation) == 54 &&
    offsetof(zr_mesh_instance, base_color_tex) == 60 && offsetof(zr_mesh_instance, alpha_factor_cutoff) == 62, "MeshInstance layout");
__device__ inline uint16_t Lo16(uint32_t w) { return (uint16_t)(w & 0xffffu); }
__device__ inline uint16_t Hi16(uint32_t w) { return (uint16_t)(w >> 16); }
__device__ inline uint32_t Pack16(uint16_t lo, uint16_t hi) { return (uint32_t)lo | ((uint32_t)hi << 16); }
__device__ inline zr_mesh_instance LoadInstance(const zr_mesh_instance* p)
{
    const uint4 a = reinterpret_cast<const uint4*>(p)[0], b = reinterpret_cast<const uint4*>(p)[1], c = reinterpret_cast<const uint4*>(p)[2], d = reinterpret_cast<const uint4*>(p)[3];
    zr_mesh_instance I;
    I.base_vtx_offset = a.x; I.base_idx_offset = a.y;
    I.rotation[0] = Lo16(a.z); I.rotation[1] = Hi16(a.z); I.rotation[2] = Lo16(a.w); I.rotation[3] = Hi16(a.w);
    I.scale[0] = Lo16(b.x); I.scale[1] = Hi16(b.x); I.scale[2] = Lo16(b.y); I.mat_idx = Hi16(b.y);
    I.base_emissive_tri_offset = b.z;
    I.translation[0] = zr_asfloat(b.w); I.translation[1] = zr_asfloat(c.x); I.translation[2] = zr_asfloat(c.y);
    I.prev_rotation[0] = Lo16(c.z); I.prev_rotation[1] = Hi16(c.z); I.prev_rotation[2] = Lo16(c.w); I.prev_rotation[3] = Hi16(c.w);
    I.prev_scale[0] = Lo16(d.x); I.prev_scale[1] = Hi16(d.x); I.prev_scale[2] = Lo16(d.y);
    I.d_translation[0] = Hi16(d.y); I.d_translation[1] = Lo16(d.z); I.d_translation[2] = Hi16(d.z);
    I.base_color_tex = Lo16(d.w); I.alpha_factor_cutoff = Hi16(d.w);
    return I;
}
__device__ inline void StoreInstance(zr_mesh_instance* p, const zr_mesh_instance& I)
{
    uint4* q = reinterpret_cast<uint4*>(p);
    q[0] = make_uint4(I.base_vtx_offset, I.base_idx_offset, Pack16(I.rotation[0], I.rotation[1]), Pack16(I.rotation[2], I.rotation[3]));
    q[1] = make_uint4(Pack16(I.scale[0], I.scale[1]), Pack16(I.scale[2], I.mat_idx), I.base_emissive_tri_offset, zr_asuint(I.translation[0]));
    q[2] = make_uint4(zr_asuint(I.translation[1]), zr_asuint(I.translation[2]), Pack16(I.prev_rotation[0], I.prev_rotation[1]), Pack16(I.prev_rotation[2], I.prev_rotation[3]));
    q[3] = make_uint4(Pack16(I.prev_scale[0], I.prev_scale[1]), Pack16(I.prev_scale[2], I.d_translation[0]), Pack16(I.d_translation[1], I.d_translation[2]),
        Pack16(I.base_color_tex, I.alpha_factor_cutoff));
}
__device__ inline void LoadMatrix(const float* p, float M[12])
{
    ZR_UNROLL
    for (int k = 0; k < 3; k++) { const float4 r = reinterpret_cast<const float4*>(p)[k]; M[4 * k] = r.x; M[4 * k + 1] = r.y; M[4 * k + 2] = r.z; M[4 * k + 3] = r.w; }
}

__global__ void __launch_bounds__(kBlock) k_mark_moved(uint32_t* slot, const uint32_t* movedIdx, uint32_t nMoved)
{
    const uint32_t j = blockIdx.x * kBlock + threadIdx.x;
    if (j < nMoved) slot[movedIdx[j]] = j;
}

__global__ void __launch_bounds__(kBlock) k_move_emissives(zr_emissive_triangle* emissives, const zr_emissive_triangle* object, const uint32_t* owner,
    const uint32_t* slot, const float* movedXf, uint32_t first, uint32_t end)
{
    const uint32_t k = first + blockIdx.x * kBlock + threadIdx.x;
    if (k >= end) return;
    const uint32_t o = owner[k];
    if (o == kNone) return;
    const uint32_t j = slot[o];
    if (j == kNone) return;
    float M[12]; LoadMatrix(movedXf + 12 * (size_t)j, M);
    const zr_emissive_triangle in = LoadRecord(object + k);
    zr_emissive_triangle out;
    zrsm::EmissiveToWorld(in, M, out);
    StoreRecord(emissives + k, out);
}

__global__ void __launch_bounds__(kBlock) k_move_instances(zr_mesh_instance* cur, const zr_mesh_instance* prev, float* toWorld, uint32_t* slot,
    const float* movedXf, uint32_t n)
{
    const uint32_t i = blockIdx.x * kBlock + threadIdx.x;
    if (i >= n) return;
    zr_mesh_instance I = LoadInstance(prev + i);
    const uint32_t j = slot[i];
    if (j == kNone) zrsm::InstanceBeginFrame(I);
    else
    {
        float M[12], P[12];
        LoadMatrix(movedXf + 12 * (size_t)j, M); LoadMatrix(toWorld + 12 * (size_t)i, P);
        zrsm::InstanceSetWorld(I, M, P);
        ZR_UNROLL
        for (int k = 0; k < 3; k++) reinterpret_cast<float4*>(toWorld + 12 * (size_t)i)[k] = make_float4(M[4 * k], M[4 * k + 1], M[4 * k + 2], M[4 * k + 3]);
        slot[i] = kNone;
    }
    StoreInstance(cur + i, I);
}

hipError_t LaunchMoveInstances(hipStream_t st, zr_mesh_instance* cur, const zr_mesh_instance* prev, float* toWorld, uint32_t n, uint32_t* slot,
    const uint32_t* moved, uint32_t nMoved, zr_emissive_triangle* emissives, const zr_emissive_triangle* object, const uint32_t* owner, uint32_t emFirst, uint32_t emEnd)
{
    const float* movedXf = reinterpret_cast<const float*>(moved);
    const uint32_t* movedIdx = moved + 12 * (size_t)nMoved;
    if (nMoved) hipLaunchKernelGGL(k_mark_moved, dim3((nMoved + kBlock - 1) / kBlock), dim3(kBlock), 0, st, slot, movedIdx, nMoved);
    if (emEnd > emFirst)
        hipLaunchKernelGGL(k_move_emissives, dim3((emEnd - emFirst + kBlock - 1) / kBlock), dim3(kBlock), 0, st, emissives, object, owner, slot, movedXf, emFirst, emEnd);
    if (n) hipLaunchKernelGGL(k_move_instances, dim3((n + kBlock - 1) / kBlock), dim3(kBlock), 0, st, cur, prev, toWorld, slot, movedXf, n);
    return hipGetLastError();
}

}
```

Measured before the change: 5176 Mrays/s.

## Precompute per-instance transform records and decoded vertex normals for hit shading

Adds per-scene device tables: a per-instance record holding the normalized rotation quaternion, scale, inverse scale and delta translation for current and previous frames, plus a float4 table of oct-decoded vertex normals (tangents optional). Hit-surface reconstruction, G-buffer shading and reconnection motion use these tables instead of decoding f16/oct data and computing reciprocals per hit. The tables are refreshed on every scene update and swapped with the prev buffers. Some translation units (K11 general, plain STC) opt out through macros, possibly to avoid register-pressure regressions. In exchange, the 16-byte normal loads per vertex and the 96-byte record add memory traffic.

```diff
diff --git a/zetaray_amd/csrc/zr_api.hip b/zetaray_amd/csrc/zr_api.hip
--- a/zetaray_amd/csrc/zr_api.hip
+++ b/zetaray_amd/csrc/zr_api.hip
@@ -59,6 +59,8 @@
     const post::PickWvp& m, uint32_t dw, uint32_t dh, uint32_t rw, uint32_t rh, int4* tris, uint32_t* count, uint8_t* mask, F4* out, uint32_t* outSrgb); }
 namespace zr { hipError_t LaunchMoveInstances(hipStream_t st, zr_mesh_instance* cur, const zr_mesh_instance* prev, float* toWorld, uint32_t n, uint32_t* slot,
     const uint32_t* moved, uint32_t nMoved, zr_emissive_triangle* emissives, const zr_emissive_triangle* object, const uint32_t* owner, uint32_t emFirst, uint32_t emEnd); }
+namespace zr { hipError_t LaunchFillInstRecs(hipStream_t st, InstRec* recs, const zr_mesh_instance* instances, uint32_t n);
+               hipError_t LaunchFillVtxNormals(hipStream_t st, VtxDir* out, const zr_vertex* vertices, uint32_t n, bool tangent); }
 ZR_RPT_GROUPS_PRODUCT(extern template)
 #ifdef ZR_EXPERIMENTS
 ZR_RPT_GROUP_C(extern template)
@@ -477,6 +479,10 @@
     std::vector<zr_vertex> hVertices; std::vector<uint32_t> hIndices; std::vector<uint8_t> hMask; std::vector<uint32_t> hNumTris;
     DevBuf<zr_mesh_instance> instancesPrev; DevBuf<Bvh4Node> nodesPrev; DevBuf<BvhTri> trisPrev; DevBuf<TriMeta> metaPrev;
     uint32_t numNodesPrev = 0, numTrisPrev = 0; bool hasPrev = false;
+    DevBuf<InstRec> instRecs, instRecsPrev; DevBuf<VtxDir> vtxNormals;
+#if ZR_HIT_TANGENTS
+    DevBuf<VtxDir> vtxTangents;
+#endif
     DevBuf<uint32_t> levelNodes; std::vector<uint32_t> levelOffsets, hLevelOrder; DevBuf<float> nodeBounds, toWorld; bool refitReady = false;
     DevBuf<uint8_t> dMask; DeviceBvhScratch bvhScratch; bool deviceBuilt = false;
     bool aliasStale = false;
@@ -602,6 +608,7 @@
     if (sc->hasPrev)
     {
         v.instances = sc->instancesPrev.p; v.nodes = sc->nodesPrev.p; v.tris = sc->trisPrev.p; v.triMeta = sc->metaPrev.p;
+        v.instRecs = sc->instRecsPrev.p;
         v.numNodes = sc->numNodesPrev; v.numTris = sc->numTrisPrev;
     }
     return v;
@@ -1125,6 +1132,20 @@
     return ZR_OK;
 }
 
+static int SceneFillInstRecs(zr_scene* s, hipStream_t st)
+{
+    HIP_TRY(zr::LaunchFillInstRecs(st, s->instRecs.p, s->instances.p, (uint32_t)s->instances.n));
+    s->view.instRecs = s->instRecs.p;
+    return ZR_OK;
+}
+static int SceneSwapInstRecs(zr_scene* s, size_t n)
+{
+    int r;
+    if (s->instRecsPrev.n != n && (r = s->instRecsPrev.Alloc(n))) return r;
+    std::swap(s->instRecs.p, s->instRecsPrev.p); std::swap(s->instRecs.n, s->instRecsPrev.n);
+    return ZR_OK;
+}
+
 static bool MaterialsArePlain(const std::vector<zr_material>& m)
 {
     const uint32_t lobes = (1u << ZR_MAT_METALLIC_BIT) | (1u << ZR_MAT_TRANSMISSIVE_BIT) | (1u << ZR_MAT_THIN_WALLED_BIT);
@@ -1184,6 +1205,17 @@
     }
     UP(srgb, zr_srgb_to_linear_table, 256);
 #undef UP
+    if ((r = s->instRecs.Alloc(d->num_instances)) || (r = s->vtxNormals.Alloc(d->num_vertices))) { delete s; return r; }
+    if ((r = SceneFillInstRecs(s, nullptr))) { delete s; return r; }
+    { hipError_t e = zr::LaunchFillVtxNormals(nullptr, s->vtxNormals.p, s->vertices.p, d->num_vertices, false);
+      if (e != hipSuccess) { delete s; return Fail(ZR_ERR_HIP, "k_fill_vtx_normals failed: %s", hipGetErrorString(e)); } }
+    s->view.vtxNormals = s->vtxNormals.p;
+#if ZR_HIT_TANGENTS
+    if ((r = s->vtxTangents.Alloc(d->num_vertices))) { delete s; return r; }
+    { hipError_t e = zr::LaunchFillVtxNormals(nullptr, s->vtxTangents.p, s->vertices.p, d->num_vertices, true);
+      if (e != hipSuccess) { delete s; return Fail(ZR_ERR_HIP, "k_fill_vtx_normals failed: %s", hipGetErrorString(e)); } }
+    s->view.vtxTangents = s->vtxTangents.p;
+#endif
     SceneView& v = s->view;
     v.vertices = s->vertices.p; v.indices = s->indices.p; v.instances = s->instances.p; v.materials = s->materials.p;
     v.emissives = s->emissives.p; v.alias = nullptr; v.sampleSets = nullptr; v.sampleSetSize = 0; v.nodes = s->nodes.p; v.tris = s->tris.p; v.triMeta = s->meta.p;
@@ -1317,6 +1349,7 @@
             (s->trisPrev.n < nt && (r = s->trisPrev.Alloc(nt))) || (s->metaPrev.n != s->meta.n && (r = s->metaPrev.Alloc(s->meta.n))) ||
             (s->toWorld.n != 12 * (size_t)n && (r = s->toWorld.Alloc(12 * (size_t)n)))) return r;
         if (!s->hasPrev && !s->refitReady) HIP_TRY(hipMemcpy(s->metaPrev.p, s->meta.p, s->meta.n * sizeof(TriMeta), hipMemcpyDeviceToDevice));
+        if ((r = SceneSwapInstRecs(s, n))) return r;
         std::swap(s->instances.p, s->instancesPrev.p); std::swap(s->instances.n, s->instancesPrev.n);
         std::swap(s->nodes.p, s->nodesPrev.p); std::swap(s->nodes.n, s->nodesPrev.n);
         std::swap(s->tris.p, s->trisPrev.p); std::swap(s->tris.n, s->trisPrev.n);
@@ -1326,10 +1359,11 @@
         HIP_TRY(hipMemcpy(s->toWorld.p, instance_to_world, 12 * (size_t)n * sizeof(float), hipMemcpyHostToDevice));
         s->toWorldDev = true;
         s->view.instances = s->instances.p; s->view.triMeta = s->meta.p;
-        if ((r = DeviceRebuild(s, st)))
+        if ((r = SceneFillInstRecs(s, st)) || (r = DeviceRebuild(s, st)))
         {
             (void)hipDeviceSynchronize();
             std::swap(s->instances.p, s->instancesPrev.p); std::swap(s->instances.n, s->instancesPrev.n);
+            std::swap(s->instRecs.p, s->instRecsPrev.p); std::swap(s->instRecs.n, s->instRecsPrev.n);
             std::swap(s->nodes.p, s->nodesPrev.p); std::swap(s->nodes.n, s->nodesPrev.n);
             std::swap(s->tris.p, s->trisPrev.p); std::swap(s->tris.n, s->trisPrev.n);
             std::swap(s->meta.p, s->metaPrev.p); std::swap(s->meta.n, s->metaPrev.n);
@@ -1349,6 +1383,7 @@
         if (bvh.stackNeed + 1 > (uint32_t)kTravStack) return Fail(ZR_ERR_UNSUPPORTED, "BVH needs %u traversal stack entries (limit %d)", bvh.stackNeed, kTravStack - 1);
         HIP_TRY(hipDeviceSynchronize());
         std::lock_guard<std::mutex> lock(s->mtx);
+        if ((r = SceneSwapInstRecs(s, n))) return r;
         std::swap(s->instances.p, s->instancesPrev.p); std::swap(s->instances.n, s->instancesPrev.n);
         std::swap(s->nodes.p, s->nodesPrev.p); std::swap(s->nodes.n, s->nodesPrev.n);
         std::swap(s->tris.p, s->trisPrev.p); std::swap(s->tris.n, s->trisPrev.n);
@@ -1359,6 +1394,8 @@
         SceneView& v = s->view;
         v.instances = s->instances.p; v.nodes = s->nodes.p; v.tris = s->tris.p; v.triMeta = s->meta.p;
         v.numNodes = (uint32_t)bvh.nodes4.size(); v.numTris = (uint32_t)bvh.tris.size();
+        if ((r = SceneFillInstRecs(s, nullptr))) return r;
+        HIP_TRY(hipStreamSynchronize(nullptr));
         if (bvh.maxDepth > s->maxDepth) s->maxDepth = bvh.maxDepth;
         BvhLevels(bvh.nodes4, s->hLevelOrder, s->levelOffsets);
         if ((r = s->levelNodes.Upload(s->hLevelOrder.data(), s->hLevelOrder.size()))) return r;
@@ -1426,12 +1463,15 @@
             (s->trisPrev.n != nt && (r = s->trisPrev.Alloc(nt))) || (s->metaPrev.n != s->meta.n && (r = s->metaPrev.Alloc(s->meta.n))) ||
             (nodeCap && s->nodeBounds.n < 6 * nodeCap && (r = s->nodeBounds.Alloc(6 * nodeCap))) || (s->toWorld.n != 12 * (size_t)n && (r = s->toWorld.Alloc(12 * (size_t)n)))) return r;
         HIP_TRY(hipMemcpyAsync(s->instancesPrev.p, s->instances.p, instBytes, hipMemcpyDeviceToDevice, st));
+        if (s->instRecsPrev.n != n && (r = s->instRecsPrev.Alloc(n))) return r;
+        HIP_TRY(hipMemcpyAsync(s->instRecsPrev.p, s->instRecs.p, (size_t)n * sizeof(InstRec), hipMemcpyDeviceToDevice, st));
         if (nn) HIP_TRY(hipMemcpyAsync(s->nodesPrev.p, s->nodes.p, nn * sizeof(Bvh4Node), hipMemcpyDeviceToDevice, st));
         HIP_TRY(hipMemcpyAsync(s->trisPrev.p, s->tris.p, nt * sizeof(BvhTri), hipMemcpyDeviceToDevice, st));
         HIP_TRY(hipMemcpyAsync(s->metaPrev.p, s->meta.p, s->meta.n * sizeof(TriMeta), hipMemcpyDeviceToDevice, st));
         s->refitReady = true;
     }
     std::swap(s->instances.p, s->instancesPrev.p); std::swap(s->nodes.p, s->nodesPrev.p); std::swap(s->tris.p, s->trisPrev.p); std::swap(s->meta.p, s->metaPrev.p);
+    std::swap(s->instRecs.p, s->instRecsPrev.p);
     s->numNodesPrev = (uint32_t)nn; s->numTrisPrev = (uint32_t)nt; s->hasPrev = true;
     if (!moved)
     {
@@ -1446,6 +1486,7 @@
             s->emissives.p, s->objectEmissives.p, s->emissiveOwner.p, moved->emFirst, moved->emEnd));
     }
     s->toWorldDev = true;
+    if ((r = SceneFillInstRecs(s, st))) return r;
     if ((r = StageCommit(t, st))) return r;
     uint32_t numNodesNow = (uint32_t)nn;
     if (install)
diff --git a/zetaray_amd/csrc/zr_dev_scene.h b/zetaray_amd/csrc/zr_dev_scene.h
--- a/zetaray_amd/csrc/zr_dev_scene.h
+++ b/zetaray_amd/csrc/zr_dev_scene.h
@@ -1,5 +1,6 @@
 #pragma once
 #include "zr_dev_bsdf.h"
+#include "zr_hit_tables.h"
 #include "zr_sky.h"
 #include "../../include/zr_texture.h"
 #include "../../include/zr_intersect.h"
@@ -46,6 +47,11 @@
     uint32_t plain;
     uint32_t numNodes;
     uint32_t numTris;
+    const InstRec* instRecs = nullptr;
+    const VtxDir* vtxNormals = nullptr;
+#if ZR_HIT_TANGENTS
+    const VtxDir* vtxTangents = nullptr;
+#endif
 #ifdef ZR_PROF
     unsigned long long* prof;
 #endif
@@ -510,22 +516,39 @@
     ret.matIdx = md.mat_idx;
     ret.meshIdx = meshIdx;
     uint32_t tri = primIdx * 3 + md.base_idx_offset;
-    const zr_vertex& V0 = sc.vertices[sc.indices[tri] + md.base_vtx_offset];
-    const zr_vertex& V1 = sc.vertices[sc.indices[tri + 1] + md.base_vtx_offset];
-    const zr_vertex& V2_ = sc.vertices[sc.indices[tri + 2] + md.base_vtx_offset];
-
+    const uint32_t i0 = sc.indices[tri] + md.base_vtx_offset, i1 = sc.indices[tri + 1] + md.base_vtx_offset, i2 = sc.indices[tri + 2] + md.base_vtx_offset;
+    const zr_vertex& V0 = sc.vertices[i0];
+    const zr_vertex& V1 = sc.vertices[i1];
+    const zr_vertex& V2_ = sc.vertices[i2];
+
+#if ZR_HIT_TABLES_DEV
+    const InstRec& rec = sc.instRecs[meshIdx];
+    const InstXform& xf = currFrame ? rec.curr : rec.prev;
+    V4 q = XformQ(xf);
+    V3 s = XformScale(xf);
+#else
     V4 q = normalize(DecodeNormalized4(currFrame ? md.rotation : md.prev_rotation));
     const uint16_t* sh = currFrame ? md.scale : md.prev_scale;
     V3 s = v3(zr_f16_to_f32(sh[0]), zr_f16_to_f32(sh[1]), zr_f16_to_f32(sh[2]));
+#endif
 
     float tmp = 1 - bu - bv;
     V2 uv = v2(zr_fma(bv, V2_.uv[0], tmp * V0.uv[0]), zr_fma(bv, V2_.uv[1], tmp * V0.uv[1]));
     ret.uv = v2(zr_fma(bu, V1.uv[0], uv.x), zr_fma(bu, V1.uv[1], uv.y));
 
+#if ZR_HIT_VTX_NORMALS_DEV
+    const VtxDir vn0 = sc.vtxNormals[i0], vn1 = sc.vtxNormals[i1], vn2 = sc.vtxNormals[i2];
+    V3 v0_n = v3(vn0.x, vn0.y, vn0.z), v1_n = v3(vn1.x, vn1.y, vn1.z), v2_n = v3(vn2.x, vn2.y, vn2.z);
+#else
     V3 v0_n = DecodeOct32(V0.normal), v1_n = DecodeOct32(V1.normal), v2_n = DecodeOct32(V2_.normal);
+#endif
+#if ZR_HIT_TABLES_DEV
+    const V3 scaleInv = XformScaleInv(xf);
+#else
+    const V3 scaleInv = v3(1.0f / s.x, 1.0f / s.y, 1.0f / s.z);
+#endif
     V3 hn = mad(bv, v2_n, tmp * v0_n);
     hn = mad(bu, v1_n, hn);
-    const V3 scaleInv = v3(1.0f / s.x, 1.0f / s.y, 1.0f / s.z);
     hn = hn * scaleInv;
     hn = RotateVector(hn, q);
     ret.normal = normalize(hn);
@@ -533,7 +556,11 @@
     if (WantDiffs)
     {
         V3 trn = v3p(md.translation);
+#if ZR_HIT_TABLES_DEV
+        if (!currFrame) trn = trn - RecDT(rec);
+#else
         if (!currFrame) trn = trn - v3(zr_f16_to_f32(md.d_translation[0]), zr_f16_to_f32(md.d_translation[1]), zr_f16_to_f32(md.d_translation[2]));
+#endif
         V3 v0W = TransformTRS(v3p(V0.pos), trn, q, s);
         V3 v1W = TransformTRS(v3p(V1.pos), trn, q, s);
         V3 v2W = TransformTRS(v3p(V2_.pos), trn, q, s);
diff --git a/zetaray_amd/csrc/zr_hit_tables.h b/zetaray_amd/csrc/zr_hit_tables.h
--- /dev/null
+++ b/zetaray_amd/csrc/zr_hit_tables.h
@@ -0,0 +1,61 @@
+#pragma once
+#include "zr_dev_math.h"
+
+#ifndef ZR_HIT_TABLES
+#define ZR_HIT_TABLES 1
+#endif
+#ifndef ZR_HIT_TANGENTS
+#define ZR_HIT_TANGENTS 0
+#endif
+#ifndef ZR_HIT_VTX_NORMALS
+#define ZR_HIT_VTX_NORMALS 1
+#endif
+#if ZR_HIT_TABLES && defined(__HIP_DEVICE_COMPILE__)
+#define ZR_HIT_TABLES_DEV 1
+#else
+#define ZR_HIT_TABLES_DEV 0
+#endif
+#define ZR_HIT_TANGENTS_DEV (ZR_HIT_TABLES_DEV && ZR_HIT_TANGENTS)
+#define ZR_HIT_VTX_NORMALS_DEV (ZR_HIT_TABLES_DEV && ZR_HIT_VTX_NORMALS)
+
+namespace zr {
+
+struct InstXform { float q[4]; float sInv[3]; float d0; float s[3]; float d1; };
+struct alignas(16) InstRec { InstXform curr, prev; };
+static_assert(sizeof(InstRec) == 96, "InstRec layout");
+
+ZR_HD InstXform MakeInstXform(const uint16_t* rotation, const uint16_t* scale)
+{
+    const V4 q = normalize(DecodeNormalized4(rotation));
+    const V3 s = v3(zr_f16_to_f32(scale[0]), zr_f16_to_f32(scale[1]), zr_f16_to_f32(scale[2]));
+    const V3 sInv = v3(1.0f / s.x, 1.0f / s.y, 1.0f / s.z);
+    InstXform X;
+    X.q[0] = q.x; X.q[1] = q.y; X.q[2] = q.z; X.q[3] = q.w;
+    X.sInv[0] = sInv.x; X.sInv[1] = sInv.y; X.sInv[2] = sInv.z;
+    X.s[0] = s.x; X.s[1] = s.y; X.s[2] = s.z;
+    X.d0 = 0; X.d1 = 0;
+    return X;
+}
+ZR_HD InstRec MakeInstRec(const zr_mesh_instance& md)
+{
+    InstRec R;
+    R.curr = MakeInstXform(md.rotation, md.scale);
+    R.prev = MakeInstXform(md.prev_rotation, md.prev_scale);
+    R.curr.d0 = zr_f16_to_f32(md.d_translation[0]); R.curr.d1 = zr_f16_to_f32(md.d_translation[1]); R.prev.d0 = zr_f16_to_f32(md.d_translation[2]);
+    return R;
+}
+ZR_HD V4 XformQ(const InstXform& X) { return v4(X.q[0], X.q[1], X.q[2], X.q[3]); }
+ZR_HD V3 XformScale(const InstXform& X) { return v3p(X.s); }
+ZR_HD V3 XformScaleInv(const InstXform& X) { return v3p(X.sInv); }
+ZR_HD V3 RecDT(const InstRec& R) { return v3(R.curr.d0, R.curr.d1, R.prev.d0); }
+
+ZR_HD V3 InverseTransformTRS_SInv(V3 pos, V3 tr, V4 rot, V3 scaleInv)
+{
+    V3 t = pos - tr;
+    t = RotateVector(t, v4(-rot.x, -rot.y, -rot.z, rot.w));
+    return t * scaleInv;
+}
+
+struct alignas(16) VtxDir { float x, y, z, w; };
+
+}
diff --git a/zetaray_amd/csrc/zr_kernels.h b/zetaray_amd/csrc/zr_kernels.h
--- a/zetaray_amd/csrc/zr_kernels.h
+++ b/zetaray_amd/csrc/zr_kernels.h
@@ -613,7 +613,8 @@
 #define ZR_RPT_GROUP_E(X) \
     X __global__ void k_rpt_pathtrace<true, true> ZR_RPT_ARGS_TILE; X __global__ void k_rpt_pathtrace<false, true> ZR_RPT_ARGS_TILE; \
     X __global__ void k_rpt_pathtrace_w4<true, true> ZR_RPT_ARGS_TILE; X __global__ void k_rpt_pathtrace_w4<false, true> ZR_RPT_ARGS_TILE; \
-    X __global__ void k_rpt_temporal<true, false, true> ZR_RPT_ARGS_TILE; X __global__ void k_rpt_temporal<false, false, true> ZR_RPT_ARGS_TILE; \
+    X __global__ void k_rpt_temporal<true, false, true> ZR_RPT_ARGS_TILE; X __global__ void k_rpt_temporal<false, false, true> ZR_RPT_ARGS_TILE;
+#define ZR_RPT_GROUP_J(X) \
     X __global__ void k_rpt_stc<true, false, true> ZR_RPT_ARGS_TILE; X __global__ void k_rpt_stc<false, false, true> ZR_RPT_ARGS_TILE;
 #define ZR_RPT_GROUP_C(X) \
     X __global__ void k_rpt_pathtrace_park<true> ZR_RPT_ARGS_TILE; X __global__ void k_rpt_pathtrace_park<false> ZR_RPT_ARGS_TILE; \
@@ -635,4 +636,4 @@
 #define ZR_RPT_GROUP_VP(X) ZR_RPT_VIEW_PERMS(X, k_rpt_pathtrace_view)
 #define ZR_RPT_GROUP_VT(X) ZR_RPT_VIEW_PERMS(X, k_rpt_temporal_view)
 #define ZR_RPT_GROUP_VS(X) ZR_RPT_VIEW_PERMS(X, k_rpt_stc_view)
-#define ZR_RPT_GROUPS_PRODUCT(X) ZR_RPT_GROUP_A(X) ZR_RPT_GROUP_B(X) ZR_RPT_GROUP_D(X) ZR_RPT_GROUP_E(X) ZR_RPT_GROUP_F(X) ZR_RPT_GROUP_G(X) ZR_RPT_GROUP_H(X) ZR_RPT_GROUP_I(X) ZR_RPT_GROUP_VP(X) ZR_RPT_GROUP_VT(X) ZR_RPT_GROUP_VS(X)
+#define ZR_RPT_GROUPS_PRODUCT(X) ZR_RPT_GROUP_A(X) ZR_RPT_GROUP_B(X) ZR_RPT_GROUP_D(X) ZR_RPT_GROUP_E(X) ZR_RPT_GROUP_F(X) ZR_RPT_GROUP_G(X) ZR_RPT_GROUP_H(X) ZR_RPT_GROUP_I(X) ZR_RPT_GROUP_J(X) ZR_RPT_GROUP_VP(X) ZR_RPT_GROUP_VT(X) ZR_RPT_GROUP_VS(X)
diff --git a/zetaray_amd/csrc/zr_rpt.h b/zetaray_amd/csrc/zr_rpt.h
--- a/zetaray_amd/csrc/zr_rpt.h
+++ b/zetaray_amd/csrc/zr_rpt.h
@@ -2030,6 +2030,15 @@
 ZR_HD void MoveXk(const SceneView& sc, Reconnection& rc, bool currToPrev, bool setMotionFlag)
 {
     const zr_mesh_instance& md = sc.instances[rc.meshIdx];
+#if ZR_HIT_TABLES_DEV
+    const InstRec& rec = sc.instRecs[rc.meshIdx];
+    V4 q_curr = XformQ(rec.curr), q_prev = XformQ(rec.prev);
+    V3 s_curr = XformScale(rec.curr), s_prev = XformScale(rec.prev);
+    V3 dT = RecDT(rec);
+    V3 t_curr = v3p(md.translation), t_prev = t_curr - dT;
+    if (currToPrev) rc.x_k = TransformTRS(InverseTransformTRS_SInv(rc.x_k, t_curr, q_curr, XformScaleInv(rec.curr)), t_prev, q_prev, s_prev);
+    else rc.x_k = TransformTRS(InverseTransformTRS_SInv(rc.x_k, t_prev, q_prev, XformScaleInv(rec.prev)), t_curr, q_curr, s_curr);
+#else
     V4 q_curr = normalize(DecodeNormalized4(md.rotation));
     V4 q_prev = normalize(DecodeNormalized4(md.prev_rotation));
     V3 s_curr = v3(zr_f16_to_f32(md.scale[0]), zr_f16_to_f32(md.scale[1]), zr_f16_to_f32(md.scale[2]));
@@ -2038,6 +2047,7 @@
     V3 t_curr = v3p(md.translation), t_prev = t_curr - dT;
     if (currToPrev) rc.x_k = TransformTRS(InverseTransformTRS(rc.x_k, t_curr, q_curr, s_curr), t_prev, q_prev, s_prev);
     else rc.x_k = TransformTRS(InverseTransformTRS(rc.x_k, t_prev, q_prev, s_prev), t_curr, q_curr, s_curr);
+#endif
     if (setMotionFlag)
     {
         V4 dRot = v4(q_prev.x - q_curr.x, q_prev.y - q_curr.y, q_prev.z - q_curr.z, q_prev.w - q_curr.w);
diff --git a/zetaray_amd/csrc/zr_stages.h b/zetaray_amd/csrc/zr_stages.h
--- a/zetaray_amd/csrc/zr_stages.h
+++ b/zetaray_amd/csrc/zr_stages.h
@@ -135,22 +135,43 @@
     if (picked) *picked = tm.mesh;
     const zr_mesh_instance& md = sc.instances[tm.mesh];
     uint32_t tri = tm.prim * 3 + md.base_idx_offset;
-    const zr_vertex& V0 = sc.vertices[sc.indices[tri] + md.base_vtx_offset];
-    const zr_vertex& V1 = sc.vertices[sc.indices[tri + 1] + md.base_vtx_offset];
-    const zr_vertex& V2_ = sc.vertices[sc.indices[tri + 2] + md.base_vtx_offset];
+    const uint32_t i0 = sc.indices[tri] + md.base_vtx_offset, i1 = sc.indices[tri + 1] + md.base_vtx_offset, i2 = sc.indices[tri + 2] + md.base_vtx_offset;
+    const zr_vertex& V0 = sc.vertices[i0];
+    const zr_vertex& V1 = sc.vertices[i1];
+    const zr_vertex& V2_ = sc.vertices[i2];
+#if ZR_HIT_TABLES_DEV
+    const InstRec& rec = sc.instRecs[tm.mesh];
+    V4 q = XformQ(rec.curr);
+    const V3 scale = XformScale(rec.curr);
+#else
     V4 q = normalize(DecodeNormalized4(md.rotation));
     const V3 scale = v3(zr_f16_to_f32(md.scale[0]), zr_f16_to_f32(md.scale[1]), zr_f16_to_f32(md.scale[2]));
+#endif
     const V3 trn = v3p(md.translation);
     const V2 uv0 = v2(V0.uv[0], V0.uv[1]), uv1 = v2(V1.uv[0], V1.uv[1]), uv2 = v2(V2_.uv[0], V2_.uv[1]);
 
+#if ZR_HIT_VTX_NORMALS_DEV
+    const VtxDir vn0 = sc.vtxNormals[i0], vn1 = sc.vtxNormals[i1], vn2 = sc.vtxNormals[i2];
+    V3 v0_n = v3(vn0.x, vn0.y, vn0.z), v1_n = v3(vn1.x, vn1.y, vn1.z), v2_n = v3(vn2.x, vn2.y, vn2.z);
+#else
     V3 v0_n = DecodeOct32(V0.normal), v1_n = DecodeOct32(V1.normal), v2_n = DecodeOct32(V2_.normal);
+#endif
+#if ZR_HIT_TABLES_DEV
+    const V3 scaleInv = XformScaleInv(rec.curr);
+#else
+    const V3 scaleInv = v3(1.0f / scale.x, 1.0f / scale.y, 1.0f / scale.z);
+#endif
     V3 normal = v0_n + h.u * (v1_n - v0_n) + h.v * (v2_n - v0_n);
-    const V3 scaleInv = v3(1.0f / scale.x, 1.0f / scale.y, 1.0f / scale.z);
     normal = normalize(RotateVector(normal * scaleInv, q));
 
     const V2 uv = uv0 + h.u * (uv1 - uv0) + h.v * (uv2 - uv0);
 
+#if ZR_HIT_TANGENTS_DEV
+    const VtxDir vt0 = sc.vtxTangents[i0], vt1 = sc.vtxTangents[i1], vt2 = sc.vtxTangents[i2];
+    const V3 v0_t = v3(vt0.x, vt0.y, vt0.z), v1_t = v3(vt1.x, vt1.y, vt1.z), v2_t = v3(vt2.x, vt2.y, vt2.z);
+#else
     const V3 v0_t = DecodeOct32(V0.tangent), v1_t = DecodeOct32(V1.tangent), v2_t = DecodeOct32(V2_.tangent);
+#endif
     V3 tangent = v0_t + h.u * (v1_t - v0_t) + h.v * (v2_t - v0_t);
     tangent = normalize(RotateVector(tangent * scale, q));
 
@@ -163,10 +184,17 @@
     TriDiffs td = ComputeTriDiffs(v0W, v1W, v2W, n0W, n1W, n2W, uv0, uv1, uv2);
 
     V3 hitPos = mad(h.t, dir, origin);
+#if ZR_HIT_TABLES_DEV
+    V3 posL = InverseTransformTRS_SInv(hitPos, trn, q, scaleInv);
+    V3 prevT = trn - RecDT(rec);
+    V4 qp = XformQ(rec.prev);
+    V3 ps = XformScale(rec.prev);
+#else
     V3 posL = InverseTransformTRS(hitPos, trn, q, scale);
     V3 prevT = trn - v3(zr_f16_to_f32(md.d_translation[0]), zr_f16_to_f32(md.d_translation[1]), zr_f16_to_f32(md.d_translation[2]));
     V4 qp = normalize(DecodeNormalized4(md.prev_rotation));
     V3 ps = v3(zr_f16_to_f32(md.prev_scale[0]), zr_f16_to_f32(md.prev_scale[1]), zr_f16_to_f32(md.prev_scale[2]));
+#endif
     V3 posPrev = TransformTRS(posL, prevT, qp, ps);
     V3 pvPrev = Mul3x4(g.prev_view, posPrev);
     V2 ndcPrev = v2(pvPrev.x / (pvPrev.z * g.tan_half_fov), pvPrev.y / (pvPrev.z * g.tan_half_fov));
diff --git a/zetaray_amd/csrc/zr_tu_rpt_a.hip b/zetaray_amd/csrc/zr_tu_rpt_a.hip
--- a/zetaray_amd/csrc/zr_tu_rpt_a.hip
+++ b/zetaray_amd/csrc/zr_tu_rpt_a.hip
@@ -1,2 +1,9 @@
+#ifndef ZR_HIT_TABLES_K11_GENERAL
+#define ZR_HIT_TABLES_K11_GENERAL 0
+#endif
+#if !ZR_HIT_TABLES_K11_GENERAL
+#undef ZR_HIT_TABLES
+#define ZR_HIT_TABLES 0
+#endif
 #include "zr_kernels.h"
 ZR_RPT_GROUP_A(template)
diff --git a/zetaray_amd/csrc/zr_tu_rpt_j.hip b/zetaray_amd/csrc/zr_tu_rpt_j.hip
--- /dev/null
+++ b/zetaray_amd/csrc/zr_tu_rpt_j.hip
@@ -0,0 +1,9 @@
+#ifndef ZR_HIT_TABLES_STC_PLAIN
+#define ZR_HIT_TABLES_STC_PLAIN 0
+#endif
+#if !ZR_HIT_TABLES_STC_PLAIN
+#undef ZR_HIT_TABLES
+#define ZR_HIT_TABLES 0
+#endif
+#include "zr_kernels.h"
+ZR_RPT_GROUP_J(template)
diff --git a/zetaray_amd/csrc/zr_tu_scene_update.hip b/zetaray_amd/csrc/zr_tu_scene_update.hip
--- a/zetaray_amd/csrc/zr_tu_scene_update.hip
+++ b/zetaray_amd/csrc/zr_tu_scene_update.hip
@@ -1,6 +1,7 @@
 #include <hip/hip_runtime.h>
 #include <cstddef>
 #include "../../include/zr_scene_math.h"
+#include "zr_hit_tables.h"
 
 namespace zr {
 
@@ -101,6 +102,34 @@
     StoreInstance(cur + i, I);
 }
 
+__global__ void __launch_bounds__(kBlock) k_fill_inst_recs(InstRec* recs, const zr_mesh_instance* instances, uint32_t n)
+{
+    const uint32_t i = blockIdx.x * kBlock + threadIdx.x;
+    if (i >= n) return;
+    const zr_mesh_instance I = LoadInstance(instances + i);
+    StoreRecord(recs + i, MakeInstRec(I));
+}
+__global__ void __launch_bounds__(kBlock) k_fill_vtx_normals(VtxDir* out, const zr_vertex* vertices, uint32_t n, bool tangent)
+{
+    const uint32_t i = blockIdx.x * kBlock + threadIdx.x;
+    if (i >= n) return;
+    const uint32_t w = *reinterpret_cast<const uint32_t*>(tangent ? vertices[i].tangent : vertices[i].normal);
+    const uint16_t e[2] = { Lo16(w), Hi16(w) };
+    const V3 d = DecodeOct32(e);
+    VtxDir r; r.x = d.x; r.y = d.y; r.z = d.z; r.w = 0.0f;
+    out[i] = r;
+}
+hipError_t LaunchFillInstRecs(hipStream_t st, InstRec* recs, const zr_mesh_instance* instances, uint32_t n)
+{
+    if (n) hipLaunchKernelGGL(k_fill_inst_recs, dim3((n + kBlock - 1) / kBlock), dim3(kBlock), 0, st, recs, instances, n);
+    return hipGetLastError();
+}
+hipError_t LaunchFillVtxNormals(hipStream_t st, VtxDir* out, const zr_vertex* vertices, uint32_t n, bool tangent)
+{
+    if (n) hipLaunchKernelGGL(k_fill_vtx_normals, dim3((n + kBlock - 1) / kBlock), dim3(kBlock), 0, st, out, vertices, n, tangent);
+    return hipGetLastError();
+}
+
 hipError_t LaunchMoveInstances(hipStream_t st, zr_mesh_instance* cur, const zr_mesh_instance* prev, float* toWorld, uint32_t n, uint32_t* slot,
     const uint32_t* moved, uint32_t nMoved, zr_emissive_triangle* emissives, const zr_emissive_triangle* object, const uint32_t* owner, uint32_t emFirst, uint32_t emEnd)
 {
```

Result: faster. 5267 Mrays/s (median of 6 runs) (+1.8%).
